# adfriend45/HYBRID9

Measured on AMD Instinct MI355X. Metric: grid-cell-steps/sec at 0.5° global (1/2/4/8 GPUs) + achieved HBM GB/s, higher is better.
Workload: dtype f32

## Files before the change

### hybrid9_amd/csrc/h9g.hip

```cpp
#include <hip/hip_runtime.h>

#include <math.h>
#include <stdio.h>
#include <stdlib.h>
#include <string.h>

#include <algorithm>
#include <atomic>
#include <mutex>
#include <string>
#include <thread>
#include <vector>

#include "../../include/h9g.h"
#include "h9_math.h"
#include "h9g_geo.h"
#include "h9g_step.h"
#include "h9g_pair.h"
#include "h9g_rows.h"
#include "h9g_synth.h"
#include "h9g_io.h"

using namespace h9k;
static_assert(H9G_ERR_NOSNAP_K == H9G_ERR_NOSNAP, "kernel and ABI error codes");
static_assert(H9G_NDAILY == DAILY_ROWS, "the daily line of the ABI and of h9g_rows.h");

__constant__ uint64_t c_exp2tab[32] = H9M_EXP2F_TAB_INIT;
__constant__ double c_log2tab[32] = H9M_POWF_LOG2_TAB_INIT;
static const uint64_t h_exp2tab[32] = H9M_EXP2F_TAB_INIT;
static const double h_log2tab[32] = H9M_POWF_LOG2_TAB_INIT;

#define H9G_BLOCK 256
#define H9G_YBLOCK 64
#define H9G_PCPW 22
#define H9G_PLANES (2 * H9G_PCPW)
#define H9G_PWAVES 4
#define NEVT 64
static size_t round_up(size_t x, size_t m) { return (x + m - 1) / m * m; }

struct KArgs {
  int ncell;
  int c0, cend;
  int nt;
  int nisurf;
  int grow_on;
  size_t fvar;
  const float *__restrict__ par;
  float *__restrict__ st;
  const float *__restrict__ forc;
  float *__restrict__ annual;
  int *__restrict__ err;
  int *__restrict__ err_flag;
  unsigned *__restrict__ stamps;
  float *__restrict__ sv;
  const int *__restrict__ perm;
  int sorted_io;
  int *__restrict__ hist;
  unsigned *__restrict__ pace;
  unsigned epoch;
  int prio_mode;
  int bend, split, nt2;
  float *__restrict__ st2;
  int *__restrict__ err2;
  size_t iostride;
  int raw;
};

#define H9G_NXCD 8
__host__ __device__ __forceinline__ unsigned xcd_vwg(unsigned b, unsigned nb) {
  const unsigned x = b % H9G_NXCD, q = nb / H9G_NXCD, r = nb % H9G_NXCD;
  return x * q + (x < r ? x : r) + b / H9G_NXCD;
}

__device__ __forceinline__ void load_tabs(uint64_t *e2, double *l2) {
  const int t = threadIdx.x;
  if (t < 32) {
    e2[t] = c_exp2tab[t];
    l2[t] = c_log2tab[t];
  }
  __syncthreads();
}

template <int L>
constexpr int pair_waves() { return pair_resident<L>(); }

template <int L, class G, int R, int C = H9G_PCPW, bool MON = false>
__device__ __forceinline__ void pair_body(const KArgs &a, const G &g, float *mon = nullptr) {
  typedef PairStore<L, 2 * C, R> PS;
  __shared__ uint64_t s_e2[32];
  __shared__ double s_l2[32];
  __shared__ float s_cell[H9G_PWAVES][PS::ROWS * 2 * C];
  __shared__ float s_zt[zt_size<L>()];
  static_assert(sizeof(s_e2) + sizeof(s_l2) + sizeof(s_cell) + sizeof(s_zt) <= (size_t)PS::GBLOCK,
                "pair kernel LDS footprint exceeds the day-snapshot block");
  if (threadIdx.x == 0) fill_zt<L>(g, s_zt);
  load_tabs(s_e2, s_l2);
  const h9m::Tabs T = {s_e2, s_l2};
  const int wave = threadIdx.x >> 6, lane = threadIdx.x & 63;
  const bool spare = lane >= 2 * C;
  if (spare && !PS::kSpare) return;
  const int h = lane & 1;
  const int slot0 = __builtin_amdgcn_readfirstlane(
      a.c0 + (int)(xcd_vwg(blockIdx.x, gridDim.x) * H9G_PWAVES + wave) * C);
  const bool g2 = slot0 >= a.split;
  const int lim = g2 ? a.cend : a.bend;
  float *const st = g2 ? a.st2 : a.st;
  int *const err = g2 ? a.err2 : a.err;
  int *const hist = g2 ? nullptr : a.hist;
  const int nt = g2 ? a.nt2 : a.nt;
  const int ncol = min(C, lim - slot0);
  if (ncol <= 0) return;
  const int pl = spare ? (lane - 2 * C + (C == H9G_PCPW ? 12 : 0)) % (2 * ncol) : lane;
  const int slot = slot0 + (pl >> 1);
  if (slot >= lim) return;
  const int c = a.perm ? a.perm[slot] : slot;
  const int io = a.sorted_io ? slot : c;
  const int n = a.ncell;
  const size_t ios = a.sorted_io ? a.iostride : (size_t)n;

  int prow, pslot;
  pace_key(prow, pslot);
  PS cs{(lds_float *)&s_cell[wave][pl], (lds_float *)&s_cell[wave][pl & ~1], (const lds_float *)s_zt,
        a.sv + (size_t)blockIdx.x * (PS::GBLOCK / sizeof(float)),
        Pacer{a.pace + (size_t)prow * 16, a.epoch & 0xfffffu, pslot, a.prio_mode,
              (int)((blockIdx.x * (unsigned)PS::RESIDENT) / gridDim.x)},
        (lds_float *)&s_cell[wave][0]};
  const Split2 sp{h, lane, spare};
  St<L> s;
  if (!spare) {
#pragma unroll
    for (int p = PF_TS; p <= PF_PSI; p++)
#pragma unroll
      for (int t = 0; t < L / 2; t++) cs.set_slot(p, t, a.par[(size_t)par_row(L, p, 2 * t + h) * n + c]);
    cs.set_sc(PS_FMAX, a.par[(size_t)Rows<L>::FMAX * n + c]);
#pragma unroll
    for (int t = 0; t < L / 2; t++) cs.set_slot(PF_ROOTR, t, st[(size_t)rootr_row(L, 2 * t + h) * n + c]);
  }
#pragma unroll
  for (int i = 1; i <= L; i++) {
    s.h2o[i] = st[(size_t)(Rows<L>::H2O + i - 1) * n + c];
    s.smp[i] = st[(size_t)(Rows<L>::SMP + i - 1) * n + c];
  }
  H9K_LOAD_SCALARS(L, s, st, n, c)
  cs.launder();

  if (!spare) {
    H9K_TS_SUM(L, cs, ts_sum)
    if (!(ts_sum > SOIL_TRUNC) || err[c] != 0) {
      if (h == 0) nan_rows(a.annual, Rows<L>::ANNUAL, ios, io);
      if constexpr (MON)
        if (h == 0) nan_rows(mon, H9G_NMONTHS * Rows<L>::ANNUAL, ios, io);
      return;
    }
    cell_inv_pair<L, G>(g, cs);
  }
  if (__builtin_amdgcn_ballot_w64(!spare) == 0) return;
  int eday = 0, estep = 0;
  float errval = 0.0f;
#if defined(H9G_STAMPS)
  StampProf pr{stamp_clock(), {0, 0, 0, 0, 0, 0, 0, 0}};
  const int code = cell_year_pair<L, G, Split2, PS, true>(g, cs, sp, s, (const gbl_float *)(a.forc + io), ios, a.fvar, nt,
                                                         a.nisurf, a.grow_on, (gbl_float *)(a.annual + io), ios, eday,
                                                         estep, errval, T, a.raw, pr);
  if (lane == 0 && a.stamps)
    for (int k = 0; k < 8; k++) a.stamps[(blockIdx.x * H9G_PWAVES + wave) * 8 + k] = pr.acc[k];
#else
  int code;
  if constexpr (MON)
    code = cell_year_pair<L, G, Split2, PS, true, NoProf, Months>(
        g, cs, sp, s, (const gbl_float *)(a.forc + io), ios, a.fvar, nt, a.nisurf, a.grow_on,
        (gbl_float *)(a.annual + io), ios, eday, estep, errval, T, a.raw, NoProf(), Months{(gbl_float *)(mon + io), ios});
  else
    code = cell_year_pair<L, G>(g, cs, sp, s, (const gbl_float *)(a.forc + io), ios, a.fvar, nt, a.nisurf,
                                a.grow_on, (gbl_float *)(a.annual + io), ios, eday, estep, errval, T, a.raw);
#endif
  if (spare || h != 0) return;
  int cw = c, iow = io;
  opaque(cw);
  opaque(iow);
  cs.launder();
  if (hist) hist[cw] = s.naq;
  H9K_STORE_CELL(L, s, cs, st, n, cw, a.grow_on, SC_N)
  if (code) {
    stop_write(err, n, cw, code, eday, estep, errval, a.err_flag);
    nan_rows(a.annual, Rows<L>::ANNUAL, ios, iow);
    if constexpr (MON) nan_rows(mon, H9G_NMONTHS * Rows<L>::ANNUAL, ios, iow);
  }
}

template <int L, class G>
__global__ void __launch_bounds__(64 * H9G_PWAVES)
    __attribute__((amdgpu_waves_per_eu(pair_waves<L>(), pair_waves<L>())))
h9g_pair_kernel(const KArgs a, const G g) {
  pair_body<L, G, pair_waves<L>()>(a, g);
}

template <int L, class G>
__global__ void __launch_bounds__(64 * H9G_PWAVES) __attribute__((amdgpu_waves_per_eu(2, 2)))
h9g_pair2_kernel(const KArgs a, const G g) {
  pair_body<L, G, 2>(a, g);
}

#define H9G_PCPW11 11
template <int L, class G>
__global__ void __launch_bounds__(64 * H9G_PWAVES) __attribute__((amdgpu_waves_per_eu(3, 3)))
h9g_pair11_kernel(const KArgs a, const G g) {
  pair_body<L, G, 3, H9G_PCPW11>(a, g);
}

template <int L, class G>
__global__ void __launch_bounds__(64 * H9G_PWAVES) __attribute__((amdgpu_waves_per_eu(1, 1)))
h9g_pair1_kernel(const KArgs a, const G g) {
  pair_body<L, G, 1, 1>(a, g);
}


#define H9G_SOLO_BODY(MON, mon)                                                                                    \
  typedef SoloStore<L> SS;                                                                                         \
  __shared__ uint64_t s_e2[32];                                                                                    \
  __shared__ double s_l2[32];                                                                                      \
  __shared__ float s_cell[SS::ROWS * H9G_YBLOCK];                                                                  \
  __shared__ float s_zt[zt_size<L>()];                                                                             \
  if (threadIdx.x == 0) fill_zt<L>(g, s_zt);                                                                       \
  load_tabs(s_e2, s_l2);                                                                                           \
  const h9m::Tabs T = {s_e2, s_l2};                                                                                \
  const int slot = a.c0 + (int)(xcd_vwg(blockIdx.x, gridDim.x) * blockDim.x + threadIdx.x);                        \
  if (slot >= a.cend) return;                                                                                      \
  const int c = a.perm ? a.perm[slot] : slot;                                                                      \
  const int io = a.sorted_io ? slot : c;                                                                           \
  const int n = a.ncell;                                                                                           \
  const size_t ios = a.sorted_io ? a.iostride : (size_t)n;                                                         \
  SS cs{(lds_float *)&s_cell[threadIdx.x], (const lds_float *)s_zt};                                               \
  const SplitAll sp;                                                                                               \
  St<L> s;                                                                                                         \
  H9K_LOAD_LANE(L, cs, s, a.par, n, c, a.st, n, c)                                                                 \
  H9K_LOAD_SCALARS(L, s, a.st, n, c)                                                                               \
  cs.launder();                                                                                                    \
  H9K_TS_SUM(L, cs, ts_sum)                                                                                        \
  if (!(ts_sum > SOIL_TRUNC) || a.err[c] != 0) {                                                                   \
    nan_rows(a.annual, Rows<L>::ANNUAL, ios, io);                                                                  \
    if constexpr (MON) nan_rows(mon, H9G_NMONTHS * Rows<L>::ANNUAL, ios, io);                                      \
    return;                                                                                                        \
  }                                                                                                                \
  cell_inv_pair<L, G>(g, cs);                                                                                      \
  int eday = 0, estep = 0;                                                                                         \
  float errval = 0.0f;                                                                                             \
  int code;                                                                                                        \
  if constexpr (MON)                                                                                               \
    code = cell_year_pair<L, G, SplitAll, SS, false, NoProf, Months>(                                              \
        g, cs, sp, s, (const gbl_float *)(a.forc + io), ios, a.fvar, a.nt, a.nisurf, a.grow_on,                    \
        (gbl_float *)(a.annual + io), ios, eday, estep, errval, T, a.raw, NoProf(),                                \
        Months{(gbl_float *)(mon + io), ios});                                                                     \
  else                                                                                                             \
    code = cell_year_pair<L, G, SplitAll, SS, false>(g, cs, sp, s, (const gbl_float *)(a.forc + io), ios, a.fvar,  \
                                                     a.nt, a.nisurf, a.grow_on, (gbl_float *)(a.annual + io), ios, \
                                                     eday, estep, errval, T, a.raw);                               \
  int cw = c, iow = io;                                                                                            \
  opaque(cw);                                                                                                      \
  opaque(iow);                                                                                                     \
  cs.launder();                                                                                                    \
  if (a.hist) a.hist[cw] = s.naq;                                                                                  \
  H9K_STORE_CELL(L, s, cs, a.st, n, cw, a.grow_on, SC_N)                                                           \
  if (code) {                                                                                                      \
    stop_write(a.err, n, cw, code, eday, estep, errval, a.err_flag);                                               \
    nan_rows(a.annual, Rows<L>::ANNUAL, ios, iow);                                                                 \
    if constexpr (MON) nan_rows(mon, H9G_NMONTHS * Rows<L>::ANNUAL, ios, iow);                                     \
  }

template <int L, class G>
__global__ void __launch_bounds__(H9G_YBLOCK) __attribute__((amdgpu_waves_per_eu(2, 2)))
h9g_solo_kernel(const KArgs a, const G g) {
  H9G_SOLO_BODY(false, ((float *)nullptr))
}

template <int L, class G>
__global__ void __launch_bounds__(64 * H9G_PWAVES)
    __attribute__((amdgpu_waves_per_eu(pair_waves<L>(), pair_waves<L>())))
h9g_pair_mon_kernel(const KArgs a, float *mon, const G g) {
  pair_body<L, G, pair_waves<L>(), H9G_PCPW, true>(a, g, mon);
}
template <int L, class G>
__global__ void __launch_bounds__(64 * H9G_PWAVES) __attribute__((amdgpu_waves_per_eu(2, 2)))
h9g_pair2_mon_kernel(const KArgs a, float *mon, const G g) {
  pair_body<L, G, 2, H9G_PCPW, true>(a, g, mon);
}
template <int L, class G>
__global__ void __launch_bounds__(64 * H9G_PWAVES) __attribute__((amdgpu_waves_per_eu(3, 3)))
h9g_pair11_mon_kernel(const KArgs a, float *mon, const G g) {
  pair_body<L, G, 3, H9G_PCPW11, true>(a, g, mon);
}
template <int L, class G>
__global__ void __launch_bounds__(64 * H9G_PWAVES) __attribute__((amdgpu_waves_per_eu(1, 1)))
h9g_pair1_mon_kernel(const KArgs a, float *mon, const G g) {
  pair_body<L, G, 1, 1, true>(a, g, mon);
}
template <int L, class G>
__global__ void __launch_bounds__(H9G_YBLOCK) __attribute__((amdgpu_waves_per_eu(2, 2)))
h9g_solo_mon_kernel(const KArgs a, float *mon, const G g) {
  H9G_SOLO_BODY(true, mon)
}

int h9g_mon_launch(int kind, const h9g_config *cfg, unsigned grid, unsigned block, hipStream_t stream, const KArgs &a,
                   float *mon);
int h9g_mon_stopped(int n, int rows, const int *err0, float *mon, hipStream_t stream);

#if !defined(H9G_MONTHLY_UNIT)
#define H9G_PF_ROWS 32
__global__ void __launch_bounds__(256) h9g_perm_forcing_kernel(int c0, int cend, int cpb, int nt, int n, size_t fvar,
                                                               size_t ds, size_t dvar, const int *__restrict__ perm,
                                                               const float *__restrict__ src, float *__restrict__ dst) {
  const unsigned nb = (unsigned)((cend - c0 + cpb - 1) / cpb), x = blockIdx.x % H9G_NXCD, j = blockIdx.x / H9G_NXCD;
  const unsigned q = nb / H9G_NXCD, r = nb % H9G_NXCD, cnt = q + (x < r ? 1u : 0u);
  const unsigned rows = 7u * (unsigned)nt, rgroups = (rows + H9G_PF_ROWS - 1) / H9G_PF_ROWS;
  if (cnt == 0 || j >= cnt * rgroups) return;
  const unsigned v = x * q + (x < r ? x : r) + j % cnt, r0 = (j / cnt) * H9G_PF_ROWS;
  for (unsigned t = threadIdx.x; t < (unsigned)cpb * H9G_PF_ROWS; t += blockDim.x) {
    const int s = c0 + (int)(v * (unsigned)cpb + t % (unsigned)cpb);
    const unsigned row = r0 + t / (unsigned)cpb;
    if (s >= cend || row >= rows) continue;
    const size_t v = row / (unsigned)nt, d = row % (unsigned)nt;
    dst[v * dvar + d * ds + s] = src[v * fvar + d * (size_t)n + perm[s]];
  }
}
static unsigned perm_forcing_blocks(int c0, int cend, int cpb, int nt) {
  const unsigned nb = (unsigned)((cend - c0 + cpb - 1) / cpb);
  const unsigned cmax = nb / H9G_NXCD + (nb % H9G_NXCD ? 1u : 0u);
  return H9G_NXCD * cmax * ((7u * (unsigned)nt + H9G_PF_ROWS - 1) / H9G_PF_ROWS);
}

__global__ void __launch_bounds__(256) h9g_unperm_annual_kernel(int m, int n, int rows, int s0, size_t ss,
                                                                const int *__restrict__ perm,
                                                                const float *__restrict__ src, float *__restrict__ dst) {
  const int s = s0 + (int)(blockIdx.x * blockDim.x + threadIdx.x);
  if (s >= s0 + m) return;
  const int c = perm[s];
  for (int r = blockIdx.y; r < rows; r += gridDim.y) dst[(size_t)r * n + c] = src[(size_t)r * ss + s];
}

__global__ void __launch_bounds__(256) h9g_chain_kernel(int m, int n, int L, const int *__restrict__ chain,
                                                        const int *__restrict__ pred, const int *__restrict__ first,
                                                        const float *__restrict__ st, const float *__restrict__ st0,
                                                        float *__restrict__ guess, const int *__restrict__ dirty,
                                                        int *__restrict__ flag) {
  const int j = blockIdx.x * blockDim.x + threadIdx.x;
  if (j >= m) return;
  const int k = chain[j];
  const float *src = first[j] ? st0 : st;
  const int p = pred[j];
  int differ = 0;
  for (int i = 0; i < L; i++) {
    const float v = src[(size_t)(smp_row(L, 0) + i) * n + p];
    differ |= __float_as_uint(v) != __float_as_uint(guess[(size_t)i * n + k]);
    guess[(size_t)i * n + k] = v;
  }
  flag[j] = differ | (dirty && dirty[k] ? 2 : 0);
}

__global__ void __launch_bounds__(256) h9g_probe_cmp_kernel(int m, int n, int srows, int rows,
                                                            const int *__restrict__ list,
                                                            const float *__restrict__ stA, const float *__restrict__ stB,
                                                            const int *__restrict__ errA, const int *__restrict__ errB,
                                                            const float *__restrict__ annA,
                                                            const float *__restrict__ annB, int *__restrict__ keep) {
  const int j = blockIdx.x * blockDim.x + threadIdx.x;
  if (j >= m) return;
  const int c = list[j];
  bool same = true;
  H9K_SAME_CELL(same, stA, stB, n, c, srows);
  H9K_SAME_CELL(same, errA, errB, n, c, STOP_ROWS);
  H9K_SAME_CELL(same, annA, annB, n, c, rows);
  keep[j] = !same;
}

__global__ void __launch_bounds__(256) h9g_settle_kernel(int n, int srows, int rows, int ny,
                                                         const float *__restrict__ fin, const int *__restrict__ fin_err,
                                                         float *__restrict__ st0, int *__restrict__ err0,
                                                         int *__restrict__ dirty, float *__restrict__ st,
                                                         int *__restrict__ err, float *__restrict__ ck_last,
                                                         int *__restrict__ eck_last, float *__restrict__ ann) {
  const int c = blockIdx.x * blockDim.x + threadIdx.x;
  if (c >= n) return;
  bool same = true;
  H9K_SAME_CELL(same, fin, st0, n, c, srows);
  H9K_SAME_CELL(same, fin_err, err0, n, c, STOP_ROWS);
  if (same) return;
  H9K_COPY_CELL(st0, n, c, fin, n, c, srows);
  H9K_COPY_CELL(err0, n, c, fin_err, n, c, STOP_ROWS);
  dirty[c] = 1;
  if (err0[c] == 0) return;
  for (int r = 0; r < srows; r++) {
    st[(size_t)r * n + c] = st0[(size_t)r * n + c];
    ck_last[(size_t)r * n + c] = st0[(size_t)r * n + c];
  }
  for (int r = 0; r < STOP_ROWS; r++) {
    err[(size_t)r * n + c] = err0[(size_t)r * n + c];
    eck_last[(size_t)r * n + c] = err0[(size_t)r * n + c];
  }
  for (int y = 0; y < ny; y++)
    for (int r = 0; r < rows; r++) ann[((size_t)y * rows + r) * n + c] = __builtin_nanf("");
}

__global__ void __launch_bounds__(256) h9g_chain_start_kernel(int m, int n, int L, const int *__restrict__ chain,
                                                              const int *__restrict__ pred, const int *__restrict__ first,
                                                              const float *__restrict__ st0, float *__restrict__ st,
                                                              float *__restrict__ guess) {
  const int j = blockIdx.x * blockDim.x + threadIdx.x;
  if (j >= m || !first[j]) return;
  const int k = chain[j], p = pred[j];
  for (int i = 0; i < L; i++) {
    const float v = st0[(size_t)(smp_row(L, 0) + i) * n + p];
    st[(size_t)(smp_row(L, 0) + i) * n + k] = v;
    guess[(size_t)i * n + k] = v;
  }
}

__global__ void __launch_bounds__(256) h9g_restart_kernel(int m, int n, int L, const int *__restrict__ list,
                                                          const float *__restrict__ st0, const int *__restrict__ err0,
                                                          const float *__restrict__ guess, float *__restrict__ st,
                                                          int *__restrict__ err) {
  const int j = blockIdx.x * blockDim.x + threadIdx.x;
  if (j >= m) return;
  const int k = list[j];
  const int rows = state_rows(L);
  H9K_COPY_CELL(st, n, k, st0, n, k, rows);
  for (int i = 0; i < L; i++) st[(size_t)(smp_row(L, 0) + i) * n + k] = guess[(size_t)i * n + k];
  H9K_COPY_CELL(err, n, k, err0, n, k, STOP_ROWS);
}

__global__ void __launch_bounds__(256) h9g_merge_kernel(int m, int n, int rows, const int *__restrict__ list,
                                                        float *__restrict__ st, int *__restrict__ err,
                                                        float *__restrict__ ckpt, int *__restrict__ eckpt,
                                                        const float *__restrict__ ckpt_last,
                                                        const int *__restrict__ eckpt_last, int *__restrict__ keep) {
  const int j = blockIdx.x * blockDim.x + threadIdx.x;
  if (j >= m) return;
  const int k = list[j];
  bool same = true;
  H9K_SAME_CELL(same, st, ckpt, n, k, rows);
  H9K_SAME_CELL(same, err, eckpt, n, k, STOP_ROWS);
  if (same) {
    H9K_COPY_CELL(st, n, k, ckpt_last, n, k, rows);
    H9K_COPY_CELL(err, n, k, eckpt_last, n, k, STOP_ROWS);
  } else {
    H9K_COPY_CELL(ckpt, n, k, st, n, k, rows);
    H9K_COPY_CELL(eckpt, n, k, err, n, k, STOP_ROWS);
  }
  keep[j] = !same;
}

#define H9G_SORT_THREADS 512
template <int L, class G>
__global__ void __launch_bounds__(H9G_SORT_THREADS)
    h9g_sort_kernel(int n, int c0, int cend, int cpb, const float *__restrict__ st, const int *__restrict__ err,
                    const int *__restrict__ hist, int nsub, int *__restrict__ perm, const int *__restrict__ list,
                    const G g) {
  constexpr int NK = L + 10;
// ... 285 lines not shown
                                                                  const float *__restrict__ ps, size_t pitch, int L,
                                                                  int layer, float *__restrict__ par,
                                                                  int *__restrict__ slow) {
  __shared__ float red[H9G_SWAVES][5];
  __shared__ int red_ok[H9G_SWAVES];
  const int c = blockIdx.x;
  const int lane = threadIdx.x & 63, wave = threadIdx.x >> 6;
  const int64_t g = gid[c];
  const int x = (int)(g % nx), y = (int)(g / nx);
  const size_t base = (size_t)y * 60 * pitch + (size_t)x * 60 + lane;
  float s0 = 0.0f, s1 = 0.0f, s2 = 0.0f, s3 = 0.0f, sj = 0.0f;
  bool ok = true;
  if (lane < 60) {
#pragma unroll 5
    for (int r = wave; r < 60; r += H9G_SWAVES) {
      const size_t i = base + (size_t)r * pitch;
      const float a = ts[i];
      if (a >= 0.0f) {
        const float b = ks[i], d = lm[i], e = ps[i];
        s0 += a; s1 += b; s2 += d; s3 += e; sj += 1.0f;
        ok = ok && small_int(a) && small_int(b) && small_int(d) && small_int(e);
      }
    }
  }
#pragma unroll
  for (int o = 32; o > 0; o >>= 1) {
    s0 += __shfl_xor(s0, o); s1 += __shfl_xor(s1, o); s2 += __shfl_xor(s2, o);
    s3 += __shfl_xor(s3, o); sj += __shfl_xor(sj, o);
  }
  const bool wok = __builtin_amdgcn_ballot_w64(!ok) == 0;
  if (lane == 0) {
    red[wave][0] = s0; red[wave][1] = s1; red[wave][2] = s2; red[wave][3] = s3; red[wave][4] = sj;
    red_ok[wave] = wok;
  }
  __syncthreads();
  if (threadIdx.x < 4) {
    const int v = threadIdx.x;
    bool all = true;
    float sum = 0.0f, cnt = 0.0f;
    for (int w = 0; w < H9G_SWAVES; w++) {
      all = all && red_ok[w];
      sum += red[w][v];
      cnt += red[w][4];
    }
    if (!all) {
      if (v == 0) slow[c] = 1;
    } else {
      SoilOut::store(par, L, layer, (size_t)ncell, c, v, sum, (int)cnt);
    }
  }
}

__global__ void h9g_soil_seq_kernel(int nx, int ncell, const int64_t *__restrict__ gid, const float *__restrict__ ts,
                                    const float *__restrict__ ks, const float *__restrict__ lm,
                                    const float *__restrict__ ps, size_t pitch, int L, int layer,
                                    float *__restrict__ par, const int *__restrict__ slow) {
  const int t = blockIdx.x * blockDim.x + threadIdx.x;
  const int c = t >> 2, v = t & 3;
  if (c >= ncell || !slow[c]) return;
  const float *src = v == 0 ? ts : (v == 1 ? ks : (v == 2 ? lm : ps));
  const int64_t g = gid[c];
  const int x = (int)(g % nx), y = (int)(g / nx);
  float sum = 0.0f;
  int j = 0;
  for (int x1 = x * 60; x1 < x * 60 + 60; x1++)
    for (int y1 = y * 60; y1 < y * 60 + 60; y1++) {
      const size_t i = (size_t)y1 * pitch + x1;
      if (ts[i] >= 0.0f) {
        sum = sum + src[i];
        j = j + 1;
      }
    }
  SoilOut::store(par, L, layer, (size_t)ncell, c, v, sum, j);
}

__global__ void __launch_bounds__(64 * H9G_PWAVES) h9g_pace_probe_kernel(unsigned *out, unsigned *arrive,
                                                                         unsigned total, long long spin) {
  extern __shared__ float pad[];
  if (threadIdx.x & 63) return;
  pad[threadIdx.x] = 0.0f;
  const unsigned w = blockIdx.x * (blockDim.x >> 6) + (threadIdx.x >> 6);
  __hip_atomic_fetch_add(arrive, 1u, __ATOMIC_RELAXED, __HIP_MEMORY_SCOPE_AGENT);
  const long long t0 = clock64();
  unsigned seen = 0;
  while ((seen = __hip_atomic_load(arrive, __ATOMIC_RELAXED, __HIP_MEMORY_SCOPE_AGENT)) < total &&
         clock64() - t0 < spin)
    __builtin_amdgcn_s_sleep(2);
  out[3 * w + 0] = __builtin_amdgcn_s_getreg((31 << 11) | 4);
  out[3 * w + 1] = __builtin_amdgcn_s_getreg((3 << 11) | 20) & 15u;
  out[3 * w + 2] = seen >= total ? 1u : 0u;
}

__global__ void h9g_div_kernel(int n, const float *x, const float *d, float *out, int *flag) {
  const int i = blockIdx.x * blockDim.x + threadIdx.x;
  if (i >= n) return;
  MathFast mf{{nullptr, nullptr}, false};
  out[i] = mf.div(x[i], d[i], recip64(d[i]));
  flag[i] = (mf.special || mf.redone) ? 1 : 0;
}

__global__ void h9g_math_kernel(int n, const float *x, const float *y, float *out) {
  __shared__ uint64_t s_e2[32];
  __shared__ double s_l2[32];
  load_tabs(s_e2, s_l2);
  const h9m::Tabs T = {s_e2, s_l2};
  const int i = blockIdx.x * blockDim.x + threadIdx.x;
  if (i >= n) return;
  out[i] = y ? h9m::powf(x[i], y[i], T) : h9m::expf(x[i], T);
}

__global__ void h9g_math_fast_kernel(int n, const float *x, const float *y, float *out, int *flag) {
  __shared__ uint64_t s_e2[32];
  __shared__ double s_l2[32];
  load_tabs(s_e2, s_l2);
  const int i = blockIdx.x * blockDim.x + threadIdx.x;
  if (i >= n) return;
  MathFast mf{{s_e2, s_l2}, false};
  out[i] = y ? mf.powf(x[i], y[i]) : mf.expf(x[i]);
  flag[i] = mf.redone ? 1 : 0;
}

#endif

enum Kind : int {
  K_PAIR = 1,
  K_SOLO = 2,
  K_MIXED = 3,
  K_PAIR2 = 4,
  K_PAIR11 = 5,
  K_PAIR1 = 6,
  K_PROBE = 7,
  K_NSTAT
};
struct KindInfo {
  const char *env;
  int wave_cols;
  int resident;
  bool pair;
  bool second_group;
  Kind pair_part;
  int block_cells;
};
static constexpr KindInfo kind_info(int kind) {
  switch (kind) {
    case K_SOLO: return {"solo", H9G_YBLOCK, pair_resident<8>(), false, false, K_SOLO, H9G_YBLOCK};
    case K_MIXED: return {"mixed", H9G_PCPW, pair_resident<8>(), true, false, K_PAIR, H9G_PCPW * H9G_PWAVES};
    case K_PAIR2: return {"pair2", H9G_PCPW, 2, true, true, K_PAIR2, H9G_PCPW * H9G_PWAVES};
    case K_PAIR11: return {"pair11", H9G_PCPW11, pair_resident<8>(), true, true, K_PAIR11, H9G_PCPW11 * H9G_PWAVES};
    case K_PAIR1: return {"pair1", 1, 1, true, false, K_PAIR1, H9G_PWAVES};
    default: return {"pair", H9G_PCPW, pair_resident<8>(), true, true, K_PAIR, H9G_PCPW * H9G_PWAVES};
  }
}

struct h9g_ctx {
  h9g_config cfg;
  int device = 0;
  int L = 8;
  size_t n = 0;
  hipStream_t sc = nullptr, sx = nullptr;
  float *d_par = nullptr, *d_st = nullptr, *d_forc = nullptr, *d_ann = nullptr;
  int *d_err = nullptr, *d_errflag = nullptr;
  double *d_diag = nullptr;
  int64_t *d_gid = nullptr;
  float *d_lat = nullptr;
  std::vector<int> slot_days;
  std::vector<hipEvent_t> ev_copied, ev_consumed;
  hipEvent_t ev0[NEVT], ev1[NEVT];
  hipEvent_t ev_ext = nullptr, ev_diag = nullptr;
  int nev = 0;
  float last_ms = 0.0f;
  double total_ms = 0.0;
  int last_year = 0;
  int params_set = 0, state_set = 0, ran = 0;
  h9g_error last_err{};
  std::string kname;
  unsigned *d_stamps = nullptr;
  std::vector<int64_t> h_gid;
  std::vector<float *> h_pin;
  std::vector<std::thread> prefetch;
  std::vector<int> prefetch_rc;
  unsigned soil_layers = 0;
  float soil_ms = 0.0f;
  int soil_slow = 0;
  int *d_slow = nullptr;
  float *d_sv = nullptr;
  int *d_perm = nullptr;
  int *d_perm2 = nullptr;
  float *d_forc_s = nullptr;
  float *d_ann_s = nullptr;
  unsigned *d_aqbits = nullptr;
  int64_t dec_stats[4] = {0, 0, 0, 0};
  std::vector<int> chain_id;
  std::vector<int64_t> dec_launches;
  int *d_hist = nullptr;
  int hist_nsub = 0;
  unsigned *d_pace = nullptr;
  unsigned epoch = 0;
  int prio_mode = -1;
  int ncu = 256;
  int sort = 1;
  size_t sv_bytes = 0;
  Kind kind = K_PAIR;
  size_t n_solo = 0;
  size_t ios = 0;
  size_t stamp_words = 0;
  int ev_kind[NEVT] = {};
  int64_t ev_cells[NEVT] = {};
  double kstat[K_NSTAT][3] = {};
  struct OrdBufs *ord = nullptr;
  int64_t ord_stats[9] = {};
  int ord_probe = 1;
  std::vector<int64_t> ord_passes;
  std::vector<int> daily_sel;
  int *d_dsel = nullptr;
  float *d_dst = nullptr;
  float *d_daily = nullptr;
  size_t daily_cap = 0;
  FocusYear *d_fyrs = nullptr;
  size_t fyrs_cap = 0;
  std::vector<FocusYear> h_fyrs;
  std::vector<int> daily_nt;
  int monthly = 0;
  float *d_mon = nullptr;
  float *d_mon_s = nullptr;
  float *d_mon_ret = nullptr;
  size_t mon_ret_cap = 0;
  int mon_base = 0;
  int mon_years = 0;
  bool mon_in_ret = false;
};

static void ord_free(h9g_ctx *ctx);

#define HIPCHK(x)                                                              \
  do {                                                                         \
    hipError_t e_ = (x);                                                       \
    if (e_ != hipSuccess) {                                                    \
      fprintf(stderr, "h9g: %s failed: %s (%s:%d)\n", #x, hipGetErrorString(e_), \
              __FILE__, __LINE__);                                             \
      return H9G_EHIP;                                                         \
    }                                                                          \
  } while (0)

static int days_in_year(int y) {
  if (y % 4 != 0) return 365;
  if (y % 100 != 0) return 366;
  if (y % 400 != 0) return 365;
  return 366;
}

enum GeoKind { GEO_R = 0, GEO_C24 = 24, GEO_C48 = 48 };

static GeoKind geo_kind(const h9g_config &c) {
  const float *zd = c.nlayers == 8 ? ZiDefault<8>::zi : ZiDefault<10>::zi;
  for (int i = 0; i <= c.nlayers + 1; i++)
    if (c.zi[i] != zd[i]) return GEO_R;
  if (c.nisurf == 24) return GEO_C24;
  if (c.nisurf == 48) return GEO_C48;
  return GEO_R;
}

#if defined(H9G_ONLY_C2)
#define H9G_DISPATCH(ctx, KERNEL, GRID, BLOCK, STREAM, ...)                          \
  do {                                                                               \
    if ((ctx)->L != 8 || geo_kind((ctx)->cfg) != GEO_C48) {                          \
      fprintf(stderr, "h9g: H9G_ONLY_C2 build runs config 2 only\n");                \
      return H9G_EINVAL;                                                             \
    }                                                                                \
    KERNEL<8, GeoC<8, 48>><<<GRID, BLOCK, 0, STREAM>>>(__VA_ARGS__, GeoC<8, 48>());  \
  } while (0)
#else
#define H9G_DISPATCH(ctx, KERNEL, GRID, BLOCK, STREAM, ...)                          \
  do {                                                                               \
    const GeoKind gk_ = geo_kind((ctx)->cfg);                                        \
    if ((ctx)->L == 8) {                                                             \
      if (gk_ == GEO_C48)                                                            \
        KERNEL<8, GeoC<8, 48>><<<GRID, BLOCK, 0, STREAM>>>(__VA_ARGS__, GeoC<8, 48>()); \
      else if (gk_ == GEO_C24)                                                       \
        KERNEL<8, GeoC<8, 24>><<<GRID, BLOCK, 0, STREAM>>>(__VA_ARGS__, GeoC<8, 24>()); \
      else                                                                           \
        KERNEL<8, GeoR<8>><<<GRID, BLOCK, 0, STREAM>>>(__VA_ARGS__,                  \
                                                       make_geo_r<8>((ctx)->cfg.zi, (ctx)->cfg.nisurf)); \
    } else {                                                                         \
      if (gk_ == GEO_C48)                                                            \
        KERNEL<10, GeoC<10, 48>><<<GRID, BLOCK, 0, STREAM>>>(__VA_ARGS__, GeoC<10, 48>()); \
      else if (gk_ == GEO_C24)                                                       \
        KERNEL<10, GeoC<10, 24>><<<GRID, BLOCK, 0, STREAM>>>(__VA_ARGS__, GeoC<10, 24>()); \
      else                                                                           \
        KERNEL<10, GeoR<10>><<<GRID, BLOCK, 0, STREAM>>>(__VA_ARGS__,                \
                                                         make_geo_r<10>((ctx)->cfg.zi, (ctx)->cfg.nisurf)); \
    }                                                                                \
  } while (0)
#endif

#if defined(H9G_ONLY_C2)
#define H9G_DISPATCH_L10(ctx, KERNEL, GRID, BLOCK, STREAM, ...) \
  do {                                                          \
    fprintf(stderr, "h9g: H9G_ONLY_C2 build runs config 2 only\n"); \
    return H9G_EINVAL;                                          \
  } while (0)
#else
#define H9G_DISPATCH_L10(ctx, KERNEL, GRID, BLOCK, STREAM, ...)                         \
  do {                                                                              \
    const GeoKind gk_ = geo_kind((ctx)->cfg);                                       \
    if (gk_ == GEO_C48)                                                             \
      KERNEL<10, GeoC<10, 48>><<<GRID, BLOCK, 0, STREAM>>>(__VA_ARGS__, GeoC<10, 48>()); \
    else if (gk_ == GEO_C24)                                                        \
      KERNEL<10, GeoC<10, 24>><<<GRID, BLOCK, 0, STREAM>>>(__VA_ARGS__, GeoC<10, 24>()); \
    else                                                                            \
      KERNEL<10, GeoR<10>><<<GRID, BLOCK, 0, STREAM>>>(__VA_ARGS__,                 \
                                                       make_geo_r<10>((ctx)->cfg.zi, (ctx)->cfg.nisurf)); \
  } while (0)
#endif

#if defined(H9G_ISA_ONLY)
#if defined(H9G_ISA_L10)
template __global__ void h9g_pair_kernel<10, GeoC<10, 24>>(const KArgs, const GeoC<10, 24>);
template __global__ void h9g_pair2_kernel<10, GeoC<10, 24>>(const KArgs, const GeoC<10, 24>);
template __global__ void h9g_pair11_kernel<10, GeoC<10, 24>>(const KArgs, const GeoC<10, 24>);
#else
template __global__ void h9g_pair1_kernel<8, GeoC<8, 48>>(const KArgs, const GeoC<8, 48>);
template __global__ void h9g_pair_kernel<8, GeoC<8, 48>>(const KArgs, const GeoC<8, 48>);
#endif
#elif defined(H9G_MONTHLY_UNIT)
__global__ void __launch_bounds__(256) h9g_stopped_mon_kernel(int n, int rows, const int *__restrict__ err0,
                                                              float *__restrict__ mon) {
  const int c = blockIdx.x * blockDim.x + threadIdx.x;
  if (c >= n || err0[c] == 0) return;
  for (int r = 0; r < rows; r++) mon[(size_t)r * n + c] = __builtin_nanf("");
}

int h9g_mon_stopped(int n, int rows, const int *err0, float *mon, hipStream_t stream) {
  h9g_stopped_mon_kernel<<<(unsigned)((n + 255) / 256), 256, 0, stream>>>(n, rows, err0, mon);
  return 0;
}

int h9g_mon_launch(int kind, const h9g_config *cfg, unsigned grid, unsigned block, hipStream_t stream, const KArgs &a,
                   float *mon) {
  const struct { int L; h9g_config cfg; } c{cfg->nlayers, *cfg};
  switch (kind) {
    case K_SOLO: H9G_DISPATCH(&c, h9g_solo_mon_kernel, grid, block, stream, a, mon); break;
    case K_PAIR2:
      if (c.L != 10) return H9G_EINVAL;
      H9G_DISPATCH_L10(&c, h9g_pair2_mon_kernel, grid, block, stream, a, mon);
      break;
    case K_PAIR11: H9G_DISPATCH(&c, h9g_pair11_mon_kernel, grid, block, stream, a, mon); break;
    case K_PAIR1: H9G_DISPATCH(&c, h9g_pair1_mon_kernel, grid, block, stream, a, mon); break;
    case K_PAIR: H9G_DISPATCH(&c, h9g_pair_mon_kernel, grid, block, stream, a, mon); break;
    default: return H9G_EINVAL;
  }
  return 0;
}
#else
static unsigned nblocks(size_t n) { return (unsigned)((n + H9G_BLOCK - 1) / H9G_BLOCK); }

extern "C" {

int h9g_abi_version(void) { return H9G_ABI_VERSION; }

int h9g_device_count(void) {
  int n = 0;
  if (hipGetDeviceCount(&n) != hipSuccess) return 0;
  return n;
}

int h9g_state_size(int nlayers) { return state_rows(nlayers); }

void h9g_destroy(h9g_ctx *ctx) {
  if (!ctx) return;
  for (auto &t : ctx->prefetch)
    if (t.joinable()) t.join();
  (void)hipSetDevice(ctx->device);
  if (ctx->sc) hipStreamSynchronize(ctx->sc);
  if (ctx->sx) hipStreamSynchronize(ctx->sx);
  (void)hipFree(ctx->d_par);
  (void)hipFree(ctx->d_st);
  (void)hipFree(ctx->d_forc);
  (void)hipFree(ctx->d_ann);
  (void)hipFree(ctx->d_err);
  (void)hipFree(ctx->d_sv);
  (void)hipFree(ctx->d_errflag);
  (void)hipFree(ctx->d_diag);
  (void)hipFree(ctx->d_gid);
  (void)hipFree(ctx->d_lat);
  (void)hipFree(ctx->d_stamps);
  (void)hipFree(ctx->d_slow);
  (void)hipFree(ctx->d_perm);
  (void)hipFree(ctx->d_perm2);
  (void)hipFree(ctx->d_forc_s);
  (void)hipFree(ctx->d_ann_s);
  (void)hipFree(ctx->d_mon);
  (void)hipFree(ctx->d_mon_s);
  (void)hipFree(ctx->d_mon_ret);
  (void)hipFree(ctx->d_hist);
  (void)hipFree(ctx->d_aqbits);
  (void)hipFree(ctx->d_pace);
  (void)hipFree(ctx->d_dsel);
  (void)hipFree(ctx->d_dst);
  (void)hipFree(ctx->d_daily);
  (void)hipFree(ctx->d_fyrs);
  ord_free(ctx);
  for (auto e : ctx->ev_copied) hipEventDestroy(e);
  for (auto e : ctx->ev_consumed) hipEventDestroy(e);
  for (int i = 0; i < NEVT; i++) {
    (void)hipEventDestroy(ctx->ev0[i]);
    (void)hipEventDestroy(ctx->ev1[i]);
  }
  if (ctx->ev_ext) (void)hipEventDestroy(ctx->ev_ext);
  if (ctx->ev_diag) (void)hipEventDestroy(ctx->ev_diag);
  for (auto p : ctx->h_pin) (void)hipHostFree(p);
  if (ctx->sc) hipStreamDestroy(ctx->sc);
  if (ctx->sx) hipStreamDestroy(ctx->sx);
  delete ctx;
}

static Kind l10_kind(size_t n, int ncu, size_t *n_solo) {
  const size_t solo_round = (size_t)4 * ncu * H9G_YBLOCK;
  *n_solo = (n / solo_round) * solo_round;
  const size_t blocks = (n + (size_t)H9G_PCPW * H9G_PWAVES - 1) / ((size_t)H9G_PCPW * H9G_PWAVES);
  return blocks <= (size_t)kind_info(K_PAIR2).resident * ncu ? K_PAIR2 : K_PAIR;
}

static size_t ord_bytes(size_t n, size_t L, size_t ny) {
  const size_t srows = state_rows((int)L), rows = annual_rows((int)L);
  return 2 * (sizeof(float) * (srows + L + ny * (rows + srows)) * n + sizeof(int) * (STOP_ROWS + STOP_ROWS * ny + 1) * n +
              sizeof(int) * 5 * (n + 1)) +
         sizeof(float) * srows * n + sizeof(int) * (STOP_ROWS * n + n + 1) +
         sizeof(float) * (L + 2 * srows + 2 * rows) * n + sizeof(int) * (2 * STOP_ROWS * n + 2 * (n + 1));
}

size_t h9g_config_bytes(const h9g_config *cfg) {
  if (!cfg || cfg->ncell <= 0 || cfg->nlayers < 1 || cfg->max_days < 1 || cfg->nslots < 1) return 0;
  const size_t n = (size_t)cfg->ncell, L = (size_t)cfg->nlayers;
  const size_t ios = 2 * round_up(n, H9G_PCPW) + 64;
  const size_t blocks = std::max((ios + (size_t)H9G_PCPW11 * H9G_PWAVES - 1) / ((size_t)H9G_PCPW11 * H9G_PWAVES),
                                 (size_t)1024 / H9G_PWAVES);
  const size_t prows = par_rows(cfg->nlayers), srows = state_rows(cfg->nlayers), arows = annual_rows(cfg->nlayers);
  return sizeof(float) * (prows + srows + 7 * (size_t)cfg->max_days * (size_t)cfg->nslots + arows + 1) * n +
         sizeof(float) * (7 * (size_t)cfg->max_days + arows) * ios + sizeof(int) * 2 * ios +
         sizeof(int) * (STOP_ROWS + 2) * n + sizeof(int64_t) * n + sizeof(double) * H9G_NDIAG + sizeof(int) +
         blocks * PairStore<8, H9G_PLANES>::GBLOCK + sizeof(unsigned) * 16 * (size_t)H9G_PACE_ROWS +
         ord_bytes(n, L, 10);
}

#define H9G_HEADROOM ((size_t)256 << 20)

static thread_local char g_create_reason[256];

static int config_fail(char *reason, int len, const char *msg) {
  if (reason && len > 0) snprintf(reason, (size_t)len, "%s", msg);
  return H9G_EINVAL;
}

int h9g_config_check(const h9g_config *cfg, char *reason, int reason_len) {
  if (reason && reason_len > 0) reason[0] = 0;
  if (!cfg) return config_fail(reason, reason_len, "cfg is NULL");
  if (cfg->ncell <= 0) return config_fail(reason, reason_len, "ncell must be > 0");
  if (!(cfg->nlayers == 8 || cfg->nlayers == 10))
    return config_fail(reason, reason_len, "nlayers must be 8 or 10");
  if (cfg->nisurf < 1) return config_fail(reason, reason_len, "nisurf must be >= 1");
  if (cfg->max_days < 366) return config_fail(reason, reason_len, "max_days must be >= 366");
  if (cfg->nslots < 1 || cfg->nslots > H9G_MAX_SLOTS)
    return config_fail(reason, reason_len, "nslots must be in [1, H9G_MAX_SLOTS]");
  if ((size_t)cfg->ncell * 7 * (size_t)cfg->max_days > (size_t)INT32_MAX * 4)
    return config_fail(reason, reason_len, "ncell * max_days too large for one slot");
  for (int i = 1; i <= cfg->nlayers + 1; i++)
    if (!(cfg->zi[i] > cfg->zi[i - 1])) return config_fail(reason, reason_len, "zi must increase strictly");
  return 0;
}

const char *h9g_create_error(void) { return g_create_reason; }

h9g_ctx *h9g_create(const h9g_config *cfg, int device) {
  g_create_reason[0] = 0;
  if (h9g_config_check(cfg, g_create_reason, sizeof g_create_reason)) return nullptr;
  if (hipSetDevice(device) != hipSuccess) {
    snprintf(g_create_reason, sizeof g_create_reason, "hipSetDevice(%d) failed: no gfx950 GPU visible?", device);
    return nullptr;
  }
  {
    size_t free_b = 0, total_b = 0;
    const size_t need = h9g_config_bytes(cfg);
    if (hipMemGetInfo(&free_b, &total_b) == hipSuccess && need + H9G_HEADROOM > free_b) {
      snprintf(g_create_reason, sizeof g_create_reason,
               "needs %.2f GB of device memory + %.2f GB headroom, %.2f GB free (reduce nslots=%d)", need / 1e9,
               H9G_HEADROOM / 1e9, free_b / 1e9, cfg->nslots);
      return nullptr;
    }
  }
  h9g_ctx *ctx = new h9g_ctx();
  ctx->cfg = *cfg;
  ctx->device = device;
  ctx->L = cfg->nlayers;
  ctx->n = (size_t)cfg->ncell;
  const size_t n = ctx->n;
  const int L = ctx->L;
  ctx->ios = 2 * round_up(n, H9G_PCPW) + 64;
  bool ok = hipStreamCreateWithFlags(&ctx->sc, hipStreamNonBlocking) == hipSuccess &&
            hipStreamCreateWithFlags(&ctx->sx, hipStreamNonBlocking) == hipSuccess &&
            hipMalloc(&ctx->d_par, sizeof(float) * par_rows(L) * n) == hipSuccess &&
            hipMalloc(&ctx->d_st, sizeof(float) * state_rows(L) * n) == hipSuccess &&
            hipMalloc(&ctx->d_forc, sizeof(float) * 7 * (size_t)cfg->max_days * n * cfg->nslots) == hipSuccess &&
            hipMalloc(&ctx->d_ann, sizeof(float) * annual_rows(L) * n) == hipSuccess &&
            hipMalloc(&ctx->d_err, sizeof(int) * STOP_ROWS * n) == hipSuccess &&
            hipMalloc(&ctx->d_errflag, sizeof(int)) == hipSuccess &&
            hipMalloc(&ctx->d_diag, sizeof(double) * H9G_NDIAG) == hipSuccess &&
            hipMalloc(&ctx->d_gid, sizeof(int64_t) * n) == hipSuccess &&
            hipMalloc(&ctx->d_lat, sizeof(float) * n) == hipSuccess &&
            hipMalloc(&ctx->d_perm, sizeof(int) * ctx->ios) == hipSuccess &&
            hipMalloc(&ctx->d_perm2, sizeof(int) * ctx->ios) == hipSuccess &&
            hipMalloc(&ctx->d_hist, sizeof(int) * n) == hipSuccess;
  if (ok) {
    ok = hipMemset(ctx->d_err, 0, sizeof(int) * STOP_ROWS * n) == hipSuccess &&
         hipMemset(ctx->d_errflag, 0, sizeof(int)) == hipSuccess &&
         hipMemset(ctx->d_diag, 0, sizeof(double) * H9G_NDIAG) == hipSuccess &&
         hipMemset(ctx->d_ann, 0xff, sizeof(float) * annual_rows(L) * n) == hipSuccess &&
         hipMemset(ctx->d_hist, 0xff, sizeof(int) * n) == hipSuccess;
  }
  ctx->slot_days.assign(cfg->nslots, 0);
  ctx->h_pin.assign(cfg->nslots, nullptr);
  ctx->prefetch.resize(cfg->nslots);
  ctx->prefetch_rc.assign(cfg->nslots, 0);
  ctx->ev_copied.resize(cfg->nslots);
  ctx->ev_consumed.resize(cfg->nslots);
  for (int s = 0; ok && s < cfg->nslots; s++)
    ok = hipEventCreateWithFlags(&ctx->ev_copied[s], hipEventDisableTiming) == hipSuccess &&
         hipEventCreateWithFlags(&ctx->ev_consumed[s], hipEventDisableTiming) == hipSuccess;
  for (int i = 0; ok && i < NEVT; i++)
    ok = hipEventCreate(&ctx->ev0[i]) == hipSuccess && hipEventCreate(&ctx->ev1[i]) == hipSuccess;
  if (ok)
    ok = hipEventCreateWithFlags(&ctx->ev_ext, hipEventDisableTiming) == hipSuccess &&
         hipEventCreateWithFlags(&ctx->ev_diag, hipEventDisableTiming) == hipSuccess;
  if (!ok) {
    snprintf(g_create_reason, sizeof g_create_reason, "device allocation failed (ncell=%d, nslots=%d)",
             cfg->ncell, cfg->nslots);
    fprintf(stderr, "h9g_create: %s\n", g_create_reason);
    h9g_destroy(ctx);
    return nullptr;
  }
  if (const char *se = getenv("H9G_SORT")) ctx->sort = atoi(se) != 0;
  if (const char *se = getenv("H9G_PRIO")) ctx->prio_mode = atoi(se);
  if (getenv("H9G_NO_PROBE")) ctx->ord_probe = 0;
  const char *kenv = getenv("H9G_KERNEL");
  int ncu = 256;
  if (hipDeviceGetAttribute(&ncu, hipDeviceAttributeMultiprocessorCount, device) != hipSuccess || ncu < 1)
    ncu = 256;
  ctx->ncu = ncu;
  if (ncu != 32 * H9G_NXCD) {
    static bool said = false;
    if (!said) {
      fprintf(stderr, "h9g: device %d has %d CUs, not %d: XCD-aware cell orders assume %d XCDs (SPX); results are "
                      "unaffected, L2 locality may not hold\n", device, ncu, 32 * H9G_NXCD, H9G_NXCD);
      said = true;
    }
  }
  Kind forced = K_NSTAT;
  for (int k = K_PAIR; kenv && k < K_PROBE; k++)
    if (strcmp(kenv, kind_info(k).env) == 0 && (k != K_PAIR2 || L == 10)) forced = (Kind)k;
  if (forced == K_MIXED) {
    ctx->kind = K_MIXED;
    size_t ns = 0;
    (void)l10_kind(n, ncu, &ns);
    if (const char *sp = getenv("H9G_SPLIT")) ns = (size_t)strtoull(sp, nullptr, 10);
    ctx->n_solo = std::min(ns, n);
  } else if (forced != K_NSTAT)
    ctx->kind = forced;
  else if (L == 8)
    ctx->kind = K_PAIR;
  else
    ctx->kind = l10_kind(n, ncu, &ctx->n_solo);
  const GeoKind gk = geo_kind(*cfg);
  const std::string targs = "<" + std::to_string(L) + "," +
                            (gk == GEO_R ? "GeoR" : "GeoC<" + std::to_string(L) + "," + std::to_string((int)gk) + ">") + ">";
  auto kernel_name = [&](int k) { return "h9g_" + std::string(kind_info(k).env) + "_kernel" + targs; };
  ctx->kname = ctx->kind == K_MIXED ? kernel_name(K_SOLO) + "+" + kernel_name(K_PAIR) : kernel_name(ctx->kind);
  return ctx;
}

int h9g_set_params(h9g_ctx *ctx, const float *theta_s, const float *hksat, const float *bsw,
                   const float *psi_s, const float *fmax) {
  if (!ctx || !theta_s || !hksat || !bsw || !psi_s || !fmax) return H9G_EINVAL;
  const size_t n = ctx->n;
  const int L = ctx->L;
  std::vector<float> rows(par_rows(L) * n);
  const float *src[4] = {theta_s, hksat, bsw, psi_s};
  for (int k = 0; k < 4; k++)
    for (size_t c = 0; c < n; c++)
      for (int i = 0; i < L; i++) rows[(size_t)par_row(L, k, i) * n + c] = src[k][c * L + i];
  memcpy(&rows[(size_t)fmax_row(L) * n], fmax, sizeof(float) * n);
  HIPCHK(hipSetDevice(ctx->device));
  HIPCHK(hipMemcpyAsync(ctx->d_par, rows.data(), sizeof(float) * rows.size(), hipMemcpyHostToDevice, ctx->sc));
  HIPCHK(hipStreamSynchronize(ctx->sc));
  ctx->params_set = 1;
  return 0;
}

int h9g_get_params(h9g_ctx *ctx, float *theta_s, float *hksat, float *bsw, float *psi_s, float *fmax) {
  if (!ctx || !theta_s || !hksat || !bsw || !psi_s || !fmax) return H9G_EINVAL;
  const size_t n = ctx->n;
  const int L = ctx->L;
  std::vector<float> rows(par_rows(L) * n);
  HIPCHK(hipSetDevice(ctx->device));
  HIPCHK(hipStreamSynchronize(ctx->sc));
  HIPCHK(hipMemcpy(rows.data(), ctx->d_par, sizeof(float) * rows.size(), hipMemcpyDeviceToHost));
  float *dst[4] = {theta_s, hksat, bsw, psi_s};
  for (int k = 0; k < 4; k++)
    for (size_t c = 0; c < n; c++)
      for (int i = 0; i < L; i++) dst[k][c * L + i] = rows[(size_t)par_row(L, k, i) * n + c];
  memcpy(fmax, &rows[(size_t)fmax_row(L) * n], sizeof(float) * n);
  return 0;
}

int h9g_init_state(h9g_ctx *ctx) {
  if (!ctx) return H9G_EINVAL;
  if (!ctx->params_set) return H9G_ESTATE;
  HIPCHK(hipSetDevice(ctx->device));
  const int n = (int)ctx->n;
  H9G_DISPATCH(ctx, h9g_init_kernel, nblocks(n), H9G_BLOCK, ctx->sc, n, ctx->d_par, ctx->d_st);
  HIPCHK(hipGetLastError());
  HIPCHK(hipMemsetAsync(ctx->d_err, 0, sizeof(int) * STOP_ROWS * ctx->n, ctx->sc));
  HIPCHK(hipMemsetAsync(ctx->d_errflag, 0, sizeof(int), ctx->sc));
  HIPCHK(hipStreamSynchronize(ctx->sc));
  HIPCHK(hipMemsetAsync(ctx->d_hist, 0xff, sizeof(int) * ctx->n, ctx->sc));
  ctx->hist_nsub = 0;
  ctx->state_set = 1;
  ctx->last_err = h9g_error{};
  return 0;
}

int h9g_set_state(h9g_ctx *ctx, const float *packed) {
  if (!ctx || !packed) return H9G_EINVAL;
  const size_t n = ctx->n;
  std::vector<float> rows((size_t)h9g_state_size(ctx->L) * n);
  state_rows_from_packed(ctx->L, n, packed, rows.data());
  HIPCHK(hipSetDevice(ctx->device));
  HIPCHK(hipMemcpyAsync(ctx->d_st, rows.data(), sizeof(float) * rows.size(), hipMemcpyHostToDevice, ctx->sc));
  HIPCHK(hipMemsetAsync(ctx->d_err, 0, sizeof(int) * STOP_ROWS * n, ctx->sc));
  HIPCHK(hipMemsetAsync(ctx->d_errflag, 0, sizeof(int), ctx->sc));
  HIPCHK(hipStreamSynchronize(ctx->sc));
  HIPCHK(hipMemsetAsync(ctx->d_hist, 0xff, sizeof(int) * ctx->n, ctx->sc));
  ctx->hist_nsub = 0;
  ctx->state_set = 1;
  ctx->last_err = h9g_error{};
  return 0;
}

int h9g_get_state(h9g_ctx *ctx, float *packed) {
  if (!ctx || !packed) return H9G_EINVAL;
  const size_t n = ctx->n;
  std::vector<float> rows((size_t)h9g_state_size(ctx->L) * n);
  HIPCHK(hipSetDevice(ctx->device));
  HIPCHK(hipStreamSynchronize(ctx->sc));
  HIPCHK(hipMemcpy(rows.data(), ctx->d_st, sizeof(float) * rows.size(), hipMemcpyDeviceToHost));
  state_packed_from_rows(ctx->L, n, rows.data(), packed);
  return 0;
}

float *h9g_forcing_slot(h9g_ctx *ctx, int slot) {
  if (!ctx || slot < 0 || slot >= ctx->cfg.nslots) return nullptr;
  return ctx->d_forc + (size_t)slot * 7 * ctx->cfg.max_days * ctx->n;
}

void *h9g_host_alloc(size_t bytes) {
  void *p = nullptr;
  if (hipHostMalloc(&p, bytes, hipHostMallocDefault) != hipSuccess) return nullptr;
  return p;
}

void h9g_host_free(void *p) {
  if (p) (void)hipHostFree(p);
}

static int push_impl(h9g_ctx *ctx, int slot, int nday, const float *src, hipMemcpyKind kind, bool async) {
  if (!ctx || !src || slot < 0 || slot >= ctx->cfg.nslots || nday < 1 || nday > ctx->cfg.max_days)
    return H9G_EINVAL;
  HIPCHK(hipSetDevice(ctx->device));
  float *dst = h9g_forcing_slot(ctx, slot);
  const size_t n = ctx->n;
  HIPCHK(hipStreamWaitEvent(ctx->sx, ctx->ev_consumed[slot], 0));
  HIPCHK(hipMemcpy2DAsync(dst, sizeof(float) * ctx->cfg.max_days * n, src, sizeof(float) * nday * n,
                          sizeof(float) * nday * n, 7, kind, ctx->sx));
  HIPCHK(hipEventRecord(ctx->ev_copied[slot], ctx->sx));
  if (!async) HIPCHK(hipStreamSynchronize(ctx->sx));
  ctx->slot_days[slot] = nday;
  return 0;
}

int h9g_push_forcing(h9g_ctx *ctx, int slot, int nday, const float *forcing, int async) {
  return push_impl(ctx, slot, nday, forcing, hipMemcpyHostToDevice, async != 0);
}

int h9g_push_forcing_device(h9g_ctx *ctx, int slot, int nday, const float *dev_forcing) {
  return push_impl(ctx, slot, nday, dev_forcing, hipMemcpyDeviceToDevice, true);
}

static int join_prefetch(h9g_ctx *ctx, int slot) {
  if (ctx->prefetch[slot].joinable()) ctx->prefetch[slot].join();
  const int rc = ctx->prefetch_rc[slot];
  ctx->prefetch_rc[slot] = 0;
  return rc;
}

#define H9G_PAIR1_MAX 1024
static int pace_mode(const h9g_ctx *ctx, int kind, size_t blocks) {
  if (ctx->prio_mode >= 0) return ctx->prio_mode;
  return blocks <= (size_t)ctx->ncu * kind_info(kind).resident ? 2 : 1;
}

static bool g2_fits(const h9g_ctx *ctx, size_t base, size_t k) {
  const KindInfo ki = kind_info(ctx->kind);
  if (k == 0 || !ctx->sort || !ki.second_group) return false;
#if defined(H9G_DUMP_AQ)
  return false;
#endif
  const size_t C = (size_t)ki.wave_cols, per = (size_t)ki.block_cells;
  if (round_up(base, C) + k > ctx->ios) return false;
  const size_t slots = (size_t)ctx->ncu * ki.resident;
  const size_t b1 = (base + per - 1) / per, b2 = (round_up(base, C) + k + per - 1) / per;
  return (b2 + slots - 1) / slots == (b1 + slots - 1) / slots;
}

static int fold_events(h9g_ctx *ctx) {
  HIPCHK(hipStreamSynchronize(ctx->sc));
  for (int i = 0; i < ctx->nev; i++) {
    float ms = 0.0f;
    HIPCHK(hipEventElapsedTime(&ms, ctx->ev0[i], ctx->ev1[i]));
    ctx->total_ms += ms;
    ctx->last_ms = ms;
    const int k = ctx->ev_kind[i];
    ctx->kstat[k][0] += 1.0;
    ctx->kstat[k][1] += (double)ctx->ev_cells[i];
    ctx->kstat[k][2] += ms;
  }
  ctx->nev = 0;
  return 0;
}

struct YearSpec {
  int slot = 0, jyear = 0;
  const int *d_list = nullptr;
  int m = 0;
  float *ann_dst = nullptr;
  float *mon_dst = nullptr;
  float *st = nullptr;
  int *err = nullptr;
  bool bulk = false;
  const int *h2 = nullptr;
  int k2 = 0, slot2 = 0, jyear2 = 0;
  float *st2 = nullptr, *ann2 = nullptr, *mon2 = nullptr;
  int *err2 = nullptr;
  int ndays = 0;
  bool probe = false;
};

#define H9G_PAIR11_LIST 16384
static Kind list_kind(const h9g_ctx *ctx, int m) {
  if (ctx->kind == K_SOLO) return K_SOLO;
  if (m <= H9G_PAIR1_MAX && !getenv("H9G_NO_PAIR1")) return K_PAIR1;
  if (ctx->L == 8 && ctx->kind == K_PAIR && m <= H9G_PAIR11_LIST && !getenv("H9G_NO_PAIR11")) return K_PAIR11;
  return kind_info(ctx->kind).pair_part;
}

struct LaunchRange { int c0, cend, cpb; Kind kind; };
static int year_ranges(const h9g_ctx *ctx, LaunchRange r[2]) {
  const int n = (int)ctx->n, ns = (int)ctx->n_solo, cpb = kind_info(ctx->kind).block_cells;
  int k = 0;
  if (ctx->kind != K_MIXED) {
    r[k++] = {0, n, cpb, ctx->kind};
  } else {
    if (ns > 0) r[k++] = {0, ns, H9G_YBLOCK, K_SOLO};
    if (ns < n) r[k++] = {ns, n, cpb, K_PAIR};
  }
  return k;
}

static int launch_year(h9g_ctx *ctx, int kind, KArgs a, size_t blocks, float *mon) {
  const unsigned pb = (unsigned)blocks, pt = 64 * H9G_PWAVES;
  if (mon && kind != K_MIXED) {
    const bool solo = kind == K_SOLO;
    if (int rc = h9g_mon_launch(kind, &ctx->cfg, solo ? (unsigned)(((size_t)(a.cend - a.c0) + H9G_YBLOCK - 1) / H9G_YBLOCK) : pb,
                                solo ? H9G_YBLOCK : pt, ctx->sc, a, mon))
      return rc;
    HIPCHK(hipGetLastError());
    return 0;
  }
  switch (kind) {
    case K_SOLO:
      H9G_DISPATCH(ctx, h9g_solo_kernel, (unsigned)(((size_t)(a.cend - a.c0) + H9G_YBLOCK - 1) / H9G_YBLOCK), H9G_YBLOCK,
                   ctx->sc, a);
      break;
    case K_MIXED: {
      LaunchRange r[2];
      const int nr = year_ranges(ctx, r);
      for (int i = 0; i < nr; i++) {
        a.c0 = r[i].c0;
        a.cend = a.bend = a.split = r[i].cend;
        if (int rc = launch_year(ctx, r[i].kind, a, blocks, mon)) return rc;
      }
      return 0;
    }
    case K_PAIR2: H9G_DISPATCH_L10(ctx, h9g_pair2_kernel, pb, pt, ctx->sc, a); break;
    case K_PAIR11: H9G_DISPATCH(ctx, h9g_pair11_kernel, pb, pt, ctx->sc, a); break;
    case K_PAIR1: H9G_DISPATCH(ctx, h9g_pair1_kernel, pb, pt, ctx->sc, a); break;
    default: H9G_DISPATCH(ctx, h9g_pair_kernel, pb, pt, ctx->sc, a); break;
  }
  HIPCHK(hipGetLastError());
  return 0;
}

static int run_year_impl(h9g_ctx *ctx, const YearSpec &ys) {
  const int *d_list = ys.d_list;
  const int m = ys.m;
  if (!ctx || ys.slot < 0 || ys.slot >= ctx->cfg.nslots || ys.jyear < 1861 || ys.jyear > 2299) return H9G_EINVAL;
  if (d_list && (m < 1 || (size_t)m > ctx->n || !ys.ann_dst)) return H9G_EINVAL;
  if (ys.bulk && (!d_list || ys.st || ctx->kind == K_SOLO || ctx->kind == K_MIXED)) return H9G_EINVAL;
  if (ys.probe && (!d_list || ys.bulk || !ys.st || ys.k2 > 0 || ys.ndays < 1)) return H9G_EINVAL;
  const bool two = ys.k2 > 0;
  if (two && ((d_list && !ys.bulk) || !ys.h2 || !ys.st2 || !ys.err2 || !ys.ann2 || ys.slot2 < 0 ||
              ys.slot2 >= ctx->cfg.nslots || ys.jyear2 < 1861 || ys.jyear2 > 2299 ||
              !g2_fits(ctx, d_list ? (size_t)m : ctx->n, (size_t)ys.k2)))
    return H9G_EINVAL;
  if (!ctx->params_set || !ctx->state_set) return H9G_ESTATE;
  const bool mon = ctx->monthly && !ys.probe;
  if (mon && ((d_list && !ys.mon_dst) || (two && !ys.mon2))) return H9G_EINVAL;
#if defined(H9G_DUMP_AQ)
  if (d_list || ys.st) return H9G_EINVAL;
#endif
  if (const int prc = join_prefetch(ctx, ys.slot)) return prc;
  if (two)
    if (const int prc = join_prefetch(ctx, ys.slot2)) return prc;
  const int nt = ys.probe ? std::min(ys.ndays, days_in_year(ys.jyear)) : days_in_year(ys.jyear);
  const int nt2 = two ? days_in_year(ys.jyear2) : nt;
  if (ctx->slot_days[ys.slot] < nt || (two && ctx->slot_days[ys.slot2] < nt2)) return H9G_EINVAL;
  HIPCHK(hipSetDevice(ctx->device));
  HIPCHK(hipStreamWaitEvent(ctx->sc, ctx->ev_copied[ys.slot], 0));
  if (two) HIPCHK(hipStreamWaitEvent(ctx->sc, ctx->ev_copied[ys.slot2], 0));
  const int n = (int)ctx->n;
  const size_t ios = ctx->ios;
  const size_t mrows = (size_t)H9G_NMONTHS * annual_rows(ctx->L);
  if (mon && !ctx->d_mon) {
    HIPCHK(hipMalloc(&ctx->d_mon, sizeof(float) * mrows * ctx->n));
    HIPCHK(hipMemsetAsync(ctx->d_mon, 0xff, sizeof(float) * mrows * ctx->n, ctx->sc));
  }
  KArgs a;
  a.ncell = n;
  a.c0 = 0;
  a.cend = d_list ? m : n;
  a.nt = nt;
  a.nisurf = ctx->cfg.nisurf;
  a.grow_on = ctx->cfg.grow_on;
  a.fvar = (size_t)ctx->cfg.max_days * ctx->n;
  a.par = ctx->d_par;
  a.st = ys.st ? ys.st : ctx->d_st;
  a.forc = h9g_forcing_slot(ctx, ys.slot);
  a.annual = ctx->d_ann;
  a.err = ys.err ? ys.err : ctx->d_err;
  a.err_flag = ctx->d_errflag;
  a.stamps = nullptr;
  a.sv = nullptr;
  a.perm = nullptr;
  a.sorted_io = 0;
  a.hist = ys.st ? nullptr : ctx->d_hist;
  a.bend = a.split = a.cend;
  a.nt2 = nt;
  a.st2 = a.st;
  a.err2 = a.err;
  a.iostride = ios;
  a.raw = ys.probe ? 1 : 0;
  const Kind kind = d_list && !ys.bulk ? list_kind(ctx, m) : ctx->kind;
  const KindInfo ki = kind_info(kind);
  const size_t ncells = d_list ? (size_t)m : ctx->n;
  if (d_list || ctx->sort) {
    if (!ctx->d_forc_s) HIPCHK(hipMalloc(&ctx->d_forc_s, sizeof(float) * 7 * (size_t)ctx->cfg.max_days * ios));
    if (!ctx->d_ann_s) HIPCHK(hipMalloc(&ctx->d_ann_s, sizeof(float) * annual_rows(ctx->L) * ios));
    if (mon && !ctx->d_mon_s) HIPCHK(hipMalloc(&ctx->d_mon_s, sizeof(float) * mrows * ios));
  }
  const size_t dvar = (size_t)ctx->cfg.max_days * ios;
  auto second_group = [&](int base, int pcpb) -> int {
    const int split = (int)round_up((size_t)base, (size_t)ki.wave_cols);
    HIPCHK(hipMemcpyAsync(ctx->d_perm2 + split, ys.h2, sizeof(int) * ys.k2, hipMemcpyHostToDevice, ctx->sc));
    H9G_DISPATCH(ctx, h9g_sort_kernel, H9G_NXCD, H9G_SORT_THREADS, ctx->sc, n, split, split + ys.k2, pcpb, ys.st2,
                 ys.err2, ctx->d_hist, ctx->hist_nsub, ctx->d_perm, ctx->d_perm2);
    h9g_perm_forcing_kernel<<<perm_forcing_blocks(split, split + ys.k2, pcpb, nt2), 256, 0, ctx->sc>>>(
        split, split + ys.k2, pcpb, nt2, n, a.fvar, ios, dvar, ctx->d_perm, h9g_forcing_slot(ctx, ys.slot2),
        ctx->d_forc_s);
    HIPCHK(hipGetLastError());
    a.split = split;
    a.cend = split + ys.k2;
    a.nt2 = nt2;
    a.st2 = ys.st2;
    a.err2 = ys.err2;
    return 0;
  };
  if (d_list) {
    const int pcpb = ki.block_cells;
    a.perm = d_list;
    if (ctx->sort && kind != K_PAIR1) {
      H9G_DISPATCH(ctx, h9g_sort_kernel, H9G_NXCD, H9G_SORT_THREADS, ctx->sc, n, 0, m, pcpb, a.st, a.err, ctx->d_hist,
                   ctx->hist_nsub, ctx->d_perm, d_list);
      a.perm = ctx->d_perm;
    }
    h9g_perm_forcing_kernel<<<perm_forcing_blocks(0, m, pcpb, nt), 256, 0, ctx->sc>>>(
        0, m, pcpb, nt, n, a.fvar, ios, dvar, a.perm, a.forc, ctx->d_forc_s);
    HIPCHK(hipGetLastError());
    if (two)
      if (int r = second_group(m, pcpb)) return r;
    a.forc = ctx->d_forc_s;
    a.annual = ctx->d_ann_s;
    a.sorted_io = 1;
  } else if (ctx->sort) {
    LaunchRange r[2];
    const int nr = year_ranges(ctx, r);
    for (int i = 0; i < nr; i++)
      H9G_DISPATCH(ctx, h9g_sort_kernel, H9G_NXCD, H9G_SORT_THREADS, ctx->sc, n, r[i].c0, r[i].cend, r[i].cpb, ctx->d_st,
                   ctx->d_err, ctx->d_hist, ctx->hist_nsub, ctx->d_perm, nullptr);
    HIPCHK(hipGetLastError());
    a.perm = ctx->d_perm;
#if !defined(H9G_DUMP_AQ)
    for (int i = 0; i < nr; i++)
      h9g_perm_forcing_kernel<<<perm_forcing_blocks(r[i].c0, r[i].cend, r[i].cpb, nt), 256, 0, ctx->sc>>>(
          r[i].c0, r[i].cend, r[i].cpb, nt, n, a.fvar, ios, dvar, ctx->d_perm, a.forc, ctx->d_forc_s);
    HIPCHK(hipGetLastError());
    if (two)
      if (int rc = second_group(n, ki.block_cells)) return rc;
    a.forc = ctx->d_forc_s;
    a.annual = ctx->d_ann_s;
    a.sorted_io = 1;
#endif
  }
  if (a.sorted_io) a.fvar = dvar;
  float *const mon_a = !mon ? nullptr : a.sorted_io ? ctx->d_mon_s : ctx->d_mon;
  const size_t per_block = (size_t)ki.block_cells;
  const size_t blocks = kind == K_MIXED ? (ctx->n - ctx->n_solo + per_block - 1) / per_block
                                        : ((size_t)a.cend + per_block - 1) / per_block;
  if (ki.pair) {
    const size_t need = std::max<size_t>(blocks, 1) * PairStore<8, H9G_PLANES>::GBLOCK;
    if (ctx->sv_bytes < need) {
      (void)hipFree(ctx->d_sv);
      ctx->d_sv = nullptr;
      ctx->sv_bytes = 0;
      HIPCHK(hipMalloc(&ctx->d_sv, need));
      ctx->sv_bytes = need;
    }
    a.sv = ctx->d_sv;
    if (!ctx->d_pace) {
      const size_t pb = sizeof(unsigned) * 16 * H9G_PACE_ROWS;
      HIPCHK(hipMalloc(&ctx->d_pace, pb));
      HIPCHK(hipMemsetAsync(ctx->d_pace, 0, pb, ctx->sc));
    }
  }
  a.pace = ctx->d_pace;
  a.epoch = ++ctx->epoch;
  a.prio_mode = pace_mode(ctx, kind, blocks);
#if defined(H9G_STAMPS)
  {
    const size_t words = (size_t)8 * H9G_PWAVES * (blocks + 1);
    if (ctx->stamp_words < words) {
      (void)hipFree(ctx->d_stamps);
      ctx->d_stamps = nullptr;
      HIPCHK(hipMalloc(&ctx->d_stamps, sizeof(unsigned) * words));
      ctx->stamp_words = words;
    }
    HIPCHK(hipMemsetAsync(ctx->d_stamps, 0, sizeof(unsigned) * words, ctx->sc));
    a.stamps = ctx->d_stamps;
  }
#endif
  if (ctx->nev >= NEVT)
    if (int r = fold_events(ctx)) return r;
#if defined(H9G_DUMP_AQ)
  if (const char *path = getenv("H9G_AQ_DUMP"); path && ctx->d_aqbits && ctx->ran) {
    std::vector<unsigned> bits(12 * ctx->n);
    HIPCHK(hipStreamSynchronize(ctx->sc));
    HIPCHK(hipMemcpy(bits.data(), ctx->d_aqbits, sizeof(unsigned) * bits.size(), hipMemcpyDeviceToHost));
    if (FILE *f = fopen(path, "ab")) {
      const int hdr[2] = {ctx->last_year, (int)ctx->n};
      fwrite(hdr, sizeof(int), 2, f);
      fwrite(bits.data(), sizeof(unsigned), bits.size(), f);
      fclose(f);
    }
  }
  if (!ctx->d_aqbits) HIPCHK(hipMalloc(&ctx->d_aqbits, sizeof(unsigned) * 12 * ctx->n));
  HIPCHK(hipMemsetAsync(ctx->d_aqbits, 0, sizeof(unsigned) * 12 * ctx->n, ctx->sc));
  {
    const float *base = ctx->d_ann;
    HIPCHK(hipMemcpyToSymbolAsync(HIP_SYMBOL(h9g_aq_bits), &ctx->d_aqbits, sizeof(void *), 0,
                                  hipMemcpyHostToDevice, ctx->sc));
    HIPCHK(hipMemcpyToSymbolAsync(HIP_SYMBOL(h9g_aq_base), &base, sizeof(void *), 0, hipMemcpyHostToDevice,
                                  ctx->sc));
  }
#endif
  const int e = ctx->nev++;
  ctx->ev_kind[e] = ys.probe ? K_PROBE : kind;
  ctx->ev_cells[e] = (int64_t)ncells + (two ? ys.k2 : 0);
  HIPCHK(hipEventRecord(ctx->ev0[e], ctx->sc));
  if (int r = launch_year(ctx, kind, a, blocks, mon_a)) return r;
  HIPCHK(hipEventRecord(ctx->ev1[e], ctx->sc));
  HIPCHK(hipEventRecord(ctx->ev_consumed[ys.slot], ctx->sc));
  if (two) HIPCHK(hipEventRecord(ctx->ev_consumed[ys.slot2], ctx->sc));
  if (a.sorted_io) {
    const unsigned rows = (unsigned)annual_rows(ctx->L);
    h9g_unperm_annual_kernel<<<dim3((unsigned)((ncells + 255) / 256), rows), 256, 0, ctx->sc>>>(
        (int)ncells, n, (int)rows, 0, ios, a.perm, ctx->d_ann_s, d_list ? ys.ann_dst : ctx->d_ann);
    if (two)
      h9g_unperm_annual_kernel<<<dim3((unsigned)((ys.k2 + 255) / 256), rows), 256, 0, ctx->sc>>>(
          ys.k2, n, (int)rows, a.split, ios, a.perm, ctx->d_ann_s, ys.ann2);
    if (mon) {
      h9g_unperm_annual_kernel<<<dim3((unsigned)((ncells + 255) / 256), rows), 256, 0, ctx->sc>>>(
          (int)ncells, n, (int)mrows, 0, ios, a.perm, ctx->d_mon_s, d_list ? ys.mon_dst : ctx->d_mon);
      if (two)
        h9g_unperm_annual_kernel<<<dim3((unsigned)((ys.k2 + 255) / 256), rows), 256, 0, ctx->sc>>>(
            ys.k2, n, (int)mrows, a.split, ios, a.perm, ctx->d_mon_s, ys.mon2);
    }
    HIPCHK(hipGetLastError());
  }
  if (!d_list || ys.bulk) {
    h9g_diag_kernel<<<1, 1024, 0, ctx->sc>>>((int)ctx->n, ctx->L, ctx->d_ann, ctx->d_st, ctx->d_err, ctx->d_diag);
    HIPCHK(hipGetLastError());
  }
  if (!ys.st) {
    ctx->last_year = ys.jyear;
    ctx->hist_nsub = nt * ctx->cfg.nisurf;
  }
  ctx->ran = 1;
  return 0;
}


static int daily_begin(h9g_ctx *ctx, int jyear0, int nyears) {
  ctx->daily_nt.clear();
  size_t days = 0;
  for (int y = 0; y < nyears; y++) days += (size_t)days_in_year(jyear0 + y);
  const size_t need = days * H9G_NDAILY * ctx->daily_sel.size();
  if (ctx->daily_cap < need || ctx->fyrs_cap < (size_t)nyears) HIPCHK(hipStreamSynchronize(ctx->sc));
  if (ctx->daily_cap < need) {
    (void)hipFree(ctx->d_daily);
    ctx->d_daily = nullptr;
    ctx->daily_cap = 0;
    if (hipMalloc(&ctx->d_daily, sizeof(float) * need) != hipSuccess) {
      (void)hipGetLastError();
      return H9G_ENOMEM;
    }
    ctx->daily_cap = need;
  }
  if (ctx->fyrs_cap < (size_t)nyears) {
    (void)hipFree(ctx->d_fyrs);
    ctx->d_fyrs = nullptr;
    ctx->fyrs_cap = 0;
    if (hipMalloc(&ctx->d_fyrs, sizeof(FocusYear) * (size_t)nyears) != hipSuccess) {
      (void)hipGetLastError();
      return H9G_ENOMEM;
    }
    ctx->fyrs_cap = (size_t)nyears;
  }
  ctx->h_fyrs.resize(std::max(ctx->h_fyrs.size(), (size_t)nyears));
  return 0;
}

static int daily_launch(h9g_ctx *ctx, const float *st, const float *guess, const int *err, const int32_t *slots,
                        int jyear0, int ny) {
  const int nsel = (int)ctx->daily_sel.size(), n = (int)ctx->n, L = ctx->L;
  const size_t k0 = ctx->daily_nt.size();
  size_t day0 = 0, days = 0;
  for (int nt : ctx->daily_nt) day0 += (size_t)nt;
  if (k0 + (size_t)ny > ctx->fyrs_cap || k0 + (size_t)ny > ctx->h_fyrs.size()) return H9G_ESTATE;
  for (int y = 0; y < ny; y++) {
    const int nt = days_in_year(jyear0 + y);
    if (slots[y] < 0 || slots[y] >= ctx->cfg.nslots || ctx->slot_days[slots[y]] < nt) return H9G_EINVAL;
    ctx->h_fyrs[k0 + y].forc = h9g_forcing_slot(ctx, slots[y]);
    ctx->h_fyrs[k0 + y].nt = nt;
    days += (size_t)nt;
  }
  if ((day0 + days) * H9G_NDAILY * (size_t)nsel > ctx->daily_cap) return H9G_ESTATE;
  HIPCHK(hipMemcpyAsync(ctx->d_fyrs + k0, ctx->h_fyrs.data() + k0, sizeof(FocusYear) * (size_t)ny,
                        hipMemcpyHostToDevice, ctx->sc));
  h9g_focus_gather_kernel<<<(unsigned)((nsel + 255) / 256), 256, 0, ctx->sc>>>(nsel, n, h9g_state_size(L), L, ctx->d_dsel,
                                                                              st, guess, ctx->d_dst);
  HIPCHK(hipGetLastError());
  FocusArgs a;
  a.ncell = n;
  a.nsel = nsel;
  a.nyears = ny;
  a.nisurf = ctx->cfg.nisurf;
  a.grow_on = ctx->cfg.grow_on;
  a.fvar = (size_t)ctx->cfg.max_days * ctx->n;
  a.par = ctx->d_par;
  a.st = ctx->d_dst;
  a.sel = ctx->d_dsel;
  a.err = err;
  a.yrs = ctx->d_fyrs + k0;
  a.out = ctx->d_daily + day0 * H9G_NDAILY * (size_t)nsel;
  H9G_DISPATCH(ctx, h9g_focus_kernel, (unsigned)((nsel + 63) / 64), 64, ctx->sc, a);
  HIPCHK(hipGetLastError());
  for (int y = 0; y < ny; y++) ctx->daily_nt.push_back(days_in_year(jyear0 + y));
  return 0;
}

static int daily_year(h9g_ctx *ctx, int slot, int jyear) {
  if (slot < 0 || slot >= ctx->cfg.nslots || jyear < 1861 || jyear > 2299) return H9G_EINVAL;
  if (!ctx->params_set || !ctx->state_set) return H9G_ESTATE;
  if (const int prc = join_prefetch(ctx, slot)) return prc;
  HIPCHK(hipSetDevice(ctx->device));
  if (int r = daily_begin(ctx, jyear, 1)) return r;
  HIPCHK(hipStreamWaitEvent(ctx->sc, ctx->ev_copied[slot], 0));
  const int32_t s = slot;
  return daily_launch(ctx, ctx->d_st, nullptr, ctx->d_err, &s, jyear, 1);
}

int h9g_set_daily(h9g_ctx *ctx, int nsel, const int32_t *cells) {
  if (!ctx || nsel < 0 || (nsel > 0 && !cells) || (size_t)nsel > ctx->n) return H9G_EINVAL;
  for (int j = 0; j < nsel; j++)
    if (cells[j] < 0 || (size_t)cells[j] >= ctx->n || (j > 0 && cells[j] <= cells[j - 1])) return H9G_EINVAL;
  HIPCHK(hipSetDevice(ctx->device));
  HIPCHK(hipStreamSynchronize(ctx->sc));
  (void)hipFree(ctx->d_dsel);
  (void)hipFree(ctx->d_dst);
  ctx->d_dsel = nullptr;
  ctx->d_dst = nullptr;
  ctx->daily_sel.clear();
  ctx->daily_nt.clear();
  if (nsel == 0) return 0;
  if (hipMalloc(&ctx->d_dsel, sizeof(int) * (size_t)nsel) != hipSuccess ||
      hipMalloc(&ctx->d_dst, sizeof(float) * (size_t)h9g_state_size(ctx->L) * (size_t)nsel) != hipSuccess) {
    (void)hipGetLastError();
    (void)hipFree(ctx->d_dsel);
    ctx->d_dsel = nullptr;
    return H9G_ENOMEM;
  }
  HIPCHK(hipMemcpy(ctx->d_dsel, cells, sizeof(int) * (size_t)nsel, hipMemcpyHostToDevice));
  ctx->daily_sel.assign(cells, cells + nsel);
  return 0;
}

int h9g_get_daily(h9g_ctx *ctx, int k, float *out) {
  if (!ctx || !out) return H9G_EINVAL;
  if (ctx->daily_sel.empty() || ctx->daily_nt.empty()) return H9G_ESTATE;
  if (k < 0 || (size_t)k >= ctx->daily_nt.size()) return H9G_EINVAL;
  HIPCHK(hipSetDevice(ctx->device));
  HIPCHK(hipStreamSynchronize(ctx->sc));
  size_t day0 = 0;
  for (int y = 0; y < k; y++) day0 += (size_t)ctx->daily_nt[(size_t)y];
  const size_t row = (size_t)H9G_NDAILY * ctx->daily_sel.size();
  HIPCHK(hipMemcpy(out, ctx->d_daily + day0 * row, sizeof(float) * (size_t)ctx->daily_nt[(size_t)k] * row,
                   hipMemcpyDeviceToHost));
  return 0;
}

int h9g_run_year(h9g_ctx *ctx, int slot, int jyear) {
  if (ctx && !ctx->daily_sel.empty())
// ... 505 lines not shown
    if (int r = ord_chain(ctx, D, land)) return r;
    if (int r = ord_check(ctx, D, slots, true, S)) return r;
    if (D.phase == OrdDec::RERUN)
      if (int r = ord_run_alone(ctx, D, slots, S)) return r;
    if (D.phase == OrdDec::CHECK)
      if (int r = ord_check(ctx, D, slots, false, S)) return r;
    P = &D;
  }
  if (int r = ord_settle(ctx, *P, slots, S)) return r;
  if (int r = ord_finish(ctx, *P, nullptr, annual, stop_seen)) return r;
  S.dec_passes.push_back(P->np);
  S.passes += P->np;
  if (!ctx->daily_sel.empty()) {
    if (decs.size() != 1) return H9G_EINVAL;
    if (int r = daily_launch(ctx, P->st0, P->guess, P->err0, slots + P->k0, P->y0, P->ny)) return r;
  }
  HIPCHK(hipMemcpyAsync(ctx->d_st, ord_ck(ctx, *P, P->ny - 1), sizeof(float) * srows * n, hipMemcpyDeviceToDevice,
                        ctx->sc));
  HIPCHK(hipMemcpyAsync(ctx->d_err, ord_eck(ctx, *P, P->ny - 1), sizeof(int) * STOP_ROWS * n, hipMemcpyDeviceToDevice, ctx->sc));
  HIPCHK(hipMemcpyAsync(ctx->d_ann, ord_ann(ctx, *P, P->ny - 1), sizeof(float) * rows * n, hipMemcpyDeviceToDevice,
                        ctx->sc));
  h9g_diag_kernel<<<1, 1024, 0, ctx->sc>>>((int)n, L, ctx->d_ann, ctx->d_st, ctx->d_err, ctx->d_diag);
  HIPCHK(hipGetLastError());
  ctx->last_year = P->y0 + P->ny - 1;
  if (passes)
    for (size_t i = 0; i < S.dec_passes.size(); i++) passes[i] = (int32_t)S.dec_passes[i];
  ctx->dec_stats[0] = S.passes;
  ctx->dec_stats[1] = S.rerun_cells;
  ctx->dec_stats[2] = S.rerun_cell_years;
  ctx->dec_stats[3] = S.rerun_launches;
  ctx->dec_launches = S.launch_cells;
  const int64_t os[9] = {(int64_t)decs.size(), S.ticks, S.ride_steps, S.ride_cell_years, S.alone_steps,
                         S.alone_cell_years, S.excluded, S.probed, S.probe_kept};
  std::copy(os, os + 9, ctx->ord_stats);
  ctx->ord_passes = S.dec_passes;
  if (ctx->monthly) {
    ctx->mon_years = ctx->mon_base + nyears;
    ctx->mon_in_ret = true;
  }
  return h9g_sync(ctx);
}

static std::vector<std::pair<int, int>> ref_decades(int jyear0, int nyears) {
  std::vector<std::pair<int, int>> out;
  for (int y = jyear0, end = jyear0 + nyears; y < end;) {
    const int d = y - 1901, start = 1901 + 10 * (d >= 0 ? d / 10 : -((9 - d) / 10));
    const int e = std::min(start + 10, end);
    out.push_back({y, e - y});
    y = e;
  }
  return out;
}

int h9g_run_decade_ordered(h9g_ctx *ctx, const int32_t *slots, int jyear0, int nyears, float *annual, int32_t *passes) {
  if (nyears < 1) return H9G_EINVAL;
  if (ctx && !ctx->daily_sel.empty()) {
    if (jyear0 < 1861 || jyear0 + nyears - 1 > 2299) return H9G_EINVAL;
    HIPCHK(hipSetDevice(ctx->device));
    if (int r = daily_begin(ctx, jyear0, nyears)) return r;
  }
  if (ctx && ctx->monthly)
    if (int r = mon_begin(ctx, nyears)) return r;
  return run_ordered_impl(ctx, slots, jyear0, {{jyear0, nyears}}, annual, passes);
}

int h9g_run_ordered(h9g_ctx *ctx, const int32_t *slots, int jyear0, int nyears, float *annual, int32_t *passes) {
  if (nyears < 1 || jyear0 < 1861) return H9G_EINVAL;
  if (ctx && ctx->monthly)
    if (int r = mon_begin(ctx, nyears)) return r;
  if (ctx && !ctx->daily_sel.empty()) {
    if (!slots || jyear0 + nyears - 1 > 2299) return H9G_EINVAL;
    std::vector<char> used((size_t)ctx->cfg.nslots, 0);
    for (int y = 0; y < nyears; y++)
      if (slots[y] < 0 || slots[y] >= ctx->cfg.nslots || used[(size_t)slots[y]]++) return H9G_EINVAL;
    HIPCHK(hipSetDevice(ctx->device));
    if (int r = daily_begin(ctx, jyear0, nyears)) return r;
    const size_t rows = annual_rows(ctx->L);
    int first = 0, k0 = 0, i = 0;
    for (const auto &d : ref_decades(jyear0, nyears)) {
      ctx->mon_base = k0;
      const int r = run_ordered_impl(ctx, slots + k0, d.first, {d}, annual ? annual + (size_t)k0 * rows * ctx->n : nullptr,
                                     passes ? passes + i : nullptr);
      if (r < 0) return r;
      if (r > 0 && !first) first = r;
      k0 += d.second;
      i++;
    }
    return first;
  }
  return run_ordered_impl(ctx, slots, jyear0, ref_decades(jyear0, nyears), annual, passes);
}

int h9g_set_chains(h9g_ctx *ctx, const int32_t *chain) {
  if (!ctx) return H9G_EINVAL;
  if (!chain) {
    ctx->chain_id.clear();
    return 0;
  }
  for (size_t c = 0; c < ctx->n; c++)
    if (chain[c] < 0 || chain[c] >= (int32_t)ctx->n) {
      fprintf(stderr, "h9g_set_chains: cell %zu has chain id %d, not in [0, ncell): cells outside every reference "
                      "block (shard.reference_blocks gives -1) belong to no rank's run and must be left out of the "
                      "context\n", c, (int)chain[c]);
      return H9G_EINVAL;
    }
  ctx->chain_id.assign(chain, chain + ctx->n);
  return 0;
}

int h9g_decade_stats(h9g_ctx *ctx, int64_t *out, int n) {
  if (!ctx || !out || n < 1) return H9G_EINVAL;
  int m = 0;
  for (; m < n && m < 4; m++) out[m] = ctx->dec_stats[m];
  for (size_t i = 0; m < n && i < ctx->dec_launches.size(); i++) out[m++] = ctx->dec_launches[i];
  return m;
}

int h9g_ordered_stats(h9g_ctx *ctx, int64_t *out, int n) {
  if (!ctx || !out || n < 1) return H9G_EINVAL;
  int m = 0;
  for (; m < n && m < 9; m++) out[m] = ctx->ord_stats[m];
  for (size_t i = 0; m < n && i < ctx->ord_passes.size(); i++) out[m++] = ctx->ord_passes[i];
  return m;
}

int h9g_launch_stats(h9g_ctx *ctx, double *out, int n, int reset) {
  if (!ctx || !out || n < 1) return H9G_EINVAL;
  if (int r = fold_events(ctx)) return r;
  int m = 0;
  for (int k = K_PAIR; k <= K_PROBE; k++)
    for (int j = 0; j < 3 && m < n; j++) out[m++] = ctx->kstat[k][j];
  if (reset)
    for (auto &row : ctx->kstat) row[0] = row[1] = row[2] = 0.0;
  return m;
}

int h9g_sync(h9g_ctx *ctx) {
  if (!ctx) return H9G_EINVAL;
  HIPCHK(hipSetDevice(ctx->device));
  HIPCHK(hipStreamSynchronize(ctx->sx));
  if (int r = fold_events(ctx)) return r;
#if defined(H9G_STAMPS)
  if (ctx->d_stamps && (ctx->kind == K_PAIR || ctx->kind == K_PAIR11 || ctx->kind == K_PAIR1)) {
    const size_t cw = (size_t)kind_info(ctx->kind).wave_cols, nw = (ctx->n + cw - 1) / cw;
    std::vector<unsigned> st(8 * nw);
    HIPCHK(hipMemcpy(st.data(), ctx->d_stamps, sizeof(unsigned) * 8 * nw, hipMemcpyDeviceToHost));
    double sum[8] = {0}, tot = 0;
    for (size_t w = 0; w < nw; w++)
      for (int k = 0; k < 8; k++) sum[k] += st[8 * w + k];
    const double steps = (double)nw * days_in_year(ctx->last_year) * ctx->cfg.nisurf;
    fprintf(stderr, "h9g stamps (cycles/wave/substep):");
    for (int k = 0; k < 8; k++) { fprintf(stderr, " p%d=%.0f", k, sum[k] / steps); tot += sum[k]; }
    fprintf(stderr, " total=%.0f\n", tot / steps);
    std::vector<double> wt(nw, 0.0);
    for (size_t w = 0; w < nw; w++)
      for (int k = 0; k < 8; k++) wt[w] += st[8 * w + k];
    std::vector<double> ws(wt);
    std::sort(ws.begin(), ws.end());
    const double mean = tot / nw;
    fprintf(stderr, "h9g wave totals / mean: min %.3f p50 %.3f p90 %.3f p99 %.3f max %.3f\n", ws[0] / mean,
            ws[nw / 2] / mean, ws[nw * 9 / 10] / mean, ws[nw * 99 / 100] / mean, ws[nw - 1] / mean);
    double bx[8] = {0}, nx[8] = {0}, bs[4] = {0}, ns[4] = {0};
    for (size_t w = 0; w < nw; w++) {
      const size_t b = w / 4;
      bx[b % 8] += wt[w];
      nx[b % 8] += 1;
      bs[w % 4] += wt[w];
      ns[w % 4] += 1;
    }
    {
      const double cut90 = ws[nw * 9 / 10], cut50 = ws[nw / 2];
      double hi[8] = {0}, lo[8] = {0}, nh = 0, nl = 0;
      for (size_t w = 0; w < nw; w++) {
        if (wt[w] >= cut90) { nh++; for (int k = 0; k < 8; k++) hi[k] += st[8 * w + k]; }
        if (wt[w] <= cut50) { nl++; for (int k = 0; k < 8; k++) lo[k] += st[8 * w + k]; }
      }
      const double sub = (double)days_in_year(ctx->last_year) * ctx->cfg.nisurf;
      fprintf(stderr, "h9g slowest 10%% / fastest 50%% waves by phase (cycles/substep):");
      for (int k = 0; k < 8; k++) fprintf(stderr, " p%d %.0f/%.0f", k, hi[k] / nh / sub, lo[k] / nl / sub);
      fprintf(stderr, "\n");
    }
    {
      fprintf(stderr, "h9g mean wave total by slot decile:");
      for (int d = 0; d < 10; d++) {
        double a = 0, c = 0;
        for (size_t w = nw * d / 10; w < nw * (d + 1) / 10; w++) { a += wt[w]; c++; }
        fprintf(stderr, " %.3f", a / c / mean);
      }
      fprintf(stderr, "\n");
    }
    fprintf(stderr, "h9g mean wave total by block%%8:");
    for (int k = 0; k < 8; k++) fprintf(stderr, " %.3f", bx[k] / nx[k] / mean);
    fprintf(stderr, "  by wave-in-block:");
    for (int k = 0; k < 4; k++) fprintf(stderr, " %.3f", bs[k] / ns[k] / mean);
    fprintf(stderr, "\n");
  }
#endif
#if defined(H9G_COUNT_EXACT)
  {
    unsigned long long cnt = 0;
    HIPCHK(hipMemcpyFromSymbol(&cnt, HIP_SYMBOL(h9g_exact_count), sizeof(cnt)));
    fprintf(stderr, "h9g exact re-runs (lanes, cumulative): %llu\n", cnt);
    std::vector<unsigned> w(1 << 16);
    HIPCHK(hipMemcpyFromSymbol(w.data(), HIP_SYMBOL(h9g_exact_wave), sizeof(unsigned) << 16));
    std::vector<std::pair<unsigned, int>> top;
    for (int i = 0; i < (1 << 16); i++)
      if (w[i]) top.push_back({w[i], i});
    std::sort(top.rbegin(), top.rend());
    fprintf(stderr, "h9g exact re-runs: %zu waves;", top.size());
    for (size_t k = 0; k < top.size() && k < 8; k++) fprintf(stderr, " w%d:%u", top[k].second, top[k].first);
    fprintf(stderr, "\n");
  }
#endif
#if defined(H9G_COUNT_BRANCH)
  {
    static const char *names[BR_N] = {"substep", "theta", "qb", "eq_exact", "aqpow", "aq_s", "hk_exact", "tri_flux",
                                      "tri_sweep", "recharge", "baseflow", "watmin", "rerun", "powf_redo",
                                      "div_redo", "expf_redo", "powf_fix", "div_fix", "inl", "any_aq", "jwt_col",
                                      "visit2", "snap", "eb_exact", "day"};
    unsigned long long c[64];
    HIPCHK(hipMemcpyFromSymbol(c, HIP_SYMBOL(h9g_branch_count), sizeof(c)));
    const double ws = c[BR_SUBSTEP] ? (double)c[BR_SUBSTEP] : 1.0;
    fprintf(stderr, "h9g branch counts (wave entries per wave-substep, mean lanes):");
    for (int k = 0; k < BR_N; k++)
      if (c[k]) fprintf(stderr, " %s=%.4g/%.1f", names[k], c[k] / ws, (double)c[32 + k] / c[k]);
    fprintf(stderr, "\n");
    memset(c, 0, sizeof(c));
    HIPCHK(hipMemcpyToSymbol(HIP_SYMBOL(h9g_branch_count), c, sizeof(c)));
  }
#endif
  int flag = 0;
  HIPCHK(hipMemcpy(&flag, ctx->d_errflag, sizeof(int), hipMemcpyDeviceToHost));
  if (!flag) return 0;
  if (ctx->last_err.code == 0) {
    const size_t n = ctx->n;
    std::vector<int> e(STOP_ROWS * n);
    HIPCHK(hipMemcpy(e.data(), ctx->d_err, sizeof(int) * STOP_ROWS * n, hipMemcpyDeviceToHost));
    for (size_t c = 0; c < n; c++) {
      if (e[c]) {
        ctx->last_err.code = e[c];
        ctx->last_err.cell = (int)c;
        ctx->last_err.year = ctx->last_year;
        ctx->last_err.day = e[n + c];
        ctx->last_err.substep = e[2 * n + c];
        ctx->last_err.value = __builtin_bit_cast(float, e[3 * n + c]);
        break;
      }
    }
  }
  return ctx->last_err.code;
}

int h9g_run_site(h9g_ctx *ctx, int nday, const float *sub, const float *daily, const float *lai, float *diag) {
  if (!ctx || nday <= 0 || !sub || !daily || !lai || !diag) return H9G_EINVAL;
  if (!ctx->params_set || !ctx->state_set) return H9G_ESTATE;
  HIPCHK(hipSetDevice(ctx->device));
  HIPCHK(hipStreamSynchronize(ctx->sc));
  const size_t n = ctx->n, ns = (size_t)ctx->cfg.nisurf;
  const size_t nsub = (size_t)nday * ns * 5 * n, nd = (size_t)nday * 2 * n, nl = (size_t)nday * 3 * n;
  const size_t nout = (size_t)nday * DAILY_ROWS * n;
  float *buf = nullptr;
  HIPCHK(hipMalloc(&buf, sizeof(float) * (nsub + nd + nl + nout)));
  SiteArgs a;
  a.ncell = (int)n;
  a.nday = nday;
  a.nisurf = ctx->cfg.nisurf;
  a.par = ctx->d_par;
  a.st = ctx->d_st;
  a.sub = buf;
  a.daily = buf + nsub;
  a.lai = buf + nsub + nd;
  a.out = buf + nsub + nd + nl;
  a.err = ctx->d_err;
  a.err_flag = ctx->d_errflag;
  int rc = 0;
  hipError_t e = hipMemcpy(buf, sub, sizeof(float) * nsub, hipMemcpyHostToDevice);
  if (e == hipSuccess) e = hipMemcpy(buf + nsub, daily, sizeof(float) * nd, hipMemcpyHostToDevice);
  if (e == hipSuccess) e = hipMemcpy(buf + nsub + nd, lai, sizeof(float) * nl, hipMemcpyHostToDevice);
  if (e == hipSuccess) {
    H9G_DISPATCH(ctx, h9g_site_kernel, (unsigned)((n + 63) / 64), 64, ctx->sc, a);
    e = hipGetLastError();
  }
  if (e == hipSuccess) e = hipStreamSynchronize(ctx->sc);
  if (e == hipSuccess) e = hipMemcpy(diag, a.out, sizeof(float) * nout, hipMemcpyDeviceToHost);
  (void)hipFree(buf);
  if (e != hipSuccess) {
    fprintf(stderr, "h9g: h9g_run_site failed: %s\n", hipGetErrorString(e));
    return H9G_EHIP;
  }
  ctx->last_year = 0;
  ctx->ran = 1;
  rc = h9g_sync(ctx);
  return rc;
}

int h9g_get_errors(h9g_ctx *ctx, int32_t *rec) {
  if (!ctx || !rec) return H9G_EINVAL;
  HIPCHK(hipSetDevice(ctx->device));
  HIPCHK(hipStreamSynchronize(ctx->sc));
  HIPCHK(hipMemcpy(rec, ctx->d_err, sizeof(int32_t) * STOP_ROWS * ctx->n, hipMemcpyDeviceToHost));
  return 0;
}

int h9g_last_error(h9g_ctx *ctx, h9g_error *err) {
  if (!ctx || !err) return H9G_EINVAL;
  *err = ctx->last_err;
// ... 348 lines not shown
```

### hybrid9_amd/csrc/h9g_pair.h

```cpp
#pragma once
#include "h9g_step.h"
#include "h9g_expr.h"
#if !defined(__HIPCC__) && !defined(__HIP__)
#define __device__
#define __forceinline__ inline
#endif

#ifndef H9G_EXACT_HOOK
#define H9G_EXACT_HOOK(k0, ns)
#endif
#if defined(H9G_COUNT_EXACT)
__device__ unsigned long long h9g_exact_count;
__device__ unsigned h9g_exact_wave[1 << 16];
#endif
namespace h9k {

enum : int {
  PF_TS = 0, PF_HKS, PF_BSW, PF_PSI,
  PF_NINVB,
  PF_ITS,
  PF_PTE,
  PF_C3,
  PF_ROOTR,
  PF_RPSI0, PF_RPSI1,
  PF_RTS0, PF_RTS1,
  PF_SVH2O, PF_SVSMP,
  PF_N
};
enum : int {
  PS_FMAX = 0, PS_MH3, PS_TSDZ1, PS_DAY,
  PS_LAI = PS_DAY + D_N,
  PS_LAIL, PS_PM, PS_PFM, PS_PLEN, PS_RDEPTH,
  PS_DR0,
  PS_DRS = PS_DR0 + 4 * DRP_N,
  PS_SVZWT = PS_DR0 + 2 * DR_N,
  PS_SVWA, PS_SVRNF, PS_SVERR, PS_SVNS,
  PS_N
};
enum : int { SV_ZWT = 0, SV_WA, SV_RNF, SV_ERR, SV_NS };
static_assert((PS_DAY + D_NUMC) % 2 == 0 && (PS_DAY + D_RAARAC) % 2 == 0 && (PS_DAY + D_DGRAC) % 2 == 0 &&
                  (PS_DAY + D_DRR) % 2 == 0 && (PS_DAY + D_RAC) % 2 == 0 && PS_DR0 % 2 == 0,
              "pair fields must start a row");

#ifndef H9G_EB_FAST
#define H9G_EB_FAST 1
#endif
#ifndef H9G_P1_TASKS
#define H9G_P1_TASKS 7
#endif

template <int K>
struct FV {
  float v[K];
};

H9K_HD float sel(int h, float a, float b) { return h ? b : a; }
H9K_HD double seld(int h, double a, double b) { return h ? b : a; }

H9K_HD float pair_swap(float v) {
#if defined(__HIP_DEVICE_COMPILE__)
  const int x = __builtin_bit_cast(int, v);
  return __builtin_bit_cast(float, __builtin_amdgcn_update_dpp(x, x, 0xB1, 0xF, 0xF, false));
#else
  return v;
#endif
}

template <int E>
H9K_HD float pair_bcast(float v) {
#if defined(__HIP_DEVICE_COMPILE__)
  const int x = __builtin_bit_cast(int, v);
  return __builtin_bit_cast(float, __builtin_amdgcn_mov_dpp(x, E ? 0xF5 : 0xA0, 0xF, 0xF, true));
#else
  return v;
#endif
}

H9K_HD float lane_get(float v, int src) {
#if defined(__HIP_DEVICE_COMPILE__)
  return __builtin_bit_cast(float, __builtin_amdgcn_ds_bpermute(src << 2, __builtin_bit_cast(int, v)));
#else
  (void)src;
  return v;
#endif
}
H9K_HD int lane_geti(int v, int src) {
#if defined(__HIP_DEVICE_COMPILE__)
  return __builtin_amdgcn_ds_bpermute(src << 2, v);
#else
  (void)src;
  return v;
#endif
}

H9K_HD float lane0_get(float v) {
#if defined(__HIP_DEVICE_COMPILE__)
  return __builtin_bit_cast(float, __builtin_amdgcn_readlane(__builtin_bit_cast(int, v), 0));
#else
  return v;
#endif
}
H9K_HD int lane0_geti(int v) {
#if defined(__HIP_DEVICE_COMPILE__)
  return __builtin_amdgcn_readlane(v, 0);
#else
  return v;
#endif
}
H9K_HD uint64_t lane_mask(bool p) {
#if defined(__HIP_DEVICE_COMPILE__)
  return __builtin_amdgcn_ballot_w64(p);
#else
  return p ? 1u : 0u;
#endif
}

H9K_HD double join_d(float lo, float hi) {
  return __builtin_bit_cast(double, (uint64_t)__builtin_bit_cast(uint32_t, hi) << 32 |
                                        __builtin_bit_cast(uint32_t, lo));
}
H9K_HD float lo_d(double v) { return __builtin_bit_cast(float, (uint32_t)__builtin_bit_cast(uint64_t, v)); }
H9K_HD float hi_d(double v) {
  return __builtin_bit_cast(float, (uint32_t)(__builtin_bit_cast(uint64_t, v) >> 32));
}

template <int L>
struct FlatStore {
  static constexpr bool kRecip = true, kRts = true, kDayRecip = true, kRtsHK = true, kSpare = false;
  static constexpr int N = PF_N * L + PS_N;
  float *b;
  const float *zt;
  H9K_HD float zi(int i) const { return zt[i]; }
  H9K_HD float zim(int i) const { return zt[L + 2 + i]; }
  H9K_HD double rdz_t(int i) const { return join_d(zt[2 * (L + 2) + 2 * i], zt[2 * (L + 2) + 2 * i + 1]); }
  H9K_HD float lay(int p, int i) const { return b[p * L + i - 1]; }
  H9K_HD void set_lay(int p, int i, float v) const { b[p * L + i - 1] = v; }
  H9K_HD float sc(int k) const { return b[PF_N * L + k]; }
  H9K_HD void set_sc(int k, float v) const { b[PF_N * L + k] = v; }
  H9K_HD float slot(int p, int t) const { return b[p * L + 2 * t]; }
  H9K_HD void set_slot(int p, int t, float v) const { b[p * L + 2 * t] = v; }
  H9K_HD void launder() {}
  H9K_HD float day(int f) const { return sc(PS_DAY + f); }
  H9K_HD void set_day(int f, float v) const { set_sc(PS_DAY + f, v); }
  H9K_HD double day_r(int k) const { return join_d(sc(PS_DRS + 2 * k), sc(PS_DRS + 2 * k + 1)); }
  H9K_HD void set_day_r(int k, double v) const {
    set_sc(PS_DRS + 2 * k, lo_d(v));
    set_sc(PS_DRS + 2 * k + 1, hi_d(v));
  }
  H9K_HD double day_rp(int j, int h) const { return join_d(sc(PS_DR0 + 4 * j + h), sc(PS_DR0 + 4 * j + 2 + h)); }
  H9K_HD void set_day_rp(int j, int h, double v) const {
    set_sc(PS_DR0 + 4 * j + h, lo_d(v));
    set_sc(PS_DR0 + 4 * j + 2 + h, hi_d(v));
  }
  H9K_HD float root(int i) const { return lay(PF_ROOTR, i); }
  H9K_HD void set_root(int i, float v) const { set_lay(PF_ROOTR, i, v); }
  H9K_HD float sv_lay(int q, int i) const { return lay(PF_SVH2O + q, i); }
  H9K_HD void sv_set_lay(int q, int i, float v) const { set_lay(PF_SVH2O + q, i, v); }
  H9K_HD float sv_sc(int k) const { return sc(PS_SVZWT + k); }
  H9K_HD void sv_set_sc(int k, float v) const { set_sc(PS_SVZWT + k, v); }
  H9K_HD void sv_sync() const {}
  H9K_HD void day_start(int) const {}
};

struct Pacer {
  unsigned *row;
  unsigned epoch;
  int me;
  int mode;
  int round;
  __device__ __forceinline__ static void set_prio(int p) {
#if defined(__HIP_DEVICE_COMPILE__)
    if (p <= 0)
      __builtin_amdgcn_s_setprio(0);
    else if (p == 1)
      __builtin_amdgcn_s_setprio(1);
    else if (p == 2)
      __builtin_amdgcn_s_setprio(2);
    else
      __builtin_amdgcn_s_setprio(3);
#endif
  }
  __device__ __forceinline__ void day_start(int day, int resident) const {
#if defined(__HIP_DEVICE_COMPILE__)
    if (mode == 1) {
      set_prio((round + day) % resident);
    } else if (mode == 2) {
      const unsigned mine = (epoch << 12) | (unsigned)(day + 1);
      __hip_atomic_store(row + me, mine, __ATOMIC_RELAXED, __HIP_MEMORY_SCOPE_AGENT);
      const int k = (int)(__lane_id() & 15);
      const unsigned v = __hip_atomic_load(row + k, __ATOMIC_RELAXED, __HIP_MEMORY_SCOPE_AGENT);
      const bool ahead = k != me && (v >> 12) == (epoch & 0xfffffu) && (v & 0xfffu) > (unsigned)(day + 1);
      const uint64_t m = __builtin_amdgcn_ballot_w64(ahead);
      const unsigned slots = (unsigned)(m | (m >> 16) | (m >> 32) | (m >> 48)) & 0xffffu;
      set_prio(__builtin_popcount(slots));
    }
#endif
  }
};
#define H9G_PACE_ROWS 16384
__device__ __forceinline__ void pace_key(int &row, int &slot) {
#if defined(__HIP_DEVICE_COMPILE__)
  const unsigned hw = __builtin_amdgcn_s_getreg((31 << 11) | 4);
  const unsigned xcc = __builtin_amdgcn_s_getreg((3 << 11) | 20) & 15u;
  slot = (int)(hw & 15u);
  row = (int)(((((xcc * 8u + ((hw >> 13) & 7u)) * 2u + ((hw >> 12) & 1u)) * 16u + ((hw >> 8) & 15u)) * 4u) +
              ((hw >> 4) & 3u));
#else
  row = slot = 0;
#endif
}

template <int L>
constexpr int pair_resident() { return 3; }

template <int L, int S, int R = pair_resident<L>()>
struct PairStore {
  static constexpr int NT = L / 2;
  static constexpr bool kRecip = true, kRts = L <= 8 || R <= 2 || S <= 22, kDayRecip = L <= 8 || R <= 2 || S <= 22;
  static constexpr bool kRtsHK = kRts;
  static constexpr int NPF = kRecip ? (kRts ? PF_SVH2O : PF_RTS0) : PF_RPSI0;
  static constexpr int NPS = kDayRecip ? PS_SVZWT : PS_DR0;
  static constexpr int TH0 = (NPF * NT + (NPS + 1) / 2) * S;
  static constexpr int ROWS = NPF * NT + (NPS + 1) / 2 + (S == 2 ? NT : 0);
  static constexpr int GBLOCK = 65536;
  lds_float *self, *even;
  const lds_float *zt;
  float *svw;
  static constexpr int RESIDENT = R;
  Pacer pace;
  lds_float *wb;
  static constexpr int LANES = S;
  static constexpr bool kSpare = !(L >= 10 && R >= 3 && S >= 44);
  __device__ __forceinline__ void day_start(int day) const { pace.day_start(day, RESIDENT); }
  __device__ __forceinline__ float zi(int i) const { return zt[i]; }
  __device__ __forceinline__ float zim(int i) const { return zt[L + 2 + i]; }
  __device__ __forceinline__ double rdz_t(int i) const {
    return join_d(zt[2 * (L + 2) + 2 * i], zt[2 * (L + 2) + 2 * i + 1]);
  }
  __device__ __forceinline__ float lay(int p, int i) const {
    return even[(p * NT + ((i - 1) >> 1)) * S + ((i - 1) & 1)];
  }
  __device__ __forceinline__ void set_lay(int p, int i, float v) const {
    even[(p * NT + ((i - 1) >> 1)) * S + ((i - 1) & 1)] = v;
  }
  __device__ __forceinline__ float sc(int k) const { return even[(NPF * NT + (k >> 1)) * S + (k & 1)]; }
  __device__ __forceinline__ void set_sc(int k, float v) const {
    even[(NPF * NT + (k >> 1)) * S + (k & 1)] = v;
  }
  __device__ __forceinline__ float slot(int p, int t) const { return self[(p * NT + t) * S]; }
  __device__ __forceinline__ void set_slot(int p, int t, float v) const { self[(p * NT + t) * S] = v; }
  __device__ __forceinline__ void launder() {
#if defined(__HIP_DEVICE_COMPILE__)
    asm volatile("" : "+v"(self), "+v"(even), "+v"(zt)::"memory");
#endif
  }
  __device__ __forceinline__ float day(int f) const { return sc(PS_DAY + f); }
  __device__ __forceinline__ void set_day(int f, float v) const { set_sc(PS_DAY + f, v); }
  __device__ __forceinline__ double day_r(int k) const {
    return join_d(sc(PS_DRS + 2 * k), sc(PS_DRS + 2 * k + 1));
  }
  __device__ __forceinline__ void set_day_r(int k, double v) const {
    set_sc(PS_DRS + 2 * k, lo_d(v));
    set_sc(PS_DRS + 2 * k + 1, hi_d(v));
  }
  __device__ __forceinline__ double day_rp(int j, int h) const {
    return join_d(sc(PS_DR0 + 4 * j + h), sc(PS_DR0 + 4 * j + 2 + h));
  }
  __device__ __forceinline__ void set_day_rp(int j, int h, double v) const {
    set_sc(PS_DR0 + 4 * j + h, lo_d(v));
    set_sc(PS_DR0 + 4 * j + 2 + h, hi_d(v));
  }
  __device__ __forceinline__ float sc_own(int k) const { return self[(NPF * NT + (k >> 1)) * S]; }
  __device__ __forceinline__ double day_rp_own(int j) const {
    return join_d(sc_own(PS_DR0 + 4 * j), sc_own(PS_DR0 + 4 * j + 2));
  }
  __device__ __forceinline__ float root(int i) const { return lay(PF_ROOTR, i); }
  __device__ __forceinline__ void set_root(int i, float v) const { set_lay(PF_ROOTR, i, v); }
  __device__ __forceinline__ float *gl(const lds_float *p, int off) const {
    return (float *)((char *)svw + (uint32_t)(size_t)p) + off;
  }
  __device__ __forceinline__ void sv_set_slot(int q, int t, float v) const { *gl(self, (q * NT + t) * S) = v; }
  __device__ __forceinline__ float sv_lay(int q, int i) const {
    return *gl(even, (q * NT + ((i - 1) >> 1)) * S + ((i - 1) & 1));
  }
  __device__ __forceinline__ void sv_set_lay(int q, int i, float v) const {
    *gl(even, (q * NT + ((i - 1) >> 1)) * S + ((i - 1) & 1)) = v;
  }
  __device__ __forceinline__ float sv_sc(int k) const { return *gl(even, (2 * NT + (k >> 1)) * S + (k & 1)); }
  __device__ __forceinline__ void sv_set_sc(int k, float v) const {
    *gl(even, (2 * NT + (k >> 1)) * S + (k & 1)) = v;
  }
  __device__ __forceinline__ void sv_sync() const {
#if defined(__HIP_DEVICE_COMPILE__)
    __builtin_amdgcn_fence(__ATOMIC_SEQ_CST, "agent");
#endif
  }
};

template <int L>
struct SoloStore {
  static constexpr bool kRecip = false, kRts = false, kDayRecip = false, kRtsHK = false, kSpare = false;
  static constexpr int NPF = PF_RPSI0 + 2;
  static constexpr int NPS = PS_LAI + 5;
  static constexpr int ROWS = NPF * L + NPS;
  lds_float *b;
  const lds_float *zt;
  H9K_HD static constexpr int pr(int p) { return p < PF_RPSI0 ? p : p - (PF_SVH2O - PF_RPSI0); }
  H9K_HD static constexpr int kr(int k) { return k < PS_LAI ? k : k - (PS_SVZWT - PS_LAI); }
  __device__ __forceinline__ float zi(int i) const { return zt[i]; }
  __device__ __forceinline__ float zim(int i) const { return zt[L + 2 + i]; }
  __device__ __forceinline__ double rdz_t(int i) const {
    return join_d(zt[2 * (L + 2) + 2 * i], zt[2 * (L + 2) + 2 * i + 1]);
  }
  __device__ __forceinline__ float lay(int p, int i) const { return b[(pr(p) * L + i - 1) * 64]; }
  __device__ __forceinline__ void set_lay(int p, int i, float v) const { b[(pr(p) * L + i - 1) * 64] = v; }
  __device__ __forceinline__ float sc(int k) const { return b[(NPF * L + kr(k)) * 64]; }
  __device__ __forceinline__ void set_sc(int k, float v) const { b[(NPF * L + kr(k)) * 64] = v; }
  __device__ __forceinline__ float slot(int p, int t) const { return b[(pr(p) * L + 2 * t) * 64]; }
  __device__ __forceinline__ void set_slot(int p, int t, float v) const { b[(pr(p) * L + 2 * t) * 64] = v; }
  __device__ __forceinline__ void launder() {
#if defined(__HIP_DEVICE_COMPILE__)
    asm volatile("" : "+v"(b), "+v"(zt)::"memory");
#endif
  }
  __device__ __forceinline__ float day(int f) const { return sc(PS_DAY + f); }
  __device__ __forceinline__ void set_day(int f, float v) const { set_sc(PS_DAY + f, v); }
  __device__ __forceinline__ double day_r(int) const { return 0.0; }
  __device__ __forceinline__ void set_day_r(int, double) const {}
  __device__ __forceinline__ double day_rp(int, int) const { return 0.0; }
  __device__ __forceinline__ void set_day_rp(int, int, double) const {}
  __device__ __forceinline__ float root(int i) const { return lay(PF_ROOTR, i); }
  __device__ __forceinline__ void set_root(int i, float v) const { set_lay(PF_ROOTR, i, v); }
  __device__ __forceinline__ float sv_lay(int q, int i) const { return lay(PF_SVH2O + q, i); }
  __device__ __forceinline__ void sv_set_lay(int q, int i, float v) const { set_lay(PF_SVH2O + q, i, v); }
  __device__ __forceinline__ float sv_sc(int k) const { return sc(PS_SVZWT + k); }
  __device__ __forceinline__ void sv_set_sc(int k, float v) const { set_sc(PS_SVZWT + k, v); }
  __device__ __forceinline__ void sv_sync() const {}
  __device__ __forceinline__ void day_start(int) const {}
};

struct NoProf {
#if defined(H9G_ISA_PHASES) && defined(__HIP_DEVICE_COMPILE__)
  template <int K>
  __device__ __forceinline__ void markk() { asm volatile("; h9g-phase %0" ::"i"(K)); }
  H9K_HD void mark(int k) {
    switch (k) {
      case 0: markk<0>(); break;
      case 1: markk<1>(); break;
      case 2: markk<2>(); break;
      case 3: markk<3>(); break;
      case 4: markk<4>(); break;
      case 5: markk<5>(); break;
      case 6: markk<6>(); break;
      default: markk<7>(); break;
    }
  }
#else
  H9K_HD void mark(int) {}
#endif
  H9K_HD void flux(float, float) {}
};
struct FluxProf {
  float evg, tran;
  H9K_HD void mark(int) {}
  H9K_HD void flux(float e, float t) { evg = e; tran = t; }
};
#if defined(H9G_STAMPS)
H9K_HD uint64_t stamp_clock() {
#if defined(__HIP_DEVICE_COMPILE__)
  return __builtin_amdgcn_s_memtime();
#else
  return 0;
#endif
}
struct StampProf {
  uint64_t last;
  uint32_t acc[8];
  H9K_HD void mark(int k) {
    const uint64_t t = stamp_clock();
    acc[k] += (uint32_t)(t - last);
    last = t;
  }
  H9K_HD void flux(float, float) {}
};
#endif

struct SplitAll {
  static constexpr bool kSpare = false;
  H9K_HD constexpr bool act() const { return true; }
  H9K_HD SplitAll fresh() const { return *this; }
  template <class CS>
  H9K_HD float own(const CS &cs, int p, int t, int h) const { return cs.lay(p, 2 * t + 1 + h); }
  template <int NT, int K, int FE = 1, class FF, class FX>
  H9K_HD void par_d(FF fast, FX exact, float *const (&out)[K]) const {
#pragma unroll
    for (int t = 0; t < NT; t++) {
#pragma unroll
      for (int h = 0; h < 2; h++) {
        bool bad = false;
        FV<K> r = fast(t, h, bad);
        if (bad) r = exact(t, h);
#pragma unroll
        for (int k = 0; k < K; k++) out[k][2 * t + 1 + h] = r.v[k];
      }
      sched_fence();
    }
  }
  template <int K, class F>
  H9K_HD void pick(F f, FV<K> &r0, FV<K> &r1) const {
    r0 = f(0);
    r1 = f(1);
  }
  H9K_HD bool pair_any(bool p) const { return p; }
  template <class CS>
  H9K_HD float own_sc(const CS &cs, int k, int h) const { return cs.sc(k + h); }
  template <class CS>
  H9K_HD double own_day_rp(const CS &cs, int j, int h) const { return cs.day_rp(j, h); }
};

struct Split2 {
  int h;
  int ln;
  bool spare;
  static constexpr bool kSpare = true;
  H9K_HD bool act() const { return !spare; }
  H9K_HD Split2 fresh() const {
    Split2 r{h, ln, spare};
    opaque(r.h);
    return r;
  }
  H9K_HD void xchg(float v, float &e, float &o) const {
    e = pair_bcast<0>(v);
    o = pair_bcast<1>(v);
  }
  template <class CS>
  H9K_HD float own(const CS &cs, int p, int t, int) const { return cs.slot(p, t); }
  template <int NT, int K, int FE = 1, class FF, class FX>
  H9K_HD void par_d(FF fast, FX exact, float *const (&out)[K]) const {
    FV<K> r[NT];
    bool bad = false;
#pragma unroll
    for (int t = 0; t < NT; t++) {
      r[t] = fast(t, h, bad);
      if ((t + 1) % FE == 0 || t == NT - 1) sched_fence();
    }
    if (__builtin_expect(bad, 0)) {
#pragma unroll
      for (int t = 0; t < NT; t++) r[t] = exact(t, h);
    }
#pragma unroll
    for (int t = 0; t < NT; t++) {
#pragma unroll
      for (int k = 0; k < K; k++) xchg(r[t].v[k], out[k][2 * t + 1], out[k][2 * t + 2]);
    }
  }
  template <int K, class F>
  H9K_HD void pick(F f, FV<K> &r0, FV<K> &r1) const {
    const FV<K> r = f(h);
#pragma unroll
    for (int k = 0; k < K; k++) xchg(r.v[k], r0.v[k], r1.v[k]);
  }
  H9K_HD bool pair_any(bool p) const {
    const float f = p ? 1.0f : 0.0f;
    return (f + pair_swap(f)) != 0.0f;
  }
  template <class CS>
  H9K_HD float own_sc(const CS &cs, int k, int) const { return cs.sc_own(k); }
  template <class CS>
  H9K_HD double own_day_rp(const CS &cs, int j, int) const { return cs.day_rp_own(j); }
};

template <int L, class CS>
H9K_HD void save_layers(const SplitAll &, const CS &cs, int q, const float *v) {
#pragma unroll
  for (int i = 1; i <= L; i++) cs.sv_set_lay(q, i, v[i]);
}
template <int L, class CS>
H9K_HD void save_layers(const Split2 &sp, const CS &cs, int q, const float *v) {
#pragma unroll
  for (int t = 0; t < L / 2; t++) cs.sv_set_slot(q, t, sel(sp.h, v[2 * t + 1], v[2 * t + 2]));
}

template <class CS>
H9K_HD void set_lay_d(const CS &cs, int p, int i, double v) {
  cs.set_lay(p, i, lo_d(v));
  cs.set_lay(p + 1, i, hi_d(v));
}
template <class CS>
H9K_HD double lay_d(const CS &cs, int p, int i) { return join_d(cs.lay(p, i), cs.lay(p + 1, i)); }

template <bool Use, class M, class R>
H9K_HD float divr(M &m, float x, float d, R rget) {
  if constexpr (Use)
    return m.div(x, d, rget());
  else
    return x / d;
}

template <bool Use, class M, class R>
H9K_HD float divr_d(M &m, float x, float d, R rget, bool &bad) {
  if constexpr (Use) {
    const float q = m.div_d(x, d, rget());
    bad |= m.div_bad(q);
    return q;
  } else {
    return x / d;
  }
}
template <bool Use, class M>
H9K_HD void divr_fix(M &m, float &q, float x, float d) {
  if constexpr (Use) m.div_fix(q, x, d);
}

template <class M>
H9K_HD float expf_fast(M &m, float x, bool &sp) {
  if constexpr (M::kExact)
    return m.expf(x);
  else
    return h9m::expf_nx(x, m.T, sp);
}

template <class M, class F>
H9K_HD void visit_layers(M &m, F visit) {
  if constexpr (M::kExact) {
    for (int k = 0;; k++)
      if (!visit(k)) break;
  } else {
    bool more = visit(0);
    if (any_lane(more)) {
      H9G_BR(BR_VISIT2);
      if (more) more = visit(1);
      m.special |= more;
    }
  }
}

template <int L>
constexpr int zt_size() { return 4 * (L + 2); }
template <int L, class G, class T>
H9K_HD void fill_zt(const G &g, T *zt) {
#pragma unroll
  for (int i = 0; i <= L + 1; i++) {
    zt[i] = g.zi(i);
    zt[L + 2 + i] = g.zi(i) / 1000.0f;
    const double r = (i > 0 && i <= L) ? g.rdz(i) : 0.0;
    zt[2 * (L + 2) + 2 * i] = lo_d(r);
    zt[2 * (L + 2) + 2 * i + 1] = hi_d(r);
  }
}

template <int L, class G, class CS>
H9K_HD void cell_inv_pair(const G &g, const CS &cs) {
#pragma unroll
  for (int i = 1; i <= L; i++) {
    const int ip = (L < i + 1) ? L : i + 1;
    const float ts = cs.lay(PF_TS, i), tsp = cs.lay(PF_TS, ip);
    const float bsw = cs.lay(PF_BSW, i), psi = cs.lay(PF_PSI, i);
    const float e = one - one / bsw;
    cs.set_lay(PF_NINVB, i, -one / bsw);
    cs.set_lay(PF_ITS, i, one / (ts + tsp));
    const float pte = psi * ts / e;
    cs.set_lay(PF_PTE, i, pte);
    cs.set_lay(PF_C3, i, pte / (g.zi(i) - g.zi(i - 1)));
    if constexpr (CS::kRecip) set_lay_d(cs, PF_RPSI0, i, recip64(-psi));
    if constexpr (CS::kRts) set_lay_d(cs, PF_RTS0, i, recip64(ts));
  }
  float mh = cs.lay(PF_HKS, 1);
  if (cs.lay(PF_HKS, 2) < mh) mh = cs.lay(PF_HKS, 2);
  if (cs.lay(PF_HKS, 3) < mh) mh = cs.lay(PF_HKS, 3);
  cs.set_sc(PS_MH3, mh);
  cs.set_sc(PS_TSDZ1, MAXF(zero, (cs.lay(PF_TS, 1) * g.dz(1))));
}

template <class M, class SP, class CS>
constexpr bool pair1_tasks() {
  if constexpr (H9G_P1_TASKS && SP::kSpare && CS::kSpare && !M::kExact)
    return CS::LANES == 2;
  else
    return false;
}

template <int L, class G, class M, class SP, class CS, class PR = NoProf>
H9K_HD int hydrology_pair(const G &g, CS cs, const SP &sp0, St<L> &s, float &rnf_sum, float &errval,
                          M &m, PR &pr) {
  constexpr int NT = L / 2;
  const SP sp = L >= 10 ? sp0.fresh() : sp0;
  const float dt = g.dt();
  constexpr double r1000 = 1.0 / 1000.0;
  float zim[L + 1];
#pragma unroll
  for (int i = 1; i <= L; i++) zim[i] = g.zim(i);
  float *h2o = s.h2o, *smp = s.smp;
  float theta[L + 1];
  cs.launder();
#define TS(i) cs.lay(PF_TS, i)
#define HKS(i) cs.lay(PF_HKS, i)
#define BSW(i) cs.lay(PF_BSW, i)
#define PSI(i) cs.lay(PF_PSI, i)
#define LAYF(F, i) cs.lay(F, i)
#define ROOT(i) cs.lay(PF_ROOTR, i)
#define DC(F) cs.sc(PS_DAY + F)
#define OWN(p) sp.own(cs, p, t, h)

  float w0 = DC(D_FORC) * dt + s.wa;
  bool bad = false;
#pragma unroll
  for (int i = 1; i <= L; i++) {
    w0 = w0 + h2o[i];
    theta[i] = m.div_d(h2o[i], g.thk(i), g.rthk(i));
    bad |= m.div_bad(theta[i]);
  }
  if (__builtin_expect(bad, 0)) {
    H9G_BR(BR_THETA);
#pragma unroll
    for (int i = 1; i <= L; i++) m.div_fix(theta[i], h2o[i], g.thk(i));
  }
  const float qflx_top_soil = DC(D_FORC);
  const float hkdepth = one / 2.5f;
  const float fff = 1.0f / hkdepth;
  const float fsat = cs.sc(PS_FMAX) * m.expf(-0.5f * fff * s.zwt);
  float qflx_surf = fsat * qflx_top_soil;
  const float frac_h2osfc = zero;
  float beta = zero;
  {
    float rb[L + 1];
    float *const out[1] = {rb};
    auto qb_x = [&](int t, int h) __attribute__((always_inline)) {
      return sel(h, smp[2 * t + 1] - g.zc(2 * t + 1), smp[2 * t + 2] - g.zc(2 * t + 2));
    };
    auto term = [&](int t, int h, float q) __attribute__((always_inline)) {
      float b = one - q;
      b = MINC(one, b);
      b = MAXF(zero, b);
      return FV<1>{{sp.own(cs, PF_ROOTR, t, h) * b}};
    };
    sp.template par_d<NT, 1, NT>(
        [&](int t, int h, bool &bad) __attribute__((always_inline)) -> FV<1> {
          const float q = m.div_d(qb_x(t, h), -150000.0f, 1.0 / -150000.0);
          bad |= m.div_bad(q);
          return term(t, h, q);
        },
        [&](int t, int h) __attribute__((always_inline)) -> FV<1> {
          H9G_BR(BR_QB);
          return term(t, h, m.div(qb_x(t, h), -150000.0f, 1.0 / -150000.0));
        },
        out);
#pragma unroll
    for (int i = 1; i <= L; i++) beta = beta + rb[i];
  }
  float rss;
  if (theta[1] <= 0.15f)
    rss = (10.0f + DC(D_LIT1000)) * m.expf(0.3563f * 100.0f * (0.15f - theta[1]));
  else
    rss = (10.0f + DC(D_LIT1000) * (1.0f - divr<CS::kRts>(m, theta[1], TS(1), [&]() { return lay_d(cs, PF_RTS0, 1); })));
  const float desatdT = DC(D_DESAT), gamma = DC(D_GAMMA);
  const float Ra = DC(D_DG) * DC(D_RAA);
  float rsc, tran, evg;
  bool eb_fast = false;
  if constexpr (H9G_EB_FAST && !M::kExact && CS::kDayRecip) {
    bool bad = false;
    auto mdiv = [&](float x, float d) __attribute__((always_inline)) { return mk_div(x, d, bad); };
    auto ddiv = [&](float x, float d, auto rget) __attribute__((always_inline)) {
      const float q = m.div_d(x, d, rget());
      bad |= m.div_bad(q);
      return q;
    };
    const bool open = (DC(D_OK) != zero) && (beta > zero);
    bool bo = bad;
    const float q_rsc = mdiv(DC(D_X), DC(D_LAI2) * beta * DC(D_PW28));
    bad = bo | (open && bad);
    float rscf = open ? q_rsc : 1.0E6f;
    rscf = MAXF(rscf, DC(D_RSCMIN));
    FV<2> c2, s2;
    sp.template pick<2>(
        [&](int h) __attribute__((always_inline)) -> FV<2> {
          const float r = sel(h, rscf, rss);
          const float q = ddiv(r, sp.own_sc(cs, PS_DAY + D_RAARAC, h), [&]() { return sp.own_day_rp(cs, DRP_RAARA, h); });
          const float PM = mdiv(sp.own_sc(cs, PS_DAY + D_NUMC, h), desatdT + gamma * (one + q));
          const float R = sp.own_sc(cs, PS_DAY + D_DGRAC, h) + gamma * r;
          return FV<2>{{PM, R}};
        },
        c2, s2);
    FV<1> cc, cs1;
    sp.template pick<1>(
        [&](int h) __attribute__((always_inline)) -> FV<1> {
          const float Rh = sel(h, c2.v[1], s2.v[1]), Ro = sel(h, s2.v[1], c2.v[1]);
          return FV<1>{{mdiv(one, one + mdiv(Rh * Ra, Ro * (Rh + Ra)))}};
        },
        cc, cs1);
    const float LEf = cc.v[0] * c2.v[0] + cs1.v[0] * s2.v[0];
    const float VDD0f = DC(D_VDD) + ddiv((DC(D_A1) - DC(D_DG) * LEf) * DC(D_RAA), DC(D_RHOCP),
                                              [&]() { return cs.day_r(DR_RHOCP); });
    FV<1> ft, fe;
    sp.template pick<1>(
        [&](int h) __attribute__((always_inline)) -> FV<1> {
          const float r = sel(h, rscf, rss);
          const float d = sp.own_sc(cs, PS_DAY + D_RAC, h);
          auto rr = [&]() __attribute__((always_inline)) { return sp.own_day_rp(cs, DRP_RA, h); };
          const float LEh = mdiv(sp.own_sc(cs, PS_DAY + D_DRR, h) + ddiv(DC(D_RHOCP) * VDD0f, d, rr),
                                 desatdT + gamma * (1.0f + ddiv(r, d, rr)));
          return FV<1>{{ddiv(LEh * 1.0E3f, DC(D_RL), [&]() { return cs.day_r(DR_RL); })}};
        },
        ft, fe);
#if defined(H9G_FORCE_RERUN)
    bad |= (__builtin_bit_cast(uint32_t, theta[1]) & 15u) == 0;
#endif
    if (!__builtin_expect(any_lane(bad), 0)) {
      rsc = rscf;
      tran = ft.v[0];
      evg = fe.v[0];
      eb_fast = true;
    }
  }
  if (!eb_fast) {
  H9G_BR(BR_EBX);
  if ((DC(D_OK) != zero) && (beta > zero))
    rsc = DC(D_X) / (DC(D_LAI2) * beta * DC(D_PW28));
  else
    rsc = 1.0E6f;
  rsc = MAXF(rsc, DC(D_RSCMIN));
  FV<2> ebc, ebs;
  sp.template pick<2>(
      [&](int h) __attribute__((always_inline)) -> FV<2> {
        const float r = sel(h, rsc, rss);
        const float q = divr<CS::kDayRecip>(m, r, sp.own_sc(cs, PS_DAY + D_RAARAC, h),
                                            [&]() { return sp.own_day_rp(cs, DRP_RAARA, h); });
        const float PM = sp.own_sc(cs, PS_DAY + D_NUMC, h) / (desatdT + gamma * (one + q));
        const float R = sp.own_sc(cs, PS_DAY + D_DGRAC, h) + gamma * r;
        return FV<2>{{PM, R}};
      },
      ebc, ebs);
  const float PMc = ebc.v[0], Rc = ebc.v[1], PMs = ebs.v[0], Rs = ebs.v[1];
  FV<1> ccf, csf;
  sp.template pick<1>(
      [&](int h) __attribute__((always_inline)) -> FV<1> {
        const float Rh = sel(h, Rc, Rs), Ro = sel(h, Rs, Rc);
        return FV<1>{{one / (one + Rh * Ra / (Ro * (Rh + Ra)))}};
      },
      ccf, csf);
  const float LE = ccf.v[0] * PMc + csf.v[0] * PMs;
  const float VDD0 = DC(D_VDD) + divr<CS::kDayRecip>(m, (DC(D_A1) - DC(D_DG) * LE) * DC(D_RAA), DC(D_RHOCP),
                                                     [&]() { return cs.day_r(DR_RHOCP); });
  FV<1> ftr, fev;
  sp.template pick<1>(
      [&](int h) __attribute__((always_inline)) -> FV<1> {
        const float r = sel(h, rsc, rss);
        const float d = sp.own_sc(cs, PS_DAY + D_RAC, h);
        auto rr = [&]() __attribute__((always_inline)) { return sp.own_day_rp(cs, DRP_RA, h); };
        const float LEh = (sp.own_sc(cs, PS_DAY + D_DRR, h) + divr<CS::kDayRecip>(m, DC(D_RHOCP) * VDD0, d, rr)) /
                          (desatdT + gamma * (1.0f + divr<CS::kDayRecip>(m, r, d, rr)));
        return FV<1>{{divr<CS::kDayRecip>(m, LEh * 1.0E3f, DC(D_RL), [&]() { return cs.day_r(DR_RL); })}};
      },
      ftr, fev);
  tran = ftr.v[0];
  evg = fev.v[0];
  }
  float em1 = m.div(g.dz(1) * (theta[1] - watmin), dt, g.rdt()) - tran * ROOT(1);
  em1 = MAXF(zero, em1);
  evg = MINF(em1, evg);
  pr.flux(evg, tran);
  const float qflx_evap = evg;
  float qflx_in_soil = (one - frac_h2osfc) * (qflx_top_soil - qflx_surf);
  qflx_in_soil = qflx_in_soil - (one - frac_h2osfc) * qflx_evap;
  const float qinmax = (one - fsat) * cs.sc(PS_MH3);
  const float qflx_infl_excess = MAXF(zero, qflx_in_soil - (one - frac_h2osfc) * qinmax);
  const float qflx_infl = qflx_in_soil - qflx_infl_excess;
  qflx_surf = qflx_surf + qflx_infl_excess;
  float zwtmm = 1000.0f * s.zwt;
  const int jwt = jwt_of<L>(s.zwt, zim);
  const bool aq = (jwt == L);
  cs.launder();
  pr.mark(1);

  float zq[L + 2];
  float hk[L + 1], dhkdw[L + 1], dsmpdw[L + 1];
  constexpr bool kTask = pair1_tasks<M, SP, CS>();
  FV<1> p0{{zero}}, p1{{zero}};
  FV<2> eA{{zero, zero}}, eS{{zero, zero}};
  bool picks = true, aq_task = false;
  float c_q[L + 1], c_1[L + 1], c_2[L + 1];
  bool flux_done = false;
  float rc_smp = zero, rc_zq = zero;
  {
    float *const outq[1] = {zq};
    float *const outk[4] = {hk, dhkdw, smp, dsmpdw};
    auto eq_exact = [&](int t, int h) __attribute__((always_inline)) -> FV<1> {
          H9G_BR(BR_EQX);
          const int i0 = 2 * t + 1;
          const int il = i0 + h;
          const float zlo = cs.zi(il - 1), zhi = cs.zi(il);
          const float ts = OWN(PF_TS), psi = OWN(PF_PSI);
          float vol_eq;
          if (zwtmm <= zlo) {
            vol_eq = ts;
          } else {
            const float expo = one + OWN(PF_NINVB);
            auto rp = [&]() __attribute__((always_inline)) {
              return join_d(OWN(PF_RPSI0), OWN(PF_RPSI1));
            };
            const bool inl = (zwtmm < zhi) && (zwtmm > zlo);
            const float n0 = ((-psi) + zwtmm - zlo), ni = (-psi + zwtmm - zhi);
            bool bq = false;
            float b0 = divr_d<CS::kRecip>(m, n0, -psi, rp, bq);
            float bi = divr_d<CS::kRecip>(m, ni, -psi, rp, bq);
            if (__builtin_expect(bq, 0)) {
              divr_fix<CS::kRecip>(m, b0, n0, -psi);
              divr_fix<CS::kRecip>(m, bi, ni, -psi);
            }
            bi = inl ? one : bi;
            bool s0, si;
            float temp0 = m.powf_d(b0, expo, s0);
            float tpi = m.powf_d(bi, expo, si);
            if (__builtin_expect(s0 | si, 0)) {
              m.powf_fix(temp0, b0, expo, s0);
              m.powf_fix(tpi, bi, expo, si);
            }
            if (inl) {
              const float tempi = one;
              const float voleq1 = OWN(PF_PTE) / (zwtmm - zlo) * (tempi - temp0);
              vol_eq = m.div(voleq1 * (zwtmm - zlo) + ts * (zhi - zwtmm), zhi - zlo, cs.rdz_t(il));
              vol_eq = MINF(ts, vol_eq);
              vol_eq = MAXF(vol_eq, zero);
            } else {
              vol_eq = vol_eq_below(OWN(PF_C3), ts, tpi, temp0);
            }
          }
          const float qv = divr<CS::kRts>(m, vol_eq, ts, [&]() { return join_d(OWN(PF_RTS0), OWN(PF_RTS1)); });
          return FV<1>{{smp_of(psi, m.powf(MAXX(qv, 0.01f), -OWN(PF_BSW)))}};
    };
    auto eq_body = [&](int il, auto O, float zw, bool &bad, bool inl_all) __attribute__((always_inline)) -> FV<1> {
          const float zlo = cs.zi(il - 1), zhi = cs.zi(il);
          const float ts = O(PF_TS), psi = O(PF_PSI);
          const bool sat = zw <= zlo;
          const bool inl = (zw < zhi) && (zw > zlo);
          const float expo = one + O(PF_NINVB);
          auto rp = [&]() __attribute__((always_inline)) { return join_d(O(PF_RPSI0), O(PF_RPSI1)); };
          const float n0 = ((-psi) + zw - zlo), ni = (-psi + zw - zhi);
          float b0 = divr_d<CS::kRecip>(m, n0, -psi, rp, bad);
          float bi = divr_d<CS::kRecip>(m, ni, -psi, rp, bad);
          b0 = sat ? one : b0;
          bi = (sat || inl) ? one : bi;
          bool s0, si;
          const float temp0 = m.powf_d(b0, expo, s0);
          const float tpi = m.powf_d(bi, expo, si);
          bad |= s0 | si;
          float vin = zero;
          if (inl_all || any_lane(inl)) {
          H9G_BR(BR_INL);
          vin = vol_eq_in_fast(m, [&]() { return O(PF_PTE); }, ts, temp0, zw, zlo, zhi,
                               [&]() { return cs.rdz_t(il); }, inl, bad);
          }
          const float vbl = vol_eq_below(O(PF_C3), ts, tpi, temp0);
          const float vol_eq = sat ? ts : (inl ? vin : vbl);
          const float qv = divr_d<CS::kRts>(m, vol_eq, ts, [&]() { return join_d(O(PF_RTS0), O(PF_RTS1)); }, bad);
          bool sz;
          const float z = psi * m.powf_d(MAXX(qv, 0.01f), -O(PF_BSW), sz);
          bad |= sz;
          return FV<1>{{MAXC(smpmin, z)}};
    };
    auto eq_fast = [&](int t, int h, bool &bad) __attribute__((always_inline)) -> FV<1> {
          return eq_body(2 * t + 1 + h, [&](int p) __attribute__((always_inline)) { return OWN(p); }, zwtmm, bad,
                         false);
    };
    auto hk_exact = [&](int t, int h) __attribute__((always_inline)) -> FV<4> {
          H9G_BR(BR_HKX);
          const int i0 = 2 * t + 1;
          const int ip1 = (L < i0 + 2) ? L : i0 + 2;
          const float th = sel(h, theta[i0], theta[i0 + 1]);
          const float thp = sel(h, theta[i0 + 1], theta[ip1]);
          const float ts = OWN(PF_TS);
          const float tsp = sel(h, TS(i0 + 1), TS(ip1));
          float s1 = 0.5f * (th + thp) / (0.5f * (ts + tsp));
          s1 = MINC(one, s1);
          const float bsw = OWN(PF_BSW);
          const float s_node =
              sat_node(divr<CS::kRtsHK>(m, th, ts, [&]() { return join_d(OWN(PF_RTS0), OWN(PF_RTS1)); }));
          const float ek = 2.0f * bsw + 2.0f, es = -bsw;
          bool sk, ss;
          float pk = m.powf_d(s1, ek, sk);
          float ps = m.powf_d(s_node, es, ss);
          if (__builtin_expect(sk | ss, 0)) {
            m.powf_fix(pk, s1, ek, sk);
            m.powf_fix(ps, s_node, es, ss);
          }
          const float s2 = OWN(PF_HKS) * pk;
          FV<4> r;
          r.v[0] = s1 * s2;
          r.v[1] = (2.0f * bsw + 3.0f) * s2 * OWN(PF_ITS);
          const float sm = smp_of(OWN(PF_PSI), ps);
          r.v[2] = sm;
          r.v[3] = dsmpdw_div(bsw, sm, s_node, ts);
          return r;
    };
    auto hk_body = [&](auto O, float th, float thp, float tsp, bool &bad) __attribute__((always_inline)) -> FV<4> {
          const float ts = O(PF_TS);
          const float s1 = s1_mk(th + thp, ts + tsp, O(PF_ITS), bad);
          const float bsw = O(PF_BSW);
          const float s_node =
              sat_node(divr_d<CS::kRtsHK>(m, th, ts, [&]() { return join_d(O(PF_RTS0), O(PF_RTS1)); }, bad));
          const float ek = 2.0f * bsw + 2.0f, es = -bsw;
          bool sk, ss;
          const float pk = m.powf_d(s1, ek, sk);
          const float ps = m.powf_d(s_node, es, ss);
          bad |= sk | ss;
          FV<4> r;
          hk_dhk(s1, pk, O(PF_HKS), bsw, O(PF_ITS), r.v[0], r.v[1]);
          r.v[2] = smp_of(O(PF_PSI), ps);
          r.v[3] = dsmpdw_fast<L>(bsw, r.v[2], s_node, ts, bad);
          return r;
    };
    auto hk_fast = [&](int t, int h, bool &bad) __attribute__((always_inline)) -> FV<4> {
          const int i0 = 2 * t + 1;
          const int ip1 = (L < i0 + 2) ? L : i0 + 2;
          return hk_body([&](int p) __attribute__((always_inline)) { return OWN(p); }, sel(h, theta[i0], theta[i0 + 1]),
                         sel(h, theta[i0 + 1], theta[ip1]), sel(h, TS(i0 + 1), TS(ip1)), bad);
    };
    if constexpr (kTask) {
      constexpr int NA = 4 * L + 2;
      (void)outq;
      static_assert(NA <= 64 && CS::kRecip && CS::kRts && CS::kRtsHK, "a lane per task, every reciprocal stored");
      const bool st = sp.spare;
      const int hh = sp.h;
#if (H9G_P1_TASKS & 2)
      float den_l = g.den(1);
      double rden_l = g.rden(1);
// ... 230 lines not shown
          const lds_float *o = st ? cs.wb + k + u * S : cs.self + t * S;
          bool b = false;
          r[t] = eq_body(st ? 2 * u + 1 + (k & 1) : 2 * t + 1 + hh,
                         [&](int p) __attribute__((always_inline)) { return o[p * NT * S]; },
                         st ? zwk[q] : zwtmm, b, U + q == NT - 1);
          rv[q] = r[t].v[0];
          fl |= (b ? 1 : 0) << q;
        }
#pragma unroll
        for (int u = 0; u < U; u++) r[u].v[0] = back(rv, u);
        const bool bad = !st & ((fl != 0) | flags_back(fl));
        if (__builtin_expect(bad, 0)) {
#pragma unroll
          for (int t = 0; t < NT; t++) r[t] = eq_exact(t, hh);
        }
#pragma unroll
        for (int t = 0; t < NT; t++) sp.xchg(r[t].v[0], zq[2 * t + 1], zq[2 * t + 2]);
      }
      pr.mark(2);
      {
        float thu[U], thpu[U];
#pragma unroll
        for (int u = 0; u < U; u++) {
          thu[u] = sel(hh, theta[2 * u + 1], theta[2 * u + 2]);
          thpu[u] = sel(hh, theta[2 * u + 2], theta[2 * u + 3]);
        }
        float thk[R], thpk[R];
#pragma unroll
        for (int q = 0; q < R; q++) {
          const int tau = tau_q(q), k = tau % S, u = tau / S;
          float a = lane_get(thu[ulo(q)], k), b = lane_get(thpu[ulo(q)], k);
#pragma unroll
          for (int w = ulo(q) + 1; w <= uhi(q); w++) {
            const float ga = lane_get(thu[w], k), gb = lane_get(thpu[w], k);
            a = u == w ? ga : a;
            b = u == w ? gb : b;
          }
          thk[q] = a;
          thpk[q] = b;
        }
        const lds_float *pe = cs.even + PF_TS * NT * S + (hh ? S : 1);
        FV<4> r[NT];
        float rv[4][R];
        int fl = 0;
#pragma unroll
        for (int q = 0; q < R; q++) {
          const int tau = tau_q(q), k = tau % S, u = tau / S;
          const int t = U + q;
          const lds_float *o = st ? cs.wb + k + u * S : cs.self + t * S;
          const lds_float *pt_h = cs.wb + ((k & 1) ? (k & ~1) + S : (k | 1)) + (PF_TS * NT + u) * S;
          const lds_float *pt_own = t == NT - 1 ? cs.even + 1 + (PF_TS * NT + NT - 1) * S : pe + t * S;
          const lds_float *pt = st ? pt_h : pt_own;
          bool b = false;
          r[t] = hk_body([&](int p) __attribute__((always_inline)) { return o[p * NT * S]; },
                         st ? thk[q] : sel(hh, theta[2 * t + 1], theta[2 * t + 2]),
                         st ? thpk[q] : sel(hh, theta[2 * t + 2], theta[2 * t + 3 <= L ? 2 * t + 3 : L]), *pt, b);
#pragma unroll
          for (int kk = 0; kk < 4; kk++) rv[kk][q] = r[t].v[kk];
          fl |= (b ? 1 : 0) << q;
        }
#pragma unroll
        for (int kk = 0; kk < 4; kk++)
#pragma unroll
          for (int u = 0; u < U; u++) r[u].v[kk] = back(rv[kk], u);
        const bool bad = !st & ((fl != 0) | flags_back(fl));
        if (__builtin_expect(bad, 0)) {
#pragma unroll
          for (int t = 0; t < NT; t++) r[t] = hk_exact(t, hh);
        }
#pragma unroll
        for (int t = 0; t < NT; t++)
#pragma unroll
          for (int kk = 0; kk < 4; kk++) sp.xchg(r[t].v[kk], outk[kk][2 * t + 1], outk[kk][2 * t + 2]);
      }
    } else {
      sp.template par_d<NT, 1>(eq_fast, eq_exact, outq);
      pr.mark(2);
      sp.template par_d<NT, 4>(hk_fast, hk_exact, outk);
    }
  }
  if constexpr (SP::kSpare) {
    if (!sp.act()) return 0;
  }
  bool any_aq_v;
  if constexpr (kTask)
    any_aq_v = aq_task;
  else
    any_aq_v = any_lane(aq);
  const bool any_aq = any_aq_v;
  if (!kTask || __builtin_expect(picks, 0)) {
  const int jc = aq ? L : jwt + 1;
  float s1c = one, bsw_c = zero;
  if (any_lane(!aq)) {
    float th_j = zero;
#pragma unroll
    for (int i = 1; i <= L; i++)
      if (i == jc) th_j = theta[i];
    s1c = sat_node(divr<CS::kRts>(m, th_j, cs.lay(PF_TS, jc), [&]() { return lay_d(cs, PF_RTS0, jc); }));
    bsw_c = cs.lay(PF_BSW, jc);
  }
  sp.template pick<1>(
      [&](int h) __attribute__((always_inline)) -> FV<1> {
        const float npsi = -cs.lay(PF_PSI, jc);
        const float num = (aq && h == 0) ? (-PSI(L) + zwtmm - g.zi(L)) : zwtmm;
        bool sq = false, sw = false;
        float q = divr_d<CS::kRecip>(m, num, npsi, [&]() { return lay_d(cs, PF_RPSI0, jc); }, sq);
        const float ninv = cs.lay(PF_NINVB, jc);
        const float e = h ? ninv : (aq ? one + ninv : 2.0f * bsw_c + 3.0f);
        float w = m.powf_d(h ? one + q : (aq ? q : s1c), e, sw);
        if (__builtin_expect(sq | sw, 0)) {
          H9G_BR(BR_RECH);
          divr_fix<CS::kRecip>(m, q, num, npsi);
          w = m.powf(h ? one + q : (aq ? q : s1c), e);
        }
        return FV<1>{{w}};
      },
      p0, p1);
  const FV<1> pA = p0;
  if (any_aq) {
  H9G_BR(BR_ANYAQ);
  {
    const float d0 = aq ? (zwtmm - g.zi(L)) : one;
    const float ve = vol_clamp(vol_aq(LAYF(PF_PTE, L), d0, pA.v[0]), TS(L));
    sp.template pick<2>(
        [&](int h) __attribute__((always_inline)) -> FV<2> {
          const float xn = sel(h, ve, theta[L]);
          auto xof = [&](float q2) __attribute__((always_inline)) {
            const float sn = sat_node_aq(q2);
            const float x = sel(h, MAXX(q2, 0.01f), sn);
            return aq ? x : one;
          };
          bool sq = false, sw = false;
          float q2 = divr_d<CS::kRts>(m, xn, TS(L), [&]() { return lay_d(cs, PF_RTS0, L); }, sq);
          float x = xof(q2);
          float pw = m.powf_d(x, -BSW(L), sw);
          if (__builtin_expect(sq | sw, 0)) {
            H9G_BR(BR_AQS);
            divr_fix<CS::kRts>(m, q2, xn, TS(L));
            x = xof(q2);
            pw = m.powf(x, -BSW(L));
          }
          const float z = smp_of(PSI(L), pw);
          return FV<2>{{z, dsmpdw_div(BSW(L), z, x, TS(L))}};
        },
        eA, eS);
  }
  }
  }
  const FV<1> pY = p1;
  zq[L + 1] = aq ? eA.v[0] : zero;
  const float smp1 = eS.v[0], dsmpdw1 = eS.v[1];
  cs.launder();
  pr.mark(3);
  const float zcA = 0.5f * (zwtmm + g.zc(L));
  const float dzA = (jwt < L) ? g.dz(L) : zwtmm - g.zc(L);
  cs.launder();
  float dwat2[L + 2], GAM[L + 2];
  float BET = zero;
  double rbet = 0.0;
  int zero_pivot = 0;
  auto row = [&](int i, float am, float bm, float cm, float rm) __attribute__((always_inline)) {
    float x;
    if (i == 1) {
      BET = bm;
      x = rm;
    } else {
      BET = row_bet(am, bm, GAM[i]);
      if (BET == 0.0f && !zero_pivot) zero_pivot = i;
      x = row_x(am, rm, dwat2[i - 1]);
    }
    rbet = recip64(BET);
    dwat2[i] = m.div_d(x, BET, rbet);
    bool bad = m.div_bad(dwat2[i]);
    if (i <= L) {
      GAM[i + 1] = m.div_d(cm, BET, rbet);
      bad |= m.div_bad(GAM[i + 1]);
    }
    if (__builtin_expect(bad, 0)) {
      m.div_fix(dwat2[i], x, BET);
      if (i <= L) m.div_fix(GAM[i + 1], cm, BET);
    }
  };
  bool tri_ok = false;
  if constexpr (!M::kExact) {
    bool bad = false, zp = false;
    float qo[L + 1], d1[L + 1], d2[L + 1];
    auto flux3_f = [&](float hki, float num, float dsi, float dsn, float dhk, float den, double rden, int k,
                       bool &b) __attribute__((always_inline)) {
      qo[k] = m.div_d(flux_q(hki, num), den, rden);
      d1[k] = m.div_d(flux_d1(hki, num, dsi, dhk), den, rden);
      d2[k] = m.div_d(flux_d2(hki, num, dsn, dhk), den, rden);
      b |= m.div_bad(qo[k]) | m.div_bad(d1[k]) | m.div_bad(d2[k]);
    };
    if constexpr (kTask && (H9G_P1_TASKS & 2)) {
#pragma unroll
      for (int i = 1; i <= L; i++) {
        qo[i] = c_q[i];
        d1[i] = c_1[i];
        d2[i] = c_2[i];
      }
    }
    if (!kTask || __builtin_expect(!flux_done, 0)) {
#pragma unroll
    for (int i = 1; i <= L - 1; i++)
      flux3_f(hk[i], flux_num(smp[i + 1], smp[i], zq[i + 1], zq[i]), dsmpdw[i], dsmpdw[i + 1], dhkdw[i], g.den(i),
              g.rden(i), i, bad);
    qo[L] = d1[L] = d2[L] = zero;
    if (any_aq) {
      const float den = zcA - g.zc(L);
      bool ba = false;
      flux3_f(hk[L], flux_num(smp1, smp[L], zq[L + 1], zq[L]), dsmpdw[L], dsmpdw1, dhkdw[L], den, recip64(den), L, ba);
      bad |= aq && ba;
    }
    if (__builtin_expect(bad, 0)) {
      H9G_BR(BR_TRIFLUX);
#pragma unroll
      for (int i = 1; i <= L; i++) {
        const bool a = i == L;
        const float num = a ? flux_num(smp1, smp[L], zq[L + 1], zq[L]) : flux_num(smp[i + 1], smp[i], zq[i + 1], zq[i]);
        const float dsn = a ? dsmpdw1 : dsmpdw[i < L ? i + 1 : L];
        const float den = a ? zcA - g.zc(L) : g.den(i);
        m.div_fix(qo[i], flux_q(hk[i], num), den);
        m.div_fix(d1[i], flux_d1(hk[i], num, dsmpdw[i], dhkdw[i]), den);
        m.div_fix(d2[i], flux_d2(hk[i], num, dsn, dhkdw[i]), den);
      }
      bad = false;
    }
    }
    auto row_f = [&](int i, float am, float bm, float cm, float rm) __attribute__((always_inline)) {
      float x;
      if (i == 1) {
        BET = bm;
        x = rm;
      } else {
        BET = row_bet(am, bm, GAM[i]);
        zp |= BET == 0.0f;
        x = row_x(am, rm, dwat2[i - 1]);
      }
      if constexpr (kTask && (H9G_P1_TASKS & 4)) {
        dwat2[i] = i == L + 1 ? mk_div_z(x, BET, bad) : mk_div(x, BET, bad);
        if (i <= L) GAM[i + 1] = i == L ? mk_div_z(cm, BET, bad) : mk_div(cm, BET, bad);
      } else {
      const double rb = recip64(BET);
      dwat2[i] = m.div_d(x, BET, rb);
      bad |= m.div_bad(dwat2[i]);
      if (i <= L) {
        GAM[i + 1] = m.div_d(cm, BET, rb);
        bad |= m.div_bad(GAM[i + 1]);
      }
      }
    };
    auto dzdt = [&](float dz) __attribute__((always_inline)) {
      const float q = m.div_d(dz, dt, g.rdt());
      bad |= m.div_bad(q);
      return q;
    };
    const float bm1 = dzdt(g.dz(1)) + d1[1];
    row_f(1, zero, bm1, d2[1], qflx_infl - qo[1] - tran * ROOT(1));
#pragma unroll
    for (int i = 2; i <= L - 1; i++)
      row_f(i, -d1[i - 1], dzdt(g.dz(i)) - d2[i - 1] + d1[i], d2[i], qo[i - 1] - qo[i] - tran * ROOT(i));
    row_f(L, -d1[L - 1], dzdt(g.dz(L)) - d2[L - 1] + (aq ? d1[L] : zero), aq ? d2[L] : zero,
          qo[L - 1] - (aq ? qo[L] : zero) - tran * ROOT(L));
    const float qA = dzdt(dzA);
    const float bmA = qA - d2[L] + zero;
    const float rmA = qo[L] - zero;
    row_f(L + 1, aq ? -d1[L] : zero, aq ? bmA : qA, zero, aq ? rmA : zero);
    if (__builtin_expect(bad | zp | (bm1 == 0.0f), 0)) {
      H9G_BR(BR_TRISWEEP);
      BET = zero;
      zero_pivot = 0;
      const float bm1x = m.div(g.dz(1), dt, g.rdt()) + d1[1];
      if (bm1x == 0.0f) { errval = bm1x; return 1; }
      row(1, zero, bm1x, d2[1], qflx_infl - qo[1] - tran * ROOT(1));
#pragma unroll
      for (int i = 2; i <= L - 1; i++)
        row(i, -d1[i - 1], m.div(g.dz(i), dt, g.rdt()) - d2[i - 1] + d1[i], d2[i], qo[i - 1] - qo[i] - tran * ROOT(i));
      if (!aq) {
        row(L, -d1[L - 1], m.div(g.dz(L), dt, g.rdt()) - d2[L - 1] + zero, zero, qo[L - 1] - zero - tran * ROOT(L));
        row(L + 1, zero, m.div(dzA, dt, g.rdt()), zero, zero);
      } else {
        row(L, -d1[L - 1], m.div(g.dz(L), dt, g.rdt()) - d2[L - 1] + d1[L], d2[L], qo[L - 1] - qo[L] - tran * ROOT(L));
        row(L + 1, -d1[L], m.div(dzA, dt, g.rdt()) - d2[L] + zero, zero, qo[L] - zero);
      }
      if (zero_pivot) { errval = (float)zero_pivot; return 2; }
    }
    tri_ok = true;
  }
  if (!tri_ok) {
  auto flux3 = [&](float hki, float num, float dsi, float dsn, float dhk, float den, double rden, float &qo,
                   float &d1, float &d2) __attribute__((always_inline)) {
    const float x0 = flux_q(hki, num), x1 = flux_d1(hki, num, dsi, dhk), x2 = flux_d2(hki, num, dsn, dhk);
    qo = m.div_d(x0, den, rden);
    d1 = m.div_d(x1, den, rden);
    d2 = m.div_d(x2, den, rden);
    if (__builtin_expect(m.div_bad(qo) | m.div_bad(d1) | m.div_bad(d2), 0)) {
      m.div_fix(qo, x0, den);
      m.div_fix(d1, x1, den);
      m.div_fix(d2, x2, den);
    }
  };
  float q_prev, dq0_prev, dq1_prev;
  {
    const float den = g.den(1);
    const double rden = g.rden(1);
    const float dzq = (zq[2] - zq[1]);
// ... 172 lines not shown
    visit_layers(m, [&](int k) __attribute__((always_inline)) -> bool {
      const int i = jwt2 + 1 + k;
      const float s_y = k == 0 ? sy_drain : s_y_at(i, zwtmm);
      float rstl = MAXF(rsub_top_tot, -(s_y * (cs.zi(i) - zwtmm)));
      rstl = MINF(rstl, zero);
#pragma unroll
      for (int j = 1; j <= L; j++) {
        int hit = (j == i);
        opaque(hit);
        h2o[j] = hit ? h2o[j] + rstl : h2o[j];
      }
      rsub_top_tot = rsub_top_tot - rstl;
      if (rsub_top_tot >= zero) {
        s.zwt = s.zwt - wdiv(rstl / s_y);
        return false;
      }
      s.zwt = cs.zim(i);
      return i != L;
    });
    s.zwt = s.zwt - wdiv(rsub_top_tot) / rous;
    s.wa = s.wa + rsub_top_tot;
    jwt3 = jwt_of<L>(s.zwt, zim);
  }
  s.zwt = MAXF(0.0f, s.zwt);
  s.zwt = MINC(80.0f, s.zwt);
  cs.launder();
  pr.mark(6);
#pragma unroll
  for (int i = L; i >= 2; i--) {
    const float cap = MAXF(0.01f, TS(i)) * g.dz(i);
    const float xsi = MAXF(h2o[i] - cap, zero);
    h2o[i] = MINF(cap, h2o[i]);
    h2o[i - 1] = h2o[i - 1] + xsi;
  }
  const float xs1 = MAXF(MAXF(h2o[1], zero) - cs.sc(PS_TSDZ1), zero);
  h2o[1] = MINF(cs.sc(PS_TSDZ1), h2o[1]);
  float qflx_rsub_sat = m.div_d(xs1, dt, g.rdt());
  bool low = false;
#pragma unroll
  for (int i = 1; i <= L; i++) low |= h2o[i] < watmin;
  if (__builtin_expect(low | m.div_bad(qflx_rsub_sat), 0)) {
  H9G_BR(BR_WATMIN);
  m.div_fix(qflx_rsub_sat, xs1, dt);
#pragma unroll
  for (int i = 1; i <= L - 1; i++) {
    float xs = zero;
    if (h2o[i] < watmin) {
      xs = watmin - h2o[i];
      if (i == jwt3) s.zwt = s.zwt + m.div(xs / MAXF(0.01f, TS(i)), 1000.0f, r1000);
    }
    h2o[i] = h2o[i] + xs;
    h2o[i + 1] = h2o[i + 1] - xs;
  }
  float xs = zero;
  if (h2o[L] < watmin) {
    xs = watmin - h2o[L];
    bool active = true;
#pragma unroll
    for (int j = L - 1; j >= 1; j--) {
      if (active) {
        const float avail = MAXF(h2o[j] - watmin - xs, zero);
        if (avail >= xs) {
          h2o[L] = h2o[L] + xs;
          h2o[j] = h2o[j] - xs;
          xs = zero;
          active = false;
        } else {
          h2o[L] = h2o[L] + avail;
          h2o[j] = h2o[j] - avail;
          xs = xs - avail;
        }
      }
    }
  }
  h2o[L] = h2o[L] + xs;
  rsub_top = rsub_top - m.div(xs, dt, g.rdt());
  }
  float w1 = ((1.0f - frac_h2osfc) * (qflx_surf + evg + tran) + rsub_top + qflx_rsub_sat) * dt + s.wa;
#pragma unroll
  for (int i = 1; i <= L; i++) w1 = w1 + h2o[i];
  pr.mark(7);
  if (absf(w1 - w0) > 0.1f) { errval = w1 - w0; return 4; }
  rnf_sum = rnf_sum + qflx_surf * dt;
  rnf_sum = rnf_sum + rsub_top * dt;
  return 0;
#undef TS
#undef HKS
#undef BSW
#undef PSI
#undef LAYF
#undef ROOT
#undef DC
#undef OWN
}

template <int L, class SP, class CS>
H9K_HD void save_day(const SP &sp, const CS &cs, const St<L> &s, float rnf_sum, int ns) {
  save_layers<L>(sp, cs, 0, s.h2o);
  save_layers<L>(sp, cs, 1, s.smp);
  cs.sv_set_sc(SV_ZWT, s.zwt);
  cs.sv_set_sc(SV_WA, s.wa);
  cs.sv_set_sc(SV_RNF, rnf_sum);
  cs.sv_set_sc(SV_NS, (float)ns);
}

template <int L, class G, class CS>
H9K_RARE int substep_exact_pair(const G *g, CS cs, const uint64_t *e2, const double *l2, int ns) {
  cs.sv_sync();
  St<L> s;
#pragma unroll
  for (int i = 1; i <= L; i++) {
    s.h2o[i] = cs.sv_lay(0, i);
    s.smp[i] = cs.sv_lay(1, i);
  }
  s.zwt = cs.sv_sc(SV_ZWT);
  s.wa = cs.sv_sc(SV_WA);
  float rnf = cs.sv_sc(SV_RNF), errval = zero;
  MathExact me{{e2, l2}};
  const SplitAll sa;
  NoProf np;
  int code = 0;
  H9G_EXACT_HOOK((int)cs.sv_sc(SV_NS), ns);
  for (int k = (int)cs.sv_sc(SV_NS); k <= ns && !code; k++)
    code = hydrology_pair<L, G, MathExact, SplitAll, CS>(*g, cs, sa, s, rnf, errval, me, np);
  cs.launder();
#pragma unroll
  for (int i = 1; i <= L; i++) {
    cs.sv_set_lay(0, i, s.h2o[i]);
    cs.sv_set_lay(1, i, s.smp[i]);
  }
  cs.sv_set_sc(SV_ZWT, s.zwt);
  cs.sv_set_sc(SV_WA, s.wa);
  cs.sv_set_sc(SV_RNF, rnf);
  cs.sv_set_sc(SV_ERR, errval);
  cs.sv_set_sc(SV_NS, (float)(ns + 1));
  cs.sv_sync();
  return code;
}

template <int L, class G, class SP, class CS, class PR>
H9K_HD int substep_pair(const G &g, CS cs, const SP &sp, St<L> &s, float &rnf_sum, float &errval,
                        const h9m::Tabs &T, PR &pr, int ns, bool snapped) {
  pr.mark(0);
  H9G_BR(BR_SUBSTEP);
#if defined(H9G_ISA_MARK) && defined(__HIP_DEVICE_COMPILE__)
  asm volatile("; h9g-substep");
#endif
  MathFast mf{T, false};
#if defined(H9G_FORCE_RERUN)
  const bool in_column = s.zwt <= g.zim(L);
#elif defined(H9G_FORCE_RERUN_ANY)
  const bool in_column = true;
#endif
  int code = hydrology_pair<L, G, MathFast, SP, CS, PR>(g, cs, sp, s, rnf_sum, errval, mf, pr);
#if defined(H9G_FORCE_RERUN)
  if (sp.act() && in_column && ns % H9G_FORCE_RERUN == H9G_FORCE_RERUN - 1) mf.special = true;
#elif defined(H9G_FORCE_RERUN_ANY)
  if (sp.act() && in_column && ns % H9G_FORCE_RERUN_ANY == H9G_FORCE_RERUN_ANY - 1) mf.special = true;
#endif
  if (__builtin_expect(sp.pair_any(mf.special), 0)) {
    H9G_BR(BR_RERUN);
    if (!snapped) {
      errval = (float)ns;
      return H9G_ERR_NOSNAP_K;
    }
#if defined(H9G_COUNT_EXACT) && defined(__HIP_DEVICE_COMPILE__)
    atomicAdd(&h9g_exact_count, 1ull);
    atomicAdd(&h9g_exact_wave[(blockIdx.x * 4 + (threadIdx.x >> 6)) & 0xffff], 1u);
#endif
    cs.launder();
    code = substep_exact_pair<L, G, CS>(&g, cs, T.exp2, T.log2, ns);
    cs.launder();
#pragma unroll
    for (int i = 1; i <= L; i++) {
      s.h2o[i] = cs.sv_lay(0, i);
      s.smp[i] = cs.sv_lay(1, i);
    }
    s.zwt = cs.sv_sc(SV_ZWT);
    s.wa = cs.sv_sc(SV_WA);
    rnf_sum = cs.sv_sc(SV_RNF);
    errval = cs.sv_sc(SV_ERR);
  }
  return code;
}

H9K_HD int month_end(int d1, int nt) {
  if (d1 == 31) return 0;
  switch (d1 - (nt == 366 ? 1 : 0)) {
    case 59: return 1;
    case 90: return 2;
    case 120: return 3;
    case 151: return 4;
    case 181: return 5;
    case 212: return 6;
    case 243: return 7;
    case 273: return 8;
    case 304: return 9;
    case 334: return 10;
    case 365: return 11;
    default: return -1;
  }
}
struct NoMonths {
  template <int L>
  H9K_HD void day_end(int, int, const gbl_float *, size_t, float) const {}
};
struct Months {
  gbl_float *M;
  size_t stride;
  template <int L>
  H9K_HD void day_end(int day, int nt, const gbl_float *A, size_t as, float rnf_sum) const {
    const int m = month_end(day + 1, nt);
    if (m < 0) return;
    gbl_float *o = M + (size_t)m * (12 + L) * stride;
    float v[12 + L];
#pragma unroll
    for (int k = 0; k < 12 + L; k++) v[k] = k == 2 ? rnf_sum : k == 3 ? zero : A[k * as];
#pragma unroll
    for (int k = 0; k < 12 + L; k++) o[k * stride] = v[k];
  }
};

template <int L, class G, class SP, class CS, bool Park = true, class PR = NoProf, class MO = NoMonths>
H9K_HD int cell_year_pair(const G &g, CS cs, const SP &sp, St<L> &s, const gbl_float *forc, size_t fday,
                          size_t fvar, int nt, int nisurf, int grow_on, gbl_float *acc, size_t astride,
                          int &eday, int &estep, float &errval, const h9m::Tabs &T, int raw = 0,
                          PR &&pr = PR(), MO mo = MO()) {
  enum { A_NPP = 0, A_PM, A_RNF, A_EVAP, A_TAS, A_RLDS, A_RSDS, A_HUSS, A_PS, A_PR, A_RHS,
         A_THETA, A_H2O = 11 + L };
  gbl_float *A = acc;
  const size_t as = astride;
  float rnf_sum = zero;
  const bool act = sp.act();
  if (act) {
#pragma unroll
    for (int k = 0; k < 12 + L; k++) A[k * as] = zero;
  }
  auto park = [&]() __attribute__((always_inline)) {
    if constexpr (Park) {
      if (!act) return;
      cs.set_sc(PS_LAI, s.LAI);
      cs.set_sc(PS_LAIL, s.LAI_litter);
      cs.set_sc(PS_PM, s.pm);
      cs.set_sc(PS_PFM, s.pfm);
      cs.set_sc(PS_PLEN, s.plen);
      cs.set_sc(PS_RDEPTH, s.rdepth);
    }
  };
  park();
  float npp = zero;
  int code = 0;
  MathExact me{T};
  s.naq = 0;
  for (int day = 0; day < nt; day++) {
    cs.day_start(day);
    H9G_BR(BR_DAY);
#if defined(H9G_DUMP_AQ) && defined(__HIP_DEVICE_COMPILE__)
    if (act && h9g_aq_bits && s.zwt > g.zim(L)) {
      const size_t c = (size_t)((const float *)acc - h9g_aq_base);
      atomicOr(&h9g_aq_bits[c * 12 + day / 32], 1u << (day & 31));
    }
#endif
    cs.launder();
    opaque(A);
    const gbl_float *f = forc + (size_t)day * fday;
    opaque(f);
    if (act) {
      float fv[7];
#pragma unroll
      for (int k = 0; k < 7; k++) fv[k] = ld_stream(f + k * fvar);
      const Day d = make_day(fv[0], fv[1], fv[2], fv[3], fv[4], fv[5], fv[6]);
      if constexpr (Park)
        day_consts(d, cs.sc(PS_LAI), cs.sc(PS_LAIL), cs, me);
      else
        day_consts(d, s.LAI, s.LAI_litter, cs, me);
      float a7[7];
#pragma unroll
      for (int k = 0; k < 7; k++) a7[k] = A[(A_TAS + k) * as];
#pragma unroll
      for (int k = 0; k < 7; k++) A[(A_TAS + k) * as] = a7[k] + fv[k];
    }
    bool snapped = false;
    for (int ns = 0; ns < nisurf; ns++) {
      const bool in_column = s.zwt <= g.zim(L);
      s.naq += in_column ? 0 : 1;
      if (act && !snapped && in_column) {
        H9G_BR(BR_SNAP);
        save_day<L>(sp, cs, s, rnf_sum, ns);
        snapped = true;
      }
      code = substep_pair<L, G, SP, CS>(g, cs, sp, s, rnf_sum, errval, T, pr, ns, snapped);
      if (code) { eday = day; estep = ns; break; }
    }
    cs.launder();
    if constexpr (Park) {
      s.LAI = cs.sc(PS_LAI);
      s.LAI_litter = cs.sc(PS_LAIL);
      s.pm = cs.sc(PS_PM);
      s.pfm = cs.sc(PS_PFM);
      s.plen = cs.sc(PS_PLEN);
      s.rdepth = cs.sc(PS_RDEPTH);
    }
    if (code) return code;
    if (!act) continue;
    opaque(A);
    if (grow_on) {
      opaque(f);
      grow_day<L, G, MathExact>(g, ld_stream(f), s, cs, npp, me);
      park();
    }
    auto later = [](int k) { return k != A_RNF && k != A_EVAP && (k < A_TAS || k > A_RHS); };
    float a[12 + L];
#pragma unroll
    for (int k = 0; k < 12 + L; k++)
      if (later(k)) a[k] = A[k * as];
    a[A_PM] = a[A_PM] + s.pm;
    a[A_NPP] = a[A_NPP] + npp;
    float h2o_sum = a[A_H2O];
#pragma unroll
    for (int i = 1; i <= L; i++) {
      const float theta = MAXF(s.h2o[i], 1.0E-6f) / g.thk(i);
      a[A_THETA + i - 1] = a[A_THETA + i - 1] + theta;
      h2o_sum = h2o_sum + s.h2o[i];
    }
    a[A_H2O] = h2o_sum;
#pragma unroll
    for (int k = 0; k < 12 + L; k++)
      if (later(k)) A[k * as] = a[k];
    mo.template day_end<L>(day, nt, A, as, rnf_sum);
  }
  if (!act) return 0;
  opaque(A);
  if (raw) {
    A[A_RNF * as] = rnf_sum;
    return 0;
  }
  A[A_PM * as] = A[A_PM * as] / (float)nt;
  A[A_RNF * as] = rnf_sum / (float)(nt * nisurf);
  A[A_EVAP * as] = zero / (float)(nt * nisurf);
#pragma unroll
  for (int k = A_TAS; k <= A_H2O; k++) A[k * as] = A[k * as] / (float)nt;
  return 0;
}

template <int L, class G, class CS>
H9K_HD int cell_site(const G &g, CS cs, St<L> &s, float h2o_ma1, const float *sub, const float *daily,
                     const float *lai, float *out, size_t n, int nday, int nisurf, int &eday, int &estep,
                     float &errval, const h9m::Tabs &T) {
  MathExact me{T};
  const SplitAll sp;
  FluxProf fx{zero, zero};
  float rnf_sum = zero;
  const float dt = g.dt();
  const float theta_ma1 = h2o_ma1 / g.thk(1);
  for (int day = 0; day < nday; day++) {
    const float *l = lai + (size_t)day * 3 * n;
    if (l[0] == l[0]) s.LAI = l[0];
    if (l[n] == l[n]) s.LAI_litter = s.LAI_litter + l[n] - l[2 * n];
    const float *dd = daily + (size_t)day * 2 * n;
    float evap_day = zero, evap_grnd_day = zero;
    for (int ns = 0; ns < nisurf; ns++) {
      const float *v = sub + ((size_t)day * nisurf + ns) * 5 * n;
      Day d;
      d.tak = v[0] + tf;
      d.rh = v[n];
      d.Rnet = v[2 * n];
      d.PAR = v[3 * n];
      d.forc_rain = v[4 * n] / dt;
      d.lamb = ((2503.0f - 2.386f * (d.tak - tf))) * 1.0E3f;
      d.huss = dd[0];
      d.ps = dd[n];
      day_consts(d, s.LAI, s.LAI_litter, cs, me);
      const int code = hydrology_pair<L, G, MathExact, SplitAll, CS, FluxProf>(g, cs, sp, s, rnf_sum, errval,
                                                                            me, fx);
      if (code) { eday = day; estep = ns; return code; }
      evap_day = evap_day + (fx.evg + fx.tran) * dt;
      evap_grnd_day = evap_grnd_day + fx.evg * dt;
    }
    float *o = out + (size_t)day * 11 * n;
    o[0] = evap_day;
    o[n] = evap_grnd_day;
#pragma unroll
    for (int i = 1; i <= 4; i++) o[(1 + i) * n] = MAXF(s.h2o[i], 1.0E-6f) / g.thk(i);
    o[6 * n] = theta_ma1;
    o[7 * n] = s.LAI;
    o[8 * n] = s.LAI_litter;
    o[9 * n] = zero;
    o[10 * n] = zero;
  }
  return 0;
}

struct FocusYear {
  const float *forc;
  int nt;
};

template <int L, class G, class CS>
H9K_HD int cell_focus(const G &g, CS cs, St<L> &s, float h2o_ma1, const FocusYear *yrs, int nyears, size_t cell,
                      size_t fday, size_t fvar, int nisurf, int grow_on, float *out, size_t n,
                      const h9m::Tabs &T) {
  MathExact me{T};
  const SplitAll sp;
  FluxProf fx{zero, zero};
  float rnf_sum = zero, errval = zero, npp = zero;
  const float dt = g.dt();
  const float theta_ma1 = h2o_ma1 / g.thk(1);
  const float nan = __builtin_nanf("");
  gbl_float *o = (gbl_float *)out;
  int code = 0;
  for (int y = 0; y < nyears; y++) {
    const gbl_float *forc = (const gbl_float *)yrs[y].forc + cell;
    const int nt = yrs[y].nt;
    for (int day = 0; day < nt; day++, o += 11 * n) {
      float evap_day = zero, evap_grnd_day = zero, w_i = zero, fT = zero;
      if (!code) {
        const gbl_float *f = forc + (size_t)day * fday;
        float fv[7];
#pragma unroll
        for (int k = 0; k < 7; k++) fv[k] = ld_stream(f + k * fvar);
        const Day d = make_day(fv[0], fv[1], fv[2], fv[3], fv[4], fv[5], fv[6]);
        day_consts(d, s.LAI, s.LAI_litter, cs, me);
        for (int ns = 0; ns < nisurf && !code; ns++) {
          code = hydrology_pair<L, G, MathExact, SplitAll, CS, FluxProf>(g, cs, sp, s, rnf_sum, errval, me, fx);
          evap_day = evap_day + (fx.evg + fx.tran) * dt;
          evap_grnd_day = evap_grnd_day + fx.evg * dt;
        }
        if (!code && grow_on) {
          grow_drivers<L>(fv[0], s, cs, w_i, fT);
          grow_day<L, G, MathExact>(g, fv[0], s, cs, npp, me);
        }
      }
      if (code) {
#pragma unroll
        for (int r = 0; r < 11; r++) o[r * n] = nan;
        continue;
      }
      o[0] = evap_day;
      o[n] = evap_grnd_day;
#pragma unroll
      for (int i = 1; i <= 4; i++) o[(1 + i) * n] = MAXF(s.h2o[i], 1.0E-6f) / g.thk(i);
      o[6 * n] = theta_ma1;
      o[7 * n] = s.LAI;
      o[8 * n] = s.LAI_litter;
      o[9 * n] = w_i;
      o[10 * n] = fT;
    }
  }
  return code;
}

}
```

Measured before the change: 4.321 billion.

## Split pair1 substep across a helper front wave for small cell counts

```diff
diff --git a/hybrid9_amd/csrc/h9g.hip b/hybrid9_amd/csrc/h9g.hip
--- a/hybrid9_amd/csrc/h9g.hip
+++ b/hybrid9_amd/csrc/h9g.hip
@@ -84,24 +84,27 @@
 template <int L>
 constexpr int pair_waves() { return pair_resident<L>(); }
 
-template <int L, class G, int R, int C = H9G_PCPW, bool MON = false>
+template <int L, class G, int R, int C = H9G_PCPW, bool MON = false, bool FRONT = false>
 __device__ __forceinline__ void pair_body(const KArgs &a, const G &g, float *mon = nullptr) {
-  typedef PairStore<L, 2 * C, R> PS;
+  typedef PairStore<L, 2 * C, R, FRONT ? 1 : 0> PS;
+  static_assert(!FRONT || C == 1, "the front wave serves a one-column wave");
+  constexpr int NW = FRONT ? 1 : H9G_PWAVES;
   __shared__ uint64_t s_e2[32];
   __shared__ double s_l2[32];
-  __shared__ float s_cell[H9G_PWAVES][PS::ROWS * 2 * C];
+  __shared__ float s_cell[NW][PS::ROWS * 2 * C];
   __shared__ float s_zt[zt_size<L>()];
   static_assert(sizeof(s_e2) + sizeof(s_l2) + sizeof(s_cell) + sizeof(s_zt) <= (size_t)PS::GBLOCK,
                 "pair kernel LDS footprint exceeds the day-snapshot block");
   if (threadIdx.x == 0) fill_zt<L>(g, s_zt);
   load_tabs(s_e2, s_l2);
   const h9m::Tabs T = {s_e2, s_l2};
-  const int wave = threadIdx.x >> 6, lane = threadIdx.x & 63;
+  const int wave = FRONT ? 0 : threadIdx.x >> 6, lane = threadIdx.x & 63;
+  const bool front_wave = FRONT && __builtin_amdgcn_readfirstlane((int)(threadIdx.x >> 6)) != 0;
   const bool spare = lane >= 2 * C;
   if (spare && !PS::kSpare) return;
   const int h = lane & 1;
   const int slot0 = __builtin_amdgcn_readfirstlane(
-      a.c0 + (int)(xcd_vwg(blockIdx.x, gridDim.x) * H9G_PWAVES + wave) * C);
+      a.c0 + (int)(xcd_vwg(blockIdx.x, gridDim.x) * NW + wave) * C);
   const bool g2 = slot0 >= a.split;
   const int lim = g2 ? a.cend : a.bend;
   float *const st = g2 ? a.st2 : a.st;
@@ -147,14 +150,27 @@
   if (!spare) {
     H9K_TS_SUM(L, cs, ts_sum)
     if (!(ts_sum > SOIL_TRUNC) || err[c] != 0) {
-      if (h == 0) nan_rows(a.annual, Rows<L>::ANNUAL, ios, io);
+      if (h == 0 && !front_wave) nan_rows(a.annual, Rows<L>::ANNUAL, ios, io);
       if constexpr (MON)
-        if (h == 0) nan_rows(mon, H9G_NMONTHS * Rows<L>::ANNUAL, ios, io);
+        if (h == 0 && !front_wave) nan_rows(mon, H9G_NMONTHS * Rows<L>::ANNUAL, ios, io);
       return;
     }
     cell_inv_pair<L, G>(g, cs);
   }
   if (__builtin_amdgcn_ballot_w64(!spare) == 0) return;
+  if constexpr (FRONT) {
+    if (front_wave) {
+#if defined(H9G_STAMPS)
+      StampProf fp{stamp_clock(), {0, 0, 0, 0, 0, 0, 0, 0}};
+      front_year_pair<L, G>(g, cs, sp, T, fp);
+      if (lane == 0 && a.stamps)
+        for (int k = 0; k < 8; k++) a.stamps[(gridDim.x + blockIdx.x) * 8 + k] = fp.acc[k];
+#else
+      front_year_pair<L, G>(g, cs, sp, T);
+#endif
+      return;
+    }
+  }
   int eday = 0, estep = 0;
   float errval = 0.0f;
 #if defined(H9G_STAMPS)
@@ -163,7 +179,7 @@
                                                          a.nisurf, a.grow_on, (gbl_float *)(a.annual + io), ios, eday,
                                                          estep, errval, T, a.raw, pr);
   if (lane == 0 && a.stamps)
-    for (int k = 0; k < 8; k++) a.stamps[(blockIdx.x * H9G_PWAVES + wave) * 8 + k] = pr.acc[k];
+    for (int k = 0; k < 8; k++) a.stamps[(blockIdx.x * NW + wave) * 8 + k] = pr.acc[k];
 #else
   int code;
   if constexpr (MON)
@@ -213,6 +229,14 @@
 h9g_pair1_kernel(const KArgs a, const G g) {
   pair_body<L, G, 1, 1>(a, g);
 }
+#define H9G_PAIR1_FRONT_MAX 512
+#if H9G_P1_FRONT
+template <int L, class G>
+__global__ void __launch_bounds__(128) __attribute__((amdgpu_waves_per_eu(1, 1)))
+h9g_pair1f_kernel(const KArgs a, const G g) {
+  pair_body<L, G, 1, 1, false, true>(a, g);
+}
+#endif
 
 
 #define H9G_SOLO_BODY(MON, mon)                                                                                    \
@@ -294,14 +318,21 @@
 h9g_pair1_mon_kernel(const KArgs a, float *mon, const G g) {
   pair_body<L, G, 1, 1, true>(a, g, mon);
 }
+#if H9G_P1_FRONT
+template <int L, class G>
+__global__ void __launch_bounds__(128) __attribute__((amdgpu_waves_per_eu(1, 1)))
+h9g_pair1f_mon_kernel(const KArgs a, float *mon, const G g) {
+  pair_body<L, G, 1, 1, true, true>(a, g, mon);
+}
+#endif
 template <int L, class G>
 __global__ void __launch_bounds__(H9G_YBLOCK) __attribute__((amdgpu_waves_per_eu(2, 2)))
 h9g_solo_mon_kernel(const KArgs a, float *mon, const G g) {
   H9G_SOLO_BODY(true, mon)
 }
 
-int h9g_mon_launch(int kind, const h9g_config *cfg, unsigned grid, unsigned block, hipStream_t stream, const KArgs &a,
-                   float *mon);
+int h9g_mon_launch(int kind, bool p1f, const h9g_config *cfg, unsigned grid, unsigned block, hipStream_t stream,
+                   const KArgs &a, float *mon);
 int h9g_mon_stopped(int n, int rows, const int *err0, float *mon, hipStream_t stream);
 
 #if !defined(H9G_MONTHLY_UNIT)
@@ -893,6 +924,9 @@
   }
 }
 
+static bool pair1_front(size_t cells) { return H9G_P1_FRONT && cells <= H9G_PAIR1_FRONT_MAX; }
+static int launch_block_cells(int kind, bool p1f) { return p1f ? 1 : kind_info(kind).block_cells; }
+
 struct h9g_ctx {
   h9g_config cfg;
   int device = 0;
@@ -914,7 +948,7 @@
   int last_year = 0;
   int params_set = 0, state_set = 0, ran = 0;
   h9g_error last_err{};
-  std::string kname;
+  std::string kname, targs;
   unsigned *d_stamps = nullptr;
   std::vector<int64_t> h_gid;
   std::vector<float *> h_pin;
@@ -945,6 +979,8 @@
   size_t n_solo = 0;
   size_t ios = 0;
   size_t stamp_words = 0;
+  bool stamp_p1f = false;
+  size_t stamp_blocks = 0;
   int ev_kind[NEVT] = {};
   int64_t ev_cells[NEVT] = {};
   double kstat[K_NSTAT][3] = {};
@@ -970,6 +1006,10 @@
   int mon_years = 0;
   bool mon_in_ret = false;
 };
+
+static std::string pair1_name(const h9g_ctx *ctx, bool p1f) {
+  return std::string("h9g_pair1") + (p1f ? "f" : "") + "_kernel" + ctx->targs;
+}
 
 static void ord_free(h9g_ctx *ctx);
 
@@ -1076,8 +1116,8 @@
   return 0;
 }
 
-int h9g_mon_launch(int kind, const h9g_config *cfg, unsigned grid, unsigned block, hipStream_t stream, const KArgs &a,
-                   float *mon) {
+int h9g_mon_launch(int kind, bool p1f, const h9g_config *cfg, unsigned grid, unsigned block, hipStream_t stream,
+                   const KArgs &a, float *mon) {
   const struct { int L; h9g_config cfg; } c{cfg->nlayers, *cfg};
   switch (kind) {
     case K_SOLO: H9G_DISPATCH(&c, h9g_solo_mon_kernel, grid, block, stream, a, mon); break;
@@ -1086,7 +1126,15 @@
       H9G_DISPATCH_L10(&c, h9g_pair2_mon_kernel, grid, block, stream, a, mon);
       break;
     case K_PAIR11: H9G_DISPATCH(&c, h9g_pair11_mon_kernel, grid, block, stream, a, mon); break;
-    case K_PAIR1: H9G_DISPATCH(&c, h9g_pair1_mon_kernel, grid, block, stream, a, mon); break;
+    case K_PAIR1:
+#if H9G_P1_FRONT
+      if (p1f) {
+        H9G_DISPATCH(&c, h9g_pair1f_mon_kernel, grid, block, stream, a, mon);
+        break;
+      }
+#endif
+      H9G_DISPATCH(&c, h9g_pair1_mon_kernel, grid, block, stream, a, mon);
+      break;
     case K_PAIR: H9G_DISPATCH(&c, h9g_pair_mon_kernel, grid, block, stream, a, mon); break;
     default: return H9G_EINVAL;
   }
@@ -1175,7 +1223,7 @@
   const size_t n = (size_t)cfg->ncell, L = (size_t)cfg->nlayers;
   const size_t ios = 2 * round_up(n, H9G_PCPW) + 64;
   const size_t blocks = std::max((ios + (size_t)H9G_PCPW11 * H9G_PWAVES - 1) / ((size_t)H9G_PCPW11 * H9G_PWAVES),
-                                 (size_t)1024 / H9G_PWAVES);
+                                 std::max((size_t)1024 / H9G_PWAVES, (size_t)H9G_PAIR1_FRONT_MAX));
   const size_t prows = par_rows(cfg->nlayers), srows = state_rows(cfg->nlayers), arows = annual_rows(cfg->nlayers);
   return sizeof(float) * (prows + srows + 7 * (size_t)cfg->max_days * (size_t)cfg->nslots + arows + 1) * n +
          sizeof(float) * (7 * (size_t)cfg->max_days + arows) * ios + sizeof(int) * 2 * ios +
@@ -1313,7 +1361,10 @@
   const GeoKind gk = geo_kind(*cfg);
   const std::string targs = "<" + std::to_string(L) + "," +
                             (gk == GEO_R ? "GeoR" : "GeoC<" + std::to_string(L) + "," + std::to_string((int)gk) + ">") + ">";
-  auto kernel_name = [&](int k) { return "h9g_" + std::string(kind_info(k).env) + "_kernel" + targs; };
+  ctx->targs = targs;
+  auto kernel_name = [&](int k) {
+    return k == K_PAIR1 ? pair1_name(ctx, pair1_front(ctx->n)) : "h9g_" + std::string(kind_info(k).env) + "_kernel" + targs;
+  };
   ctx->kname = ctx->kind == K_MIXED ? kernel_name(K_SOLO) + "+" + kernel_name(K_PAIR) : kernel_name(ctx->kind);
   return ctx;
 }
@@ -1504,7 +1555,8 @@
 
 struct LaunchRange { int c0, cend, cpb; Kind kind; };
 static int year_ranges(const h9g_ctx *ctx, LaunchRange r[2]) {
-  const int n = (int)ctx->n, ns = (int)ctx->n_solo, cpb = kind_info(ctx->kind).block_cells;
+  const int n = (int)ctx->n, ns = (int)ctx->n_solo;
+  const int cpb = launch_block_cells(ctx->kind, ctx->kind == K_PAIR1 && pair1_front(ctx->n));
   int k = 0;
   if (ctx->kind != K_MIXED) {
     r[k++] = {0, n, cpb, ctx->kind};
@@ -1515,11 +1567,11 @@
   return k;
 }
 
-static int launch_year(h9g_ctx *ctx, int kind, KArgs a, size_t blocks, float *mon) {
-  const unsigned pb = (unsigned)blocks, pt = 64 * H9G_PWAVES;
+static int launch_year(h9g_ctx *ctx, int kind, KArgs a, size_t blocks, float *mon, bool p1f) {
+  const unsigned pb = (unsigned)blocks, pt = p1f ? 128 : 64 * H9G_PWAVES;
   if (mon && kind != K_MIXED) {
     const bool solo = kind == K_SOLO;
-    if (int rc = h9g_mon_launch(kind, &ctx->cfg, solo ? (unsigned)(((size_t)(a.cend - a.c0) + H9G_YBLOCK - 1) / H9G_YBLOCK) : pb,
+    if (int rc = h9g_mon_launch(kind, p1f, &ctx->cfg, solo ? (unsigned)(((size_t)(a.cend - a.c0) + H9G_YBLOCK - 1) / H9G_YBLOCK) : pb,
                                 solo ? H9G_YBLOCK : pt, ctx->sc, a, mon))
       return rc;
     HIPCHK(hipGetLastError());
@@ -1536,13 +1588,21 @@
       for (int i = 0; i < nr; i++) {
         a.c0 = r[i].c0;
         a.cend = a.bend = a.split = r[i].cend;
-        if (int rc = launch_year(ctx, r[i].kind, a, blocks, mon)) return rc;
+        if (int rc = launch_year(ctx, r[i].kind, a, blocks, mon, false)) return rc;
       }
       return 0;
     }
     case K_PAIR2: H9G_DISPATCH_L10(ctx, h9g_pair2_kernel, pb, pt, ctx->sc, a); break;
     case K_PAIR11: H9G_DISPATCH(ctx, h9g_pair11_kernel, pb, pt, ctx->sc, a); break;
-    case K_PAIR1: H9G_DISPATCH(ctx, h9g_pair1_kernel, pb, pt, ctx->sc, a); break;
+    case K_PAIR1:
+#if H9G_P1_FRONT
+      if (p1f) {
+        H9G_DISPATCH(ctx, h9g_pair1f_kernel, pb, pt, ctx->sc, a);
+        break;
+      }
+#endif
+      H9G_DISPATCH(ctx, h9g_pair1_kernel, pb, pt, ctx->sc, a);
+      break;
     default: H9G_DISPATCH(ctx, h9g_pair_kernel, pb, pt, ctx->sc, a); break;
   }
   HIPCHK(hipGetLastError());
@@ -1611,6 +1671,7 @@
   const Kind kind = d_list && !ys.bulk ? list_kind(ctx, m) : ctx->kind;
   const KindInfo ki = kind_info(kind);
   const size_t ncells = d_list ? (size_t)m : ctx->n;
+  const bool p1f = kind == K_PAIR1 && pair1_front(ncells);
   if (d_list || ctx->sort) {
     if (!ctx->d_forc_s) HIPCHK(hipMalloc(&ctx->d_forc_s, sizeof(float) * 7 * (size_t)ctx->cfg.max_days * ios));
     if (!ctx->d_ann_s) HIPCHK(hipMalloc(&ctx->d_ann_s, sizeof(float) * annual_rows(ctx->L) * ios));
@@ -1634,7 +1695,7 @@
     return 0;
   };
   if (d_list) {
-    const int pcpb = ki.block_cells;
+    const int pcpb = launch_block_cells(kind, p1f);
     a.perm = d_list;
     if (ctx->sort && kind != K_PAIR1) {
       H9G_DISPATCH(ctx, h9g_sort_kernel, H9G_NXCD, H9G_SORT_THREADS, ctx->sc, n, 0, m, pcpb, a.st, a.err, ctx->d_hist,
@@ -1671,7 +1732,7 @@
   }
   if (a.sorted_io) a.fvar = dvar;
   float *const mon_a = !mon ? nullptr : a.sorted_io ? ctx->d_mon_s : ctx->d_mon;
-  const size_t per_block = (size_t)ki.block_cells;
+  const size_t per_block = (size_t)launch_block_cells(kind, p1f);
   const size_t blocks = kind == K_MIXED ? (ctx->n - ctx->n_solo + per_block - 1) / per_block
                                         : ((size_t)a.cend + per_block - 1) / per_block;
   if (ki.pair) {
@@ -1704,6 +1765,8 @@
     }
     HIPCHK(hipMemsetAsync(ctx->d_stamps, 0, sizeof(unsigned) * words, ctx->sc));
     a.stamps = ctx->d_stamps;
+    ctx->stamp_p1f = p1f;
+    ctx->stamp_blocks = blocks;
   }
 #endif
   if (ctx->nev >= NEVT)
@@ -1734,7 +1797,8 @@
   ctx->ev_kind[e] = ys.probe ? K_PROBE : kind;
   ctx->ev_cells[e] = (int64_t)ncells + (two ? ys.k2 : 0);
   HIPCHK(hipEventRecord(ctx->ev0[e], ctx->sc));
-  if (int r = launch_year(ctx, kind, a, blocks, mon_a)) return r;
+  if (int r = launch_year(ctx, kind, a, blocks, mon_a, p1f)) return r;
+  if (kind == K_PAIR1 && ctx->kind == K_PAIR1) ctx->kname = pair1_name(ctx, p1f);
   HIPCHK(hipEventRecord(ctx->ev1[e], ctx->sc));
   HIPCHK(hipEventRecord(ctx->ev_consumed[ys.slot], ctx->sc));
   if (two) HIPCHK(hipEventRecord(ctx->ev_consumed[ys.slot2], ctx->sc));
@@ -2546,6 +2610,14 @@
     fprintf(stderr, "h9g stamps (cycles/wave/substep):");
     for (int k = 0; k < 8; k++) { fprintf(stderr, " p%d=%.0f", k, sum[k] / steps); tot += sum[k]; }
     fprintf(stderr, " total=%.0f\n", tot / steps);
+    if (ctx->stamp_p1f) {
+      std::vector<unsigned> fs(8 * nw);
+      HIPCHK(hipMemcpy(fs.data(), ctx->d_stamps + 8 * ctx->stamp_blocks, sizeof(unsigned) * 8 * nw, hipMemcpyDeviceToHost));
+      double w = 0, f = 0;
+      for (size_t k = 0; k < nw; k++) { w += fs[8 * k]; f += fs[8 * k + 1]; }
+      fprintf(stderr, "h9g stamps, front waves (cycles/wave/substep): wait at barrier 1=%.0f front=%.0f\n", w / steps,
+              f / steps);
+    }
     std::vector<double> wt(nw, 0.0);
     for (size_t w = 0; w < nw; w++)
       for (int k = 0; k < 8; k++) wt[w] += st[8 * w + k];
diff --git a/hybrid9_amd/csrc/h9g_pair.h b/hybrid9_amd/csrc/h9g_pair.h
--- a/hybrid9_amd/csrc/h9g_pair.h
+++ b/hybrid9_amd/csrc/h9g_pair.h
@@ -48,6 +48,13 @@
 #ifndef H9G_P1_TASKS
 #define H9G_P1_TASKS 7
 #endif
+#ifndef H9G_P1_FRONT
+#define H9G_P1_FRONT 1
+#endif
+enum : int { ROLE_ALL = 0, ROLE_FRONT = 1, ROLE_MAIN = 2 };
+struct FrontRes {
+  float qflx_surf, tran, evg, qflx_infl;
+};
 
 template <int K>
 struct FV {
@@ -126,7 +133,7 @@
 
 template <int L>
 struct FlatStore {
-  static constexpr bool kRecip = true, kRts = true, kDayRecip = true, kRtsHK = true, kSpare = false;
+  static constexpr bool kRecip = true, kRts = true, kDayRecip = true, kRtsHK = true, kSpare = false, kFront = false;
   static constexpr int N = PF_N * L + PS_N;
   float *b;
   const float *zt;
@@ -213,15 +220,22 @@
 template <int L>
 constexpr int pair_resident() { return 3; }
 
-template <int L, int S, int R = pair_resident<L>()>
+template <int L, int S, int R = pair_resident<L>(), int F = 0>
 struct PairStore {
   static constexpr int NT = L / 2;
+  static constexpr bool kFront = F != 0;
+  static_assert(!kFront || S == 2, "the front wave serves a one-column wave");
   static constexpr bool kRecip = true, kRts = L <= 8 || R <= 2 || S <= 22, kDayRecip = L <= 8 || R <= 2 || S <= 22;
   static constexpr bool kRtsHK = kRts;
   static constexpr int NPF = kRecip ? (kRts ? PF_SVH2O : PF_RTS0) : PF_RPSI0;
   static constexpr int NPS = kDayRecip ? PS_SVZWT : PS_DR0;
   static constexpr int TH0 = (NPF * NT + (NPS + 1) / 2) * S;
-  static constexpr int ROWS = NPF * NT + (NPS + 1) / 2 + (S == 2 ? NT : 0);
+  enum : int {
+    HO_SMP = TH0 + L, HO_H2O1 = HO_SMP + L, HO_ZWT, HO_GO, HO_PAD,
+    HO_SURF, HO_TRAN, HO_EVG, HO_INFL, HO_END
+  };
+  static_assert((HO_END - TH0 - L) % 2 == 0, "whole rows");
+  static constexpr int ROWS = NPF * NT + (NPS + 1) / 2 + (S == 2 ? NT : 0) + (kFront ? (HO_END - HO_SMP) / 2 : 0);
   static constexpr int GBLOCK = 65536;
   lds_float *self, *even;
   const lds_float *zt;
@@ -254,6 +268,15 @@
     asm volatile("" : "+v"(self), "+v"(even), "+v"(zt)::"memory");
 #endif
   }
+  __device__ __forceinline__ float ho(int k) const { return wb[k]; }
+  __device__ __forceinline__ void set_ho(int k, float v) const { wb[k] = v; }
+  __device__ __forceinline__ void wg_sync() const {
+#if defined(__HIP_DEVICE_COMPILE__)
+    __builtin_amdgcn_fence(__ATOMIC_RELEASE, "workgroup");
+    __builtin_amdgcn_s_barrier();
+    __builtin_amdgcn_fence(__ATOMIC_ACQUIRE, "workgroup");
+#endif
+  }
   __device__ __forceinline__ float day(int f) const { return sc(PS_DAY + f); }
   __device__ __forceinline__ void set_day(int f, float v) const { set_sc(PS_DAY + f, v); }
   __device__ __forceinline__ double day_r(int k) const {
@@ -299,7 +322,7 @@
 
 template <int L>
 struct SoloStore {
-  static constexpr bool kRecip = false, kRts = false, kDayRecip = false, kRtsHK = false, kSpare = false;
+  static constexpr bool kRecip = false, kRts = false, kDayRecip = false, kRtsHK = false, kSpare = false, kFront = false;
   static constexpr int NPF = PF_RPSI0 + 2;
   static constexpr int NPS = PS_LAI + 5;
   static constexpr int ROWS = NPF * L + NPS;
@@ -580,9 +603,9 @@
     return false;
 }
 
-template <int L, class G, class M, class SP, class CS, class PR = NoProf>
+template <int L, class G, class M, class SP, class CS, class PR = NoProf, int ROLE = ROLE_ALL>
 H9K_HD int hydrology_pair(const G &g, CS cs, const SP &sp0, St<L> &s, float &rnf_sum, float &errval,
-                          M &m, PR &pr) {
+                          M &m, PR &pr, FrontRes *fr = nullptr) {
   constexpr int NT = L / 2;
   const SP sp = L >= 10 ? sp0.fresh() : sp0;
   const float dt = g.dt();
@@ -602,7 +625,12 @@
 #define DC(F) cs.sc(PS_DAY + F)
 #define OWN(p) sp.own(cs, p, t, h)
 
-  float w0 = DC(D_FORC) * dt + s.wa;
+  float w0 = zero;
+  if constexpr (ROLE == ROLE_FRONT) {
+    theta[1] = m.div_d(h2o[1], g.thk(1), g.rthk(1));
+    m.div_fix(theta[1], h2o[1], g.thk(1));
+  } else {
+  w0 = DC(D_FORC) * dt + s.wa;
   bool bad = false;
 #pragma unroll
   for (int i = 1; i <= L; i++) {
@@ -615,12 +643,15 @@
 #pragma unroll
     for (int i = 1; i <= L; i++) m.div_fix(theta[i], h2o[i], g.thk(i));
   }
-  const float qflx_top_soil = DC(D_FORC);
+  }
   const float hkdepth = one / 2.5f;
   const float fff = 1.0f / hkdepth;
+  const float frac_h2osfc = zero;
+  float qflx_surf = zero, tran = zero, evg = zero, qflx_infl = zero;
+  if constexpr (ROLE != ROLE_MAIN) {
+  const float qflx_top_soil = DC(D_FORC);
   const float fsat = cs.sc(PS_FMAX) * m.expf(-0.5f * fff * s.zwt);
-  float qflx_surf = fsat * qflx_top_soil;
-  const float frac_h2osfc = zero;
+  qflx_surf = fsat * qflx_top_soil;
   float beta = zero;
   {
     float rb[L + 1];
@@ -655,7 +686,7 @@
     rss = (10.0f + DC(D_LIT1000) * (1.0f - divr<CS::kRts>(m, theta[1], TS(1), [&]() { return lay_d(cs, PF_RTS0, 1); })));
   const float desatdT = DC(D_DESAT), gamma = DC(D_GAMMA);
   const float Ra = DC(D_DG) * DC(D_RAA);
-  float rsc, tran, evg;
+  float rsc;
   bool eb_fast = false;
   if constexpr (H9G_EB_FAST && !M::kExact && CS::kDayRecip) {
     bool bad = false;
@@ -764,13 +795,18 @@
   qflx_in_soil = qflx_in_soil - (one - frac_h2osfc) * qflx_evap;
   const float qinmax = (one - fsat) * cs.sc(PS_MH3);
   const float qflx_infl_excess = MAXF(zero, qflx_in_soil - (one - frac_h2osfc) * qinmax);
-  const float qflx_infl = qflx_in_soil - qflx_infl_excess;
+  qflx_infl = qflx_in_soil - qflx_infl_excess;
   qflx_surf = qflx_surf + qflx_infl_excess;
+  }
+  if constexpr (ROLE == ROLE_FRONT) {
+    *fr = FrontRes{qflx_surf, tran, evg, qflx_infl};
+    return 0;
+  }
   float zwtmm = 1000.0f * s.zwt;
   const int jwt = jwt_of<L>(s.zwt, zim);
   const bool aq = (jwt == L);
   cs.launder();
-  pr.mark(1);
+  if constexpr (ROLE != ROLE_MAIN) pr.mark(1);
 
   float zq[L + 2];
   float hk[L + 1], dhkdw[L + 1], dsmpdw[L + 1];
@@ -1307,6 +1343,14 @@
   const float smp1 = eS.v[0], dsmpdw1 = eS.v[1];
   cs.launder();
   pr.mark(3);
+  if constexpr (ROLE == ROLE_MAIN) {
+    cs.wg_sync();
+    qflx_surf = cs.ho(CS::HO_SURF);
+    tran = cs.ho(CS::HO_TRAN);
+    evg = cs.ho(CS::HO_EVG);
+    qflx_infl = cs.ho(CS::HO_INFL);
+    pr.mark(1);
+  }
   const float zcA = 0.5f * (zwtmm + g.zc(L));
   const float dzA = (jwt < L) ? g.dz(L) : zwtmm - g.zc(L);
   cs.launder();
@@ -1785,7 +1829,8 @@
 #elif defined(H9G_FORCE_RERUN_ANY)
   const bool in_column = true;
 #endif
-  int code = hydrology_pair<L, G, MathFast, SP, CS, PR>(g, cs, sp, s, rnf_sum, errval, mf, pr);
+  int code = hydrology_pair<L, G, MathFast, SP, CS, PR, CS::kFront ? ROLE_MAIN : ROLE_ALL>(g, cs, sp, s, rnf_sum,
+                                                                                            errval, mf, pr);
 #if defined(H9G_FORCE_RERUN)
   if (sp.act() && in_column && ns % H9G_FORCE_RERUN == H9G_FORCE_RERUN - 1) mf.special = true;
 #elif defined(H9G_FORCE_RERUN_ANY)
@@ -1854,6 +1899,45 @@
   }
 };
 
+template <int L, class SP, class CS>
+H9K_HD void front_post(const SP &sp, const CS &cs, const St<L> &s) {
+#pragma unroll
+  for (int t = 0; t < L / 2; t++) cs.set_ho(CS::HO_SMP + 2 * t + sp.h, sel(sp.h, s.smp[2 * t + 1], s.smp[2 * t + 2]));
+  cs.set_ho(CS::HO_H2O1, s.h2o[1]);
+  cs.set_ho(CS::HO_ZWT, s.zwt);
+  cs.set_ho(CS::HO_GO, zero);
+}
+template <class CS>
+H9K_HD void front_done(const CS &cs) {
+  cs.set_ho(CS::HO_GO, one);
+  cs.wg_sync();
+}
+template <int L, class G, class SP, class CS, class PR = NoProf>
+H9K_HD void front_year_pair(const G &g, CS cs, const SP &sp, const h9m::Tabs &T, PR &&pr = PR()) {
+  if (sp.spare) return;
+  St<L> s{};
+  float rnf_sum = zero, errval = zero;
+  for (;;) {
+    cs.wg_sync();
+    cs.launder();
+    if (lane0_get(cs.ho(CS::HO_GO)) != zero) break;
+    pr.mark(0);
+#pragma unroll
+    for (int i = 1; i <= L; i++) s.smp[i] = cs.ho(CS::HO_SMP + i - 1);
+    s.h2o[1] = cs.ho(CS::HO_H2O1);
+    s.zwt = cs.ho(CS::HO_ZWT);
+    MathFast mf{T, false};
+    FrontRes fr;
+    hydrology_pair<L, G, MathFast, SP, CS, PR, ROLE_FRONT>(g, cs, sp, s, rnf_sum, errval, mf, pr, &fr);
+    pr.mark(1);
+    cs.set_ho(CS::HO_SURF, fr.qflx_surf);
+    cs.set_ho(CS::HO_TRAN, fr.tran);
+    cs.set_ho(CS::HO_EVG, fr.evg);
+    cs.set_ho(CS::HO_INFL, fr.qflx_infl);
+    cs.wg_sync();
+  }
+}
+
 template <int L, class G, class SP, class CS, bool Park = true, class PR = NoProf, class MO = NoMonths>
 H9K_HD int cell_year_pair(const G &g, CS cs, const SP &sp, St<L> &s, const gbl_float *forc, size_t fday,
                           size_t fvar, int nt, int nisurf, int grow_on, gbl_float *acc, size_t astride,
@@ -1922,7 +2006,12 @@
         save_day<L>(sp, cs, s, rnf_sum, ns);
         snapped = true;
       }
+      if constexpr (CS::kFront) {
+        if (act) front_post<L>(sp, cs, s);
+        cs.wg_sync();
+      }
       code = substep_pair<L, G, SP, CS>(g, cs, sp, s, rnf_sum, errval, T, pr, ns, snapped);
+      if constexpr (CS::kFront) code = lane0_geti(code);
       if (code) { eday = day; estep = ns; break; }
     }
     cs.launder();
@@ -1934,7 +2023,10 @@
       s.plen = cs.sc(PS_PLEN);
       s.rdepth = cs.sc(PS_RDEPTH);
     }
-    if (code) return code;
+    if (code) {
+      if constexpr (CS::kFront) front_done(cs);
+      return code;
+    }
     if (!act) continue;
     opaque(A);
     if (grow_on) {
@@ -1962,6 +2054,7 @@
       if (later(k)) A[k * as] = a[k];
     mo.template day_end<L>(day, nt, A, as, rnf_sum);
   }
+  if constexpr (CS::kFront) front_done(cs);
   if (!act) return 0;
   opaque(A);
   if (raw) {
```

After: 4.513 billion, median of 6. +4.4%, better.
